# phantomzone-org/fhe-ram

Measured on AMD Instinct MI355X. Metric: encrypted RAM read ops/s + write ops/s at 2^18 entries; achieved HBM GB/s vs peak, higher is better.
Workload: dtype f64

## Files before the change

### fhe-ram_amd/csrc/ctx.hpp

```cpp
#pragma once
#include "../../include/fheram.h"
#include "kernels.hpp"
#include "cmux_chain.hpp"
#include "mapped_chains.hpp"

#include <algorithm>
#include <atomic>
#include <cstdio>
#include <cstdlib>
#include <cstring>
#include <map>
#include <string>
#include <vector>

using namespace fk;

namespace {

thread_local std::string g_create_err;


struct ProfCls {
    uint64_t launches = 0, blocks = 0;
    double ms = 0.0;
    std::vector<std::pair<hipEvent_t, hipEvent_t>> pending;
};

}

inline uint64_t next_addr_id() { static std::atomic<uint64_t> n{0}; return ++n; }

struct RamState {
    bool initialized = false, state = false;
    bool memo_top = false;
    int memo_alone = 0;
    bool res_in_trtop = false;
};

struct DenseBufs {
    int cap = 0;
    int32_t *A = nullptr, *B = nullptr, *C = nullptr, *D = nullptr;
    int32_t *part = nullptr, *tmp = nullptr, *tmp2 = nullptr, *res = nullptr, *tree = nullptr, *w = nullptr, *trtop = nullptr;
    double* prep = nullptr;
    int64_t *h_res = nullptr, *d_h_res = nullptr;
};

inline fheram_config config_builtin() {
    fheram_config d{};
    d.limb_split = 1; d.fine_split = 1; d.memo = 1; d.pre_inv = 1; d.tail = 1; d.tail_test = 0; d.mid = 2; d.mid_test = 0;
    d.chain = 1; d.chain_y = 3; d.pair_z = 1; d.fuse = 1; d.graph = 0; d.safe = 0; d.nco = 0; d.tail_ep = 1; d.monitor = 1; d.reserved = 0;
    return d;
}
inline fheram_config config_in_effect(const fheram_config& in) {
    using C = fheram_config;
    fheram_config e{};
    for (int32_t C::*on_off : {&C::limb_split, &C::fine_split, &C::memo, &C::tail, &C::tail_ep, &C::mid_test, &C::chain, &C::pair_z, &C::fuse, &C::graph, &C::safe})
        e.*on_off = in.*on_off ? 1 : 0;
    for (int32_t C::*upto2 : {&C::tail_test, &C::mid, &C::monitor}) e.*upto2 = in.*upto2 < 0 ? 0 : (in.*upto2 > 2 ? 2 : in.*upto2);
    e.chain_y = in.chain_y ? 3 : 0;
    e.nco = in.nco == 2 ? 2 : (in.nco == 1 ? 1 : 0);
    e.pre_inv = e.memo ? (in.pre_inv == 2 ? 2 : (in.pre_inv ? 1 : 0)) : 0;
    if (e.graph) e.pre_inv = 0;
    if (e.safe) { e.tail = 0; e.tail_test = 0; e.mid = 0; e.mid_test = 0; if (e.pre_inv == 1) e.pre_inv = 2; }
    if (e.safe && e.monitor == 1) e.monitor = 2;
    return e;
}

struct CtxResources {
    std::vector<void*> dev, pinned;
    std::vector<hipEvent_t> events;
    template <typename T> hipError_t device(T** p, size_t bytes) { const hipError_t e = hipMalloc((void**)p, bytes); if (e == hipSuccess) dev.push_back(*p); return e; }
    template <typename T> hipError_t host(T** p, size_t bytes, unsigned flags) { const hipError_t e = hipHostMalloc((void**)p, bytes, flags); if (e == hipSuccess) pinned.push_back(*p); return e; }
    hipError_t event(hipEvent_t* ev, bool timing = false) {
        const hipError_t e = timing ? hipEventCreate(ev) : hipEventCreateWithFlags(ev, hipEventDisableTiming);
        if (e == hipSuccess) events.push_back(*ev);
        return e;
    }
    void release() {
        for (hipEvent_t e : events) hipEventDestroy(e);
        for (void* p : dev) hipFree(p);
        for (void* p : pinned) hipHostFree(p);
        events.clear(); dev.clear(); pinned.clear();
    }
};

struct fheram_ctx {
    fheram_params p;
    int device = 0;
    int ws = 0, n2 = 0, n_digits = 0, max_digits = 0;
    size_t rows = 0;
    size_t rows_glob = 0;
    int shard = 0, n_shards = 1;
    std::vector<std::vector<int>> base2d;
    static constexpr int S_CT = 3, S_ADDR = 4, S_INV = 5, DNUM_CT = 3, DNUM_GGSW = 4;
    int s_evk = 4;
    size_t atk = 0;
    static constexpr size_t GLWE = (size_t)S_CT * 2 * N;
    static constexpr size_t GLWE4 = (size_t)S_ADDR * 2 * N;
    static constexpr size_t GGSW = (size_t)DNUM_CT * 2 * GLWE4;
    static constexpr size_t EVK5 = (size_t)DNUM_GGSW * S_INV * 2 * N;
    static constexpr size_t GGSW5 = (size_t)DNUM_GGSW * 2 * S_INV * 2 * N;
    int cus = 256;
    CtxResources res;
    hipStream_t stream = nullptr;
    hipStream_t stream2 = nullptr;
    hipStream_t cur = nullptr;
    hipEvent_t ev_fork = nullptr, ev_join = nullptr;
    hipEvent_t ev_xout = nullptr, ev_xin = nullptr;
    fheram_config cfg = config_builtin();
    bool wide = false;
    double* d_tw = nullptr;
    double ninv = 0.0;
    double* d_atk = nullptr;
    double* d_atk_inv = nullptr;
    double* d_tsk = nullptr;
    int64_t gal[LOGN];
    bool keys_loaded = false;
    unsigned* h_ro_flag = nullptr;
    int32_t* d_data = nullptr;
    int32_t* d_tree = nullptr;
    int32_t* d_scrA = nullptr;
    int32_t* d_scrB = nullptr;
    int32_t* d_scrC = nullptr;
    int32_t* d_scrD = nullptr;
    int32_t* d_res = nullptr;
    int32_t* d_tmp = nullptr;
    int32_t* d_tmp2 = nullptr;
    int32_t* d_w = nullptr;
    int32_t* d_trtop = nullptr;
    int32_t* d_part = nullptr;
    int32_t* d_gat[3] = {nullptr, nullptr, nullptr};
    RamState ram;
    DenseBufs batch;
    double* d_big = nullptr;
    double* d_big2 = nullptr;
    double* d_prep = nullptr;
    bool prep1_ready = false;
    int32_t* d_ggsw_tmp = nullptr;
    int32_t* d_ggsw_tmp2 = nullptr;
    unsigned tail_seq = 0;
    int tail_xoff = 0;
    uint64_t tail_launches = 0;
    unsigned* h_tail_fb = nullptr;
    unsigned tail_fb_mark = 0;
    uint64_t tail_launch_mark = 0;
    unsigned* d_tail_sync = nullptr;
    unsigned mid_seq = 0;
    uint64_t mid_launches = 0, mid_launch_mark = 0;
    unsigned mid_fb_mark = 0;
    int mid_bad_windows = 0, mid_saved = 0;
    uint64_t mid_window_cts = 0, mid_disabled_count = 0;
    unsigned mid_off_ops = 0;
    unsigned* h_mid_fb = nullptr;
    unsigned* d_mid_sync[2] = {nullptr, nullptr};
    double* d_mid_big[2] = {nullptr, nullptr};
    double* d_mid_y[2] = {nullptr, nullptr};
    uint64_t inv_id[2] = {0, 0};
    double* d_prep_inv = nullptr;
    int32_t* d_ggsw_inv = nullptr;
    hipEvent_t ev_inv[2] = {nullptr, nullptr};
    bool inv_pending[2] = {false, false};
    hipEvent_t ev_wdone = nullptr;
    bool wdone_pending = false;
    hipEvent_t ev_opstart = nullptr;
    bool opstart_valid = false;
    bool wide_unsynced = false;
    bool derive_unsynced = false;
    bool main_idle = false;
    int32_t* h_pin[2] = {nullptr, nullptr};
    hipEvent_t ev_pin[2] = {nullptr, nullptr};
    int64_t* h_res = nullptr;
    int64_t* d_h_res = nullptr;
    int32_t* h_w = nullptr;
    hipEvent_t ev_w = nullptr;
    bool w_busy = false;
    bool side_begun = false;
    bool trhi_in_C = false;
    bool tree_rotate_pending = false;
    bool words_staged = false;
    int profile = 0;
    std::map<std::string, ProfCls> prof;
    std::vector<hipEvent_t> ev_pool;
    hipEvent_t t0 = nullptr, t1 = nullptr;
    std::string err;
};

struct fheram_addr {
    fheram_ctx* ctx;
    int32_t* d_ggsw;
    int n_digits;
    int device;
    uint64_t id = next_addr_id();
    hipGraphExec_t graph[3] = {nullptr, nullptr, nullptr};
    unsigned graph_sig[3] = {0, 0, 0};
    bool empty = false;
};

struct fheram_fheuint {
    fheram_ctx* ctx;
    int device, n_bits;
    int32_t* d_std;
    double* d_prep;
};

struct fheram_secret {
    fheram_ctx* ctx;
    int device;
    std::vector<int32_t> sk;
    double* d_hat;
};

namespace {

int fail(fheram_ctx* c, int code, const std::string& msg) {
    if (c) c->err = msg; else g_create_err = msg;
    return code;
}
int check_precision(fheram_ctx* c) {
    if (c->h_ro_flag && __atomic_load_n(c->h_ro_flag, __ATOMIC_RELAXED))
        return fail(c, FHERAM_ERR_PRECISION, "FP64 round-off of an inverse transform exceeded 3/8 (fheram_roundoff_max): the rounded integers are no longer trustworthy");
    return FHERAM_OK;
}
#define HIPCHK(c, call)                                                                     \
    do {                                                                                    \
        hipError_t e_ = (call);                                                             \
        if (e_ != hipSuccess)                                                               \
            return fail((c), FHERAM_ERR_DEVICE, std::string(#call) + ": " + hipGetErrorString(e_)); \
    } while (0)

GlweRef ref(int32_t* p, long sy, long sx) { return GlweRef{p, sy, sx}; }

void main_waited(fheram_ctx* c) { c->wide_unsynced = c->derive_unsynced = false; c->main_idle = true; }
void main_enqueued(fheram_ctx* c) { c->main_idle = false; }

hipEvent_t get_event(fheram_ctx* c) {
    if (!c->ev_pool.empty()) { hipEvent_t e = c->ev_pool.back(); c->ev_pool.pop_back(); return e; }
    hipEvent_t e = nullptr; c->res.event(&e, true); return e;
}
struct ProfScope {
    fheram_ctx* c; ProfCls* cls = nullptr; hipEvent_t a = nullptr;
    ProfScope(fheram_ctx* c_, const char* name, uint64_t blocks, int steps = 1) : c(c_) {
        if (!c->profile) return;
        if (c->profile == 2 && !strstr(name, "chain_launch")) return;
        cls = &c->prof[name];
        cls->launches += steps; cls->blocks += blocks * steps;
        a = get_event(c);
        hipEventRecord(a, c->cur);
    }
    ~ProfScope() {
        if (!cls) return;
        hipEvent_t b = get_event(c);
        hipEventRecord(b, c->cur);
        cls->pending.emplace_back(a, b);
    }
};
void prof_collect(fheram_ctx* c) {
    for (auto& kv : c->prof) {
        for (auto& pr : kv.second.pending) {
            hipEventSynchronize(pr.second);
            float ms = 0.f;
            hipEventElapsedTime(&ms, pr.first, pr.second);
            kv.second.ms += ms;
            c->ev_pool.push_back(pr.first); c->ev_pool.push_back(pr.second);
        }
        kv.second.pending.clear();
    }
}

std::vector<std::vector<int>> base_2d(uint64_t max_addr, const fheram_params& p) {
    std::vector<std::vector<int>> plan;
    uint32_t x = (uint32_t)(max_addr - 1), bits = 0;
    while (x) { bits++; x >>= 1; }
    while (bits != 0) {
        std::vector<int> v;
        for (uint32_t i = 0; i < p.n_decomp; i++) {
            const uint32_t b = p.decomp_n[i];
            if (b <= bits) { v.push_back((int)b); bits -= b; }
            else { if (bits != 0) { v.push_back((int)bits); bits = 0; } break; }
        }
        plan.push_back(v);
    }
    return plan;
}
int ilog2_ceil(size_t x) { int k = 0; while (((size_t)1 << k) < x) k++; return k; }
int galois_mod(int64_t g) { const int64_t m = 2 * N; return (int)(((g % m) + m) % m); }
int galois_inv_mod(int g) {
    int64_t r = 1, b = g, e = N - 1, m = 2 * N;
    while (e) { if (e & 1) r = r * b % m; b = b * b % m; e >>= 1; }
    return (int)r;
}
int64_t galois_element(int i) {
    if (i == 0) return -1;
    int64_t g = 5, e = (int64_t)1 << (i - 1), r = 1, m = 2 * N;
    while (e) { if (e & 1) r = r * g % m; g = g * g % m; e >>= 1; }
    return r;
}

bool narrow(const int64_t* src, int32_t* dst, size_t n) {
    int64_t bad = 0;
    for (size_t i = 0; i < n; i++) {
        const int64_t v = src[i];
        bad |= (v > 65536) | (v < -65536);
        dst[i] = (int32_t)v;
    }
    return bad == 0;
}
void widen(const int32_t* src, int64_t* dst, size_t n) { for (size_t i = 0; i < n; i++) dst[i] = src[i]; }

constexpr size_t PIN_CHUNK = (size_t)1 << 21;
int pin_init(fheram_ctx* c) {
    if (c->h_pin[0]) return FHERAM_OK;
    for (int b = 0; b < 2; b++) {
        HIPCHK(c, c->res.host(&c->h_pin[b], PIN_CHUNK * sizeof(int32_t), hipHostMallocDefault));
        HIPCHK(c, c->res.event(&c->ev_pin[b]));
    }
    return FHERAM_OK;
}
int upload_i64(fheram_ctx* c, int32_t* dst, const int64_t* src, size_t n) {
    int rc = pin_init(c);
    if (rc != FHERAM_OK) return rc;
    bool ok = true;
    int k = 0;
    for (size_t off = 0; off < n && ok; off += PIN_CHUNK, k++) {
        const int b = k & 1;
        const size_t m = std::min(PIN_CHUNK, n - off);
        if (k >= 2) HIPCHK(c, hipEventSynchronize(c->ev_pin[b]));
        ok = narrow(src + off, c->h_pin[b], m);
        if (!ok) break;
        HIPCHK(c, hipMemcpyAsync(dst + off, c->h_pin[b], m * sizeof(int32_t), hipMemcpyHostToDevice, c->stream));
        HIPCHK(c, hipEventRecord(c->ev_pin[b], c->stream));
    }
    HIPCHK(c, hipStreamSynchronize(c->stream));
    if (!ok) return fail(c, FHERAM_ERR_RANGE, "limb out of the normalised range [-2^16, 2^16]");
    return FHERAM_OK;
}
int download_i64(fheram_ctx* c, int64_t* dst, const int32_t* src, size_t n) {
    int rc = pin_init(c);
    if (rc != FHERAM_OK) return rc;
    const size_t n_chunks = (n + PIN_CHUNK - 1) / PIN_CHUNK;
    for (size_t k = 0; k <= n_chunks; k++) {
        if (k < n_chunks) {
            const size_t off = k * PIN_CHUNK, m = std::min(PIN_CHUNK, n - off);
            HIPCHK(c, hipMemcpyAsync(c->h_pin[k & 1], src + off, m * sizeof(int32_t), hipMemcpyDeviceToHost, c->stream));
            HIPCHK(c, hipEventRecord(c->ev_pin[k & 1], c->stream));
        }
        if (k > 0) {
            const size_t off = (k - 1) * PIN_CHUNK, m = std::min(PIN_CHUNK, n - off);
            HIPCHK(c, hipEventSynchronize(c->ev_pin[(k - 1) & 1]));
            widen(c->h_pin[(k - 1) & 1], dst + off, m);
        }
    }
    return FHERAM_OK;
}
int stage_words(fheram_ctx* c, int32_t* d_w, const int64_t* w, int n_ct) {
    if (c->w_busy) { HIPCHK(c, hipEventSynchronize(c->ev_w)); c->w_busy = false; }
    const size_t n = (size_t)n_ct * fheram_ctx::GLWE;
    if (!narrow(w, c->h_w, n)) return fail(c, FHERAM_ERR_RANGE, "limb out of the normalised range [-2^16, 2^16]");
    main_enqueued(c);
    HIPCHK(c, hipMemcpyAsync(d_w, c->h_w, n * sizeof(int32_t), hipMemcpyHostToDevice, c->stream));
    HIPCHK(c, hipEventRecord(c->ev_w, c->stream));
    c->w_busy = true;
    return FHERAM_OK;
}

}
```

### fhe-ram_amd/csrc/fheram.hip

```cpp
#include <unistd.h>
#include <atomic>
#include "path.hpp"

extern "C" {

int fheram_params_default(fheram_params* p) {
    if (!p) return FHERAM_ERR_INVALID_ARG;
    std::memset(p, 0, sizeof(*p));
    p->log_n = 12; p->base2k = 17; p->rank = 1;
    p->k_glwe_pt = 3; p->k_glwe_ct = 51; p->k_ggsw_addr = 68; p->k_evk_trace = 68; p->k_evk_ggsw_inv = 85;
    p->word_size = 4; p->n_decomp = 4;
    p->decomp_n[0] = p->decomp_n[1] = p->decomp_n[2] = p->decomp_n[3] = 3;
    p->max_addr = (uint64_t)1 << 14;
    return FHERAM_OK;
}

const char* fheram_last_error(const fheram_ctx* c) { return c ? c->err.c_str() : g_create_err.c_str(); }

void fheram_config_default(fheram_config* cfg) {
    if (!cfg) return;
    fheram_config d = config_builtin();
    auto env = [](const char* n) { const char* v = getenv(n); return (v && v[0]) ? v[0] : '\0'; };
    if (env("FHERAM_LIMB_SPLIT") == '0') d.limb_split = 0;
    if (env("FHERAM_FINE_SPLIT") == '0') d.fine_split = 0;
    if (env("FHERAM_MEMO") == '0') d.memo = 0;
    if (env("FHERAM_PRE_INV") == '0') d.pre_inv = 0; else if (env("FHERAM_PRE_INV") == '2') d.pre_inv = 2;
    const char tl = env("FHERAM_TAIL");
    if (tl == '0') d.tail = 0;
    d.tail_test = tl == '2' ? 1 : (tl == '3' ? 2 : 0);
    const char md = env("FHERAM_MID");
    d.mid = md == '0' ? 0 : (md == '1' ? 1 : 2);
    d.mid_test = md == '2' ? 1 : 0;
    if (env("FHERAM_CHAIN") == '0') d.chain = 0;
    if (env("FHERAM_CHAIN_Y") == '0') d.chain_y = 0;
    if (env("FHERAM_PAIR_Z") == '0') d.pair_z = 0;
    if (env("FHERAM_FUSE") == '0') d.fuse = 0;
    if (env("FHERAM_GRAPH") == '1') d.graph = 1;
    if (env("FHERAM_SAFE") == '1') d.safe = 1;
    const char nc = env("FHERAM_NCO");
    d.nco = nc == '2' ? 2 : (nc == '1' ? 1 : 0);
    if (env("FHERAM_TAIL_EP") == '0') d.tail_ep = 0;
    const char mo = env("FHERAM_MONITOR");
    if (mo == '0') d.monitor = 0; else if (mo == '2') d.monitor = 2;
    *cfg = d;
}

int fheram_ctx_create(const fheram_params* p, int device, fheram_ctx** out) {
    return fheram_ctx_create_cfg(p, device, 0, 1, nullptr, out);
}

int fheram_ctx_create_sharded(const fheram_params* p, int device, int shard, int n_shards, fheram_ctx** out) {
    return fheram_ctx_create_cfg(p, device, shard, n_shards, nullptr, out);
}

int fheram_ctx_create_cfg(const fheram_params* p, int device, int shard, int n_shards, const fheram_config* user_cfg, fheram_ctx** out) {
    if (!p || !out) return fail(nullptr, FHERAM_ERR_INVALID_ARG, "null argument");
    *out = nullptr;
    if (n_shards < 1 || shard < 0 || shard >= n_shards || (n_shards & (n_shards - 1)) != 0)
        return fail(nullptr, FHERAM_ERR_INVALID_ARG, "n_shards must be a power of two and 0 <= shard < n_shards");
    auto limbs = [&](uint32_t k) { return (k + p->base2k - 1) / (p->base2k ? p->base2k : 1); };
    if (p->log_n != 12 || p->base2k != 17 || p->rank != 1 || p->k_glwe_ct == 0 || limbs(p->k_glwe_ct) != 3 || limbs(p->k_ggsw_addr) != 4 ||
        (limbs(p->k_evk_trace) != 4 && limbs(p->k_evk_trace) != 5) || limbs(p->k_evk_ggsw_inv) != 5)
        return fail(nullptr, FHERAM_ERR_UNSUPPORTED, "kernels are built for LOG_N=12, BASE2K=17, RANK=1 and limb counts K_CT: 3, K_ADDR: 4, K_EVK_TRACE: 4 or 5, K_EVK_GGSW_INV: 5");
    if (p->k_glwe_pt == 0 || p->k_glwe_pt > p->k_glwe_ct)
        return fail(nullptr, FHERAM_ERR_INVALID_ARG, "k_glwe_pt must be in [1, k_glwe_ct]");
    if (p->word_size == 0 || p->word_size > 64 || p->n_decomp == 0 || p->n_decomp > 16 || p->max_addr < 2)
        return fail(nullptr, FHERAM_ERR_INVALID_ARG, "bad word_size / decomp_n / max_addr");
    unsigned sum = 0;
    for (uint32_t i = 0; i < p->n_decomp; i++) { if (p->decomp_n[i] == 0) return fail(nullptr, FHERAM_ERR_INVALID_ARG, "zero digit width"); sum += p->decomp_n[i]; }
    if (sum != p->log_n) return fail(nullptr, FHERAM_ERR_INVALID_ARG, "DECOMP_N must sum to LOG_N (parameters.rs:168)");
    if (p->max_addr > ((uint64_t)N * N)) return fail(nullptr, FHERAM_ERR_UNSUPPORTED, "max_addr > N^2 is not supported by the reference either (SURVEY.md 3.1)");
    if (user_cfg && user_cfg->reserved != 0)
        return fail(nullptr, FHERAM_ERR_INVALID_ARG, "fheram_config.reserved must be 0 (start from fheram_config_default())");

    int ndev = 0;
    if (hipGetDeviceCount(&ndev) != hipSuccess || ndev <= 0)
        return fail(nullptr, FHERAM_ERR_DEVICE, "no HIP device: the FHE-RAM evaluator has no CPU path");
    if (device < 0 || device >= ndev) return fail(nullptr, FHERAM_ERR_INVALID_ARG, "bad device index");

    fheram_ctx* c = new fheram_ctx();
    c->p = *p; c->device = device; c->ws = (int)p->word_size;
    c->s_evk = (int)limbs(p->k_evk_trace);
    c->atk = (size_t)fheram_ctx::DNUM_CT * c->s_evk * 2 * N;
    c->rows_glob = (size_t)((p->max_addr + N - 1) / N);
    c->shard = shard; c->n_shards = n_shards;
    if (n_shards > 1 && ((c->rows_glob & (c->rows_glob - 1)) != 0 || c->rows_glob < (size_t)n_shards)) {
        delete c;
        return fail(nullptr, FHERAM_ERR_INVALID_ARG, "row sharding needs a power-of-two number of rows >= n_shards (else: replicas only)");
    }
    c->rows = c->rows_glob / (size_t)n_shards;
    c->base2d = base_2d(p->max_addr, *p);
    c->n2 = (int)c->base2d.size();
    for (auto& v : c->base2d) { c->n_digits += (int)v.size(); c->max_digits = std::max(c->max_digits, (int)v.size()); }
    for (int i = 0; i < LOGN; i++) c->gal[i] = galois_element(i);

#define CCHK(call)                                                                  \
    do {                                                                            \
        hipError_t e_ = (call);                                                     \
        if (e_ != hipSuccess) {                                                     \
            g_create_err = std::string(#call) + ": " + hipGetErrorString(e_);       \
            fheram_ctx_destroy(c);                                                  \
            return FHERAM_ERR_DEVICE;                                               \
        }                                                                           \
    } while (0)
    CCHK(hipSetDevice(device));
    CCHK(hipStreamCreateWithFlags(&c->stream, hipStreamNonBlocking));
    {
        int lo = 0, hi = 0;
        CCHK(hipDeviceGetStreamPriorityRange(&lo, &hi));
        CCHK(hipStreamCreateWithPriority(&c->stream2, hipStreamNonBlocking, lo));
    }
    c->cur = c->stream;
    for (hipEvent_t* ev : {&c->ev_fork, &c->ev_join, &c->ev_xout, &c->ev_xin}) CCHK(c->res.event(ev));
    for (hipEvent_t* ev : {&c->t0, &c->t1}) CCHK(c->res.event(ev, true));
    fheram_config asked;
    if (user_cfg) asked = *user_cfg; else fheram_config_default(&asked);
    c->cfg = config_in_effect(asked);
    static std::atomic<int> serial{0};
    c->tail_xoff = ((serial++ + (int)getpid()) & 1) * (TAIL_GROUPS / 2);
    hipDeviceProp_t prop;
    if (hipGetDeviceProperties(&prop, device) == hipSuccess && prop.multiProcessorCount > 0) c->cus = prop.multiProcessorCount;
#define LDSATTR(k) CCHK(hipFuncSetAttribute(reinterpret_cast<const void*>(k), hipFuncAttributeMaxDynamicSharedMemorySize, (int)LDS_BYTES))
    LDSATTR(k_prepare);
    LDSATTR((&k_ext_product<3, 4, 1>));
    LDSATTR((&k_ext_product<3, 4, 2>));
    LDSATTR((&k_ext_product<3, 4, 1, 1>));
    LDSATTR((&k_ext_product_fine<3, 4>));
    LDSATTR((&k_ext_product_fine<4, 5>));
    LDSATTR((&k_ext_product_chain<3, 4>));
    LDSATTR((&k_ext_product_chain_r<4>));
    LDSATTR((&k_pair_z<4>)); LDSATTR((&k_pair_z<5>));
    LDSATTR((&k_read_chain<4, 4>)); LDSATTR((&k_read_chain<5, 4>)); LDSATTR((&k_write_chain<4, 4>)); LDSATTR((&k_write_chain<5, 4>));
    LDSATTR((&k_write_chain_t<4, 4>)); LDSATTR((&k_write_chain_t<5, 4>));
    LDSATTR((&k_read_chain_w<4, 4>)); LDSATTR((&k_read_chain_w<5, 4>));
    LDSATTR((&k_read_chain_t<4, 4>)); LDSATTR((&k_read_chain_t<5, 4>));
    LDSATTR((&k_trace_tail_t<3, 4, 3>)); LDSATTR((&k_trace_tail_t<3, 5, 3>));
    LDSATTR((&k_keyswitch_chain_w<3, 4, 3, 3>)); LDSATTR((&k_keyswitch_chain_w<3, 5, 3, 3>));
    LDSATTR((&k_keyswitch_chain<3, 4, 3>));
    LDSATTR((&k_keyswitch_chain<3, 4, 3, 3>));
    LDSATTR((&k_keyswitch_chain<3, 5, 3, 3>));
    LDSATTR((&k_trace_tail<3, 4, 3>));
    LDSATTR((&k_chain_mid<false, 4, 3, 2>)); LDSATTR((&k_chain_mid<false, 5, 3, 2>)); LDSATTR((&k_chain_mid<true, 4, 3, 2>));
    LDSATTR((&k_chain_mid<false, 4, 1, 1>)); LDSATTR((&k_chain_mid<false, 5, 1, 1>));
    LDSATTR((&k_chain_mid<false, 4, 1, 2>)); LDSATTR((&k_chain_mid<false, 5, 1, 2>));
#define LDSATTR_KS4(M, SX, SK, SO) LDSATTR((&k_keyswitch<M, SX, SK, SO, 1>)); LDSATTR((&k_keyswitch<M, SX, SK, SO, 1, 1>)); LDSATTR((&k_keyswitch_fine<M, SX, SK>))
#define LDSATTR_KS(M, SX, SK, SO) LDSATTR_KS4(M, SX, SK, SO); LDSATTR((&k_keyswitch<M, SX, SK, SO, 2>))
    LDSATTR_KS(KS_AUTO, 3, 4, 3);
    LDSATTR_KS(KS_TRACE, 3, 4, 3);
    LDSATTR_KS4(KS_PAIR, 3, 4, 3);
    LDSATTR_KS(KS_ADD, 3, 4, 3);
    LDSATTR_KS(KS_SUBNEG, 3, 4, 3);
    LDSATTR((&k_keyswitch_chain<3, 5, 3>));
    LDSATTR((&k_trace_tail<3, 5, 3>));
    LDSATTR_KS(KS_AUTO, 3, 5, 3);
    LDSATTR_KS(KS_TRACE, 3, 5, 3);
    LDSATTR_KS4(KS_PAIR, 3, 5, 3);
    LDSATTR_KS(KS_ADD, 3, 5, 3);
    LDSATTR_KS(KS_SUBNEG, 3, 5, 3);
    LDSATTR_KS4(KS_AUTO, 4, 5, 4);
    LDSATTR_KS4(KS_TENSOR, 4, 5, 4);
    LDSATTR((&k_encrypt_sk<1, 1>));
    LDSATTR((&k_encrypt_sk<3, 0>)); LDSATTR((&k_encrypt_sk<3, 1>));
    LDSATTR((&k_encrypt_sk<4, 0>)); LDSATTR((&k_encrypt_sk<4, 1>));
    LDSATTR((&k_encrypt_sk<5, 0>)); LDSATTR((&k_encrypt_sk<5, 1>));
    CCHK(cmux_chain_register());
    CCHK(mapped_chains_register());
#undef LDSATTR_KS
#undef LDSATTR_KS4
#undef LDSATTR

    std::vector<double> tw = make_fft_twiddles();
    c->ninv = 1.0 / (double)NC;
    {
        CCHK(c->res.host(&c->h_ro_flag, 64, hipHostMallocDefault));
        *c->h_ro_flag = 0;
        const uint64_t mode = (uint64_t)c->cfg.monitor, flag_addr = (uint64_t)(size_t)c->h_ro_flag;
        std::memcpy(&tw[0], &mode, 8);
        std::memcpy(&tw[N + 1], &flag_addr, 8);
    }
    CCHK(c->res.device(&c->d_tw, TW_GLOBAL * sizeof(double)));
    CCHK(hipMemcpy(c->d_tw, tw.data(), TW_GLOBAL * sizeof(double), hipMemcpyHostToDevice));
    const size_t G = fheram_ctx::GLWE, nrow = (size_t)c->ws * c->rows;
    CCHK(c->res.device(&c->d_atk, (size_t)LOGN * c->atk * sizeof(double)));
    for (double** key : {&c->d_atk_inv, &c->d_tsk}) CCHK(c->res.device(key, fheram_ctx::EVK5 * sizeof(double)));
    for (int32_t** arena : {&c->d_data, &c->d_scrA, &c->d_scrB, &c->d_scrC, &c->d_scrD}) CCHK(c->res.device(arena, nrow * G * sizeof(int32_t)));
    CCHK(c->res.device(&c->d_ggsw_tmp2, (size_t)c->max_digits * fheram_ctx::GGSW * sizeof(int32_t)));
    for (int32_t** ct : {&c->d_tmp2, &c->d_part}) CCHK(c->res.device(ct, (size_t)c->ws * G * sizeof(int32_t)));
    for (double** big : {&c->d_big, &c->d_big2}) CCHK(c->res.device(big, (size_t)LIMB_SPLIT_MAX * BIG_STRIDE * sizeof(double)));
    if (n_shards > 1) for (int i = 0; i < 3; i++) CCHK(c->res.device(&c->d_gat[i], (size_t)n_shards * c->ws * G * sizeof(int32_t)));
    for (int32_t** ct : {&c->d_tree, &c->d_res, &c->d_tmp, &c->d_w, &c->d_trtop}) CCHK(c->res.device(ct, (size_t)c->ws * G * sizeof(int32_t)));
    CCHK(c->res.device(&c->d_prep, (size_t)std::max(c->n_digits, c->max_digits) * fheram_ctx::GGSW * sizeof(double)));
    CCHK(c->res.device(&c->d_ggsw_tmp, (size_t)c->max_digits * fheram_ctx::GGSW * sizeof(int32_t)));
    CCHK(hipMemset(c->d_tree, 0, (size_t)c->ws * G * sizeof(int32_t)));
    CCHK(c->res.device(&c->d_prep_inv, (size_t)c->n_digits * fheram_ctx::GGSW * sizeof(double)));
    CCHK(c->res.device(&c->d_ggsw_inv, (size_t)c->n_digits * fheram_ctx::GGSW * sizeof(int32_t)));
    for (hipEvent_t* ev : {&c->ev_inv[0], &c->ev_inv[1], &c->ev_wdone, &c->ev_opstart}) CCHK(c->res.event(ev));
    CCHK(c->res.device(&c->d_tail_sync, (size_t)(TAIL_GROUPS + 1) * 32 * sizeof(unsigned)));
    CCHK(hipMemset(c->d_tail_sync, 0, (size_t)(TAIL_GROUPS + 1) * 32 * sizeof(unsigned)));
    for (int i = 0; i < 2; i++) {
        CCHK(c->res.device(&c->d_mid_sync[i], (size_t)(MID_GROUPS_MAX + 1) * 32 * sizeof(unsigned)));
        CCHK(hipMemset(c->d_mid_sync[i], 0, (size_t)(MID_GROUPS_MAX + 1) * 32 * sizeof(unsigned)));
        CCHK(c->res.device(&c->d_mid_y[i], (size_t)2 * MID_GROUPS_MAX * 2 * N * sizeof(double)));
        CCHK(c->res.device(&c->d_mid_big[i], (size_t)2 * MID_GROUPS_MAX * BIG_STRIDE * sizeof(double)));
    }
    CCHK(c->res.host(&c->h_tail_fb, 64, hipHostMallocDefault));
    *c->h_tail_fb = 0;
    CCHK(c->res.host(&c->h_mid_fb, 128, hipHostMallocDefault));
    memset(c->h_mid_fb, 0, 128);
    CCHK(c->res.host(&c->h_res, ((size_t)c->ws * G + 1) * sizeof(int64_t), hipHostMallocMapped));
    CCHK(hipHostGetDevicePointer((void**)&c->d_h_res, c->h_res, 0));
    CCHK(c->res.host(&c->h_w, (size_t)c->ws * G * sizeof(int32_t), hipHostMallocDefault));
    CCHK(c->res.event(&c->ev_w));
#undef CCHK
    *out = c;
    return FHERAM_OK;
}

void fheram_ctx_destroy(fheram_ctx* c) {
    if (!c) return;
    hipSetDevice(c->device);
    for (hipStream_t s : {c->stream, c->stream2}) if (s) hipStreamSynchronize(s);
    prof_collect(c);
    dense_free(c->batch);
    c->res.release();
    for (hipStream_t s : {c->stream2, c->stream}) if (s) hipStreamDestroy(s);
    delete c;
}

int fheram_ctx_config(const fheram_ctx* c, fheram_config* out) {
    if (!c || !out) return FHERAM_ERR_INVALID_ARG;
    *out = c->cfg;
    out->reserved = 0;
    return FHERAM_OK;
}

size_t fheram_glwe_len(const fheram_ctx*) { return fheram_ctx::GLWE; }
size_t fheram_ggsw_len(const fheram_ctx*) { return fheram_ctx::GGSW; }
size_t fheram_atk_len(const fheram_ctx* c) { return c ? c->atk : 0; }
size_t fheram_evk_inv_len(const fheram_ctx*) { return fheram_ctx::EVK5; }
size_t fheram_rows(const fheram_ctx* c) { return c ? c->rows : 0; }
int fheram_n_digits(const fheram_ctx* c) { return c ? c->n_digits : 0; }
int fheram_n_coordinates(const fheram_ctx* c) { return c ? c->n2 : 0; }

int fheram_keys_load(fheram_ctx* c, const int64_t* gal_els, int n_gal, const int64_t* const* atk_glwe,
                     const int64_t* atk_ggsw_inv, int64_t atk_ggsw_inv_p, const int64_t* tsk) {
    if (!c) return FHERAM_ERR_INVALID_ARG;
    if (!gal_els || !atk_glwe || !atk_ggsw_inv || !tsk) return fail(c, FHERAM_ERR_INVALID_ARG, "null key pointer");
    if (n_gal != LOGN) return fail(c, FHERAM_ERR_KEYS, "expected log2(N) trace keys (keys.rs:39)");
    if (atk_ggsw_inv_p != -1) return fail(c, FHERAM_ERR_KEYS, "auto_key.p() != -1 (coordinate_prepared.rs:134)");
    HIPCHK(c, hipSetDevice(c->device));
    HIPCHK(c, hipStreamSynchronize(c->stream));
    HIPCHK(c, hipStreamSynchronize(c->stream2));
    int order[LOGN];
    for (int i = 0; i < LOGN; i++) {
        order[i] = -1;
        for (int j = 0; j < n_gal; j++) if (gal_els[j] == c->gal[i]) order[i] = j;
        if (order[i] < 0) return fail(c, FHERAM_ERR_KEYS, "missing trace key for a Galois element of GLWE::trace_galois_elements");
    }
    int32_t* d_stage = nullptr;
    const size_t stage_n = std::max(c->atk, fheram_ctx::EVK5);
    HIPCHK(c, hipMalloc(&d_stage, stage_n * sizeof(int32_t)));
    int rc = FHERAM_OK;
    for (int i = 0; i < LOGN && rc == FHERAM_OK; i++) {
        rc = upload_i64(c, d_stage, atk_glwe[order[i]], c->atk);
        if (rc == FHERAM_OK) launch_prepare(c, d_stage, c->d_atk + (size_t)i * c->atk, (int)(c->atk / N), c->gal[i]);
        hipStreamSynchronize(c->stream);
    }
    if (rc == FHERAM_OK) rc = upload_i64(c, d_stage, atk_ggsw_inv, fheram_ctx::EVK5);
    if (rc == FHERAM_OK) { launch_prepare(c, d_stage, c->d_atk_inv, (int)(fheram_ctx::EVK5 / N), -1); hipStreamSynchronize(c->stream); }
    if (rc == FHERAM_OK) rc = upload_i64(c, d_stage, tsk, fheram_ctx::EVK5);
    if (rc == FHERAM_OK) { launch_prepare(c, d_stage, c->d_tsk, (int)(fheram_ctx::EVK5 / N)); hipStreamSynchronize(c->stream); }
    hipFree(d_stage);
    if (rc != FHERAM_OK) return rc;
    HIPCHK(c, hipGetLastError());
    c->keys_loaded = true;
    c->inv_id[0] = c->inv_id[1] = 0;
    c->inv_pending[0] = c->inv_pending[1] = false;
    c->ram.memo_top = false; c->ram.memo_alone = 0;
    return FHERAM_OK;
}

int fheram_ram_upload(fheram_ctx* c, const int64_t* rows) {
    if (!c) return FHERAM_ERR_INVALID_ARG;
    if (!rows) return fail(c, FHERAM_ERR_INVALID_ARG, "null rows");
    HIPCHK(c, hipSetDevice(c->device));
    int rc = upload_i64(c, c->d_data, rows, (size_t)c->ws * c->rows * fheram_ctx::GLWE);
    if (rc != FHERAM_OK) return rc;
    c->ram.initialized = true; c->ram.state = false; c->ram.memo_top = false; c->ram.memo_alone = 0;
    return FHERAM_OK;
}
int fheram_ram_download(fheram_ctx* c, int64_t* rows) {
    if (!c || !rows) return FHERAM_ERR_INVALID_ARG;
    if (!c->ram.initialized) return fail(c, FHERAM_ERR_UNINITIALIZED, "unitialized memory: self.data.len()=0");
    HIPCHK(c, hipSetDevice(c->device));
    const int rc = download_i64(c, rows, c->d_data, (size_t)c->ws * c->rows * fheram_ctx::GLWE);
    return rc == FHERAM_OK ? check_precision(c) : rc;
}
int fheram_ram_tree_download(fheram_ctx* c, int level, int64_t* out) {
    if (!c || !out) return FHERAM_ERR_INVALID_ARG;
    if (level != 0 || c->n2 < 2) return fail(c, FHERAM_ERR_INVALID_ARG, "tree level does not exist (ram.rs:315-324)");
    HIPCHK(c, hipSetDevice(c->device));
    return download_i64(c, out, c->d_tree, (size_t)c->ws * fheram_ctx::GLWE);
}
int fheram_ram_state(const fheram_ctx* c) { return c ? (int)c->ram.state : 0; }

int fheram_address_create(fheram_ctx* c, const int64_t* const* ggsw, int n_ggsw, fheram_addr** out) {
    if (!c || !out) return FHERAM_ERR_INVALID_ARG;
    *out = nullptr;
    if (!ggsw) return fail(c, FHERAM_ERR_INVALID_ARG, "null ggsw");
    if (n_ggsw != c->n_digits) return fail(c, FHERAM_ERR_INVALID_ARG, "address digit count does not match the context's Base2D (ram.rs:404)");
    HIPCHK(c, hipSetDevice(c->device));
    fheram_addr* a = new fheram_addr{c, nullptr, n_ggsw, c->device};
    hipError_t e = hipMalloc(&a->d_ggsw, (size_t)n_ggsw * fheram_ctx::GGSW * sizeof(int32_t));
    if (e != hipSuccess) { delete a; return fail(c, FHERAM_ERR_DEVICE, std::string("hipMalloc: ") + hipGetErrorString(e)); }
    for (int i = 0; i < n_ggsw; i++) {
        if (!ggsw[i]) { fheram_address_destroy(a); return fail(c, FHERAM_ERR_INVALID_ARG, "null ggsw digit"); }
        int rc = upload_i64(c, a->d_ggsw + (size_t)i * fheram_ctx::GGSW, ggsw[i], fheram_ctx::GGSW);
        if (rc != FHERAM_OK) { fheram_address_destroy(a); return rc; }
    }
    *out = a;
    return FHERAM_OK;
}
void fheram_address_destroy(fheram_addr* a) {
    if (!a) return;
    hipSetDevice(a->device);
    for (auto& g : a->graph) if (g) { hipGraphExecDestroy(g); g = nullptr; }
    if (a->d_ggsw) hipFree(a->d_ggsw);
    delete a;
}

int fheram_result_map(fheram_ctx* c, const int64_t** out) {
    if (!c || !out) return FHERAM_ERR_INVALID_ARG;
    HIPCHK(c, hipSetDevice(c->device));
    const ResRun run{c->ram.res_in_trtop ? c->d_trtop : c->d_res, (size_t)c->ws * fheram_ctx::GLWE};
    *out = c->h_res;
    return result_export(c, &run, 1, c->h_res, c->d_h_res, nullptr);
}
int fheram_result_download(fheram_ctx* c, int64_t* out) {
    if (!c || !out) return FHERAM_ERR_INVALID_ARG;
    const int64_t* src = nullptr;
    const int rc = fheram_result_map(c, &src);
    if (rc != FHERAM_OK) return rc;
    std::memcpy(out, src, (size_t)c->ws * fheram_ctx::GLWE * sizeof(int64_t));
    return FHERAM_OK;
}
int fheram_sync(fheram_ctx* c) {
    if (!c) return FHERAM_ERR_INVALID_ARG;
    HIPCHK(c, hipSetDevice(c->device));
    HIPCHK(c, hipStreamSynchronize(c->stream));
    HIPCHK(c, hipGetLastError());
    main_waited(c);
    return check_precision(c);
}
int fheram_roundoff_max(fheram_ctx* c, double* max_out) {
    if (!c || !max_out) return FHERAM_ERR_INVALID_ARG;
    HIPCHK(c, hipSetDevice(c->device));
    HIPCHK(c, hipStreamSynchronize(c->stream));
    HIPCHK(c, hipStreamSynchronize(c->stream2));
    double m = 0.0;
    HIPCHK(c, hipMemcpy(&m, c->d_tw + N, sizeof(double), hipMemcpyDeviceToHost));
    *max_out = m;
    if (c->cfg.monitor && m > MON_LIMIT) __atomic_store_n(c->h_ro_flag, 1u, __ATOMIC_RELAXED);
    return check_precision(c);
}
int fheram_roundoff_reset(fheram_ctx* c) {
    if (!c) return FHERAM_ERR_INVALID_ARG;
    HIPCHK(c, hipSetDevice(c->device));
    HIPCHK(c, hipStreamSynchronize(c->stream));
    HIPCHK(c, hipStreamSynchronize(c->stream2));
    HIPCHK(c, hipMemset(c->d_tw + N, 0, sizeof(double)));
    __atomic_store_n(c->h_ro_flag, 0u, __ATOMIC_RELAXED);
    return FHERAM_OK;
}

int fheram_read(fheram_ctx* c, const fheram_addr* addr, int64_t* out) {
    int rc = check_common(c, addr);
    if (rc != FHERAM_OK) return rc;
    if (c->n_shards != 1) return fail(c, FHERAM_ERR_INVALID_ARG, "row-sharded context: use fheram_read_partial / fheram_read_finish");
    if (c->ram.state) return fail(c, FHERAM_ERR_STATE, "invalid call to Memory.read: internal state is true -> requires calling Memory.write");
    HIPCHK(c, hipSetDevice(c->device));
    rc = run_op(c, addr, 0, [&] { return read_impl(one_addr(c, &addr), ctx_view(c), false); });
    if (rc != FHERAM_OK) return rc;
    HIPCHK(c, hipGetLastError());
    return out ? fheram_result_download(c, out) : FHERAM_OK;
}
int fheram_read_batch(fheram_ctx* c, const fheram_addr* const* addrs, int n_addr, int64_t* out) {
    if (!c) return FHERAM_ERR_INVALID_ARG;
    if (!addrs) return fail(c, FHERAM_ERR_INVALID_ARG, "null address list");
    if (n_addr < 1 || n_addr > FHERAM_READ_BATCH_MAX)
        return fail(c, FHERAM_ERR_INVALID_ARG, "n_addr = " + std::to_string(n_addr) + " is outside [1, FHERAM_READ_BATCH_MAX = " + std::to_string(FHERAM_READ_BATCH_MAX) + "]");
    for (int k = 0; k < n_addr; k++) {
        const int rc = check_common(c, addrs[k]);
        if (rc != FHERAM_OK) return rc;
    }
    if (c->n_shards != 1) return fail(c, FHERAM_ERR_INVALID_ARG, "row-sharded context: use fheram_read_partial / fheram_read_finish");
    if (c->ram.state) return fail(c, FHERAM_ERR_STATE, "invalid call to Memory.read: internal state is true -> requires calling Memory.write");
    HIPCHK(c, hipSetDevice(c->device));
    int rc;
    if (n_addr == 1) {
        rc = run_op(c, addrs[0], 0, [&] { return read_impl(one_addr(c, addrs), ctx_view(c), false); });
        if (rc != FHERAM_OK) return rc;
        HIPCHK(c, hipGetLastError());
        return out ? fheram_result_download(c, out) : FHERAM_OK;
    }
    return read_many(c, c->batch, &c->ram, addrs, n_addr, c->ws, 0, false, out, [&](const Opnds& o) {
        launch_copy(c, o.slice(ref(c->batch.res, (long)fheram_ctx::GLWE, 0), n_addr - 1), ref(c->d_res, (long)fheram_ctx::GLWE, 0), 1, c->ws);
    });
}
int fheram_read_prepare_write(fheram_ctx* c, const fheram_addr* addr, int64_t* out) {
    int rc = check_common(c, addr);
    if (rc != FHERAM_OK) return rc;
    if (c->n_shards != 1) return fail(c, FHERAM_ERR_INVALID_ARG, "row-sharded context: use fheram_read_partial / fheram_read_finish");
    if (c->ram.state) return fail(c, FHERAM_ERR_STATE, "invalid call to Memory.read: internal state is true -> requires calling Memory.write");
    HIPCHK(c, hipSetDevice(c->device));
    rc = run_op(c, addr, 1, [&] { return read_impl(one_addr(c, &addr), ctx_view(c), true); });
    if (rc != FHERAM_OK) return rc;
    c->ram.state = true;
    HIPCHK(c, hipGetLastError());
    return out ? fheram_result_download(c, out) : FHERAM_OK;
}
int fheram_word_stage(fheram_ctx* c, const int64_t* w, int n_w) {
    if (!c || !w) return FHERAM_ERR_INVALID_ARG;
    if (n_w != c->ws) return fail(c, FHERAM_ERR_INVALID_ARG, "w.len() != subrams.len() (ram.rs:243)");
    HIPCHK(c, hipSetDevice(c->device));
    const int rc = stage_words(c, c->d_w, w, c->ws);
    if (rc == FHERAM_OK) c->words_staged = true;
    return rc;
}
int fheram_write(fheram_ctx* c, const int64_t* w, int n_w, const fheram_addr* addr) {
    int rc = check_common(c, addr);
    if (rc != FHERAM_OK) return rc;
    if (n_w != c->ws) return fail(c, FHERAM_ERR_INVALID_ARG, "w.len() != subrams.len() (ram.rs:243)");
    if (!c->ram.state) return fail(c, FHERAM_ERR_STATE, "invalid call to Memory.write: internal state is false -> requires calling Memory.read_prepare_write");
    HIPCHK(c, hipSetDevice(c->device));
    if (c->n_shards != 1) return fail(c, FHERAM_ERR_INVALID_ARG, "row-sharded context: use fheram_write_root / fheram_write_shard");
    if (!w && !c->words_staged) return fail(c, FHERAM_ERR_INVALID_ARG, "w == NULL and no staged words");
    const Opnds o = one_addr(c, &addr);
    if (w && !c->side_begun && !capturing(c)) write_side_begin(o, ctx_view(c));
    if (w) { rc = fheram_word_stage(c, w, n_w); if (rc != FHERAM_OK) { write_side_abort(c); return rc; } }
    rc = run_op(c, addr, 2, [&] {
        if (!c->side_begun) write_side_begin(o, ctx_view(c));
        int r2 = write_top(o, ctx_view(c));
        return r2 == FHERAM_OK ? write_rows(o, ctx_view(c)) : r2;
    });
    if (rc != FHERAM_OK) return rc;
    c->ram.state = false;
    HIPCHK(c, hipGetLastError());
    return FHERAM_OK;
}

namespace {
int export_glwes(fheram_ctx* c, const int32_t* src, void* dst, int on_device, size_t n_glwe) {
    const size_t n = n_glwe * fheram_ctx::GLWE;
    if (on_device) { main_enqueued(c); HIPCHK(c, hipMemcpyAsync(dst, src, n * 4, hipMemcpyDeviceToDevice, c->stream)); return FHERAM_OK; }
    return download_i64(c, (int64_t*)dst, src, n);
}
int import_glwes(fheram_ctx* c, int32_t* dst, const void* src, int on_device, size_t n_glwe) {
    const size_t n = n_glwe * fheram_ctx::GLWE;
    if (on_device) { main_enqueued(c); HIPCHK(c, hipMemcpyAsync(dst, src, n * 4, hipMemcpyDeviceToDevice, c->stream)); return FHERAM_OK; }
    return upload_i64(c, dst, (const int64_t*)src, n);
}
}

int fheram_shard_info(const fheram_ctx* c, int* shard, int* n_shards, size_t* local_rows) {
    if (!c) return FHERAM_ERR_INVALID_ARG;
    if (shard) *shard = c->shard;
    if (n_shards) *n_shards = c->n_shards;
    if (local_rows) *local_rows = c->rows;
    return FHERAM_OK;
}
int fheram_read_partial(fheram_ctx* c, const fheram_addr* addr, int prepare_write, void* out, int out_on_device) {
    int rc = check_common(c, addr);
    if (rc != FHERAM_OK) return rc;
    if (!out) return fail(c, FHERAM_ERR_INVALID_ARG, "null output");
    if (c->ram.state) return fail(c, FHERAM_ERR_STATE, "invalid call to Memory.read: internal state is true -> requires calling Memory.write");
    HIPCHK(c, hipSetDevice(c->device));
    GlweRef packed;
    rc = read_local(one_addr(c, &addr), ctx_view(c), prepare_write != 0, &packed, true);
    if (rc != FHERAM_OK) return rc;
    HIPCHK(c, hipGetLastError());
    if (prepare_write) c->ram.state = true;
    return export_glwes(c, c->d_part, out, out_on_device, (size_t)c->ws);
}
int fheram_stream_signal(fheram_ctx* c, void* hip_stream) {
    if (!c) return FHERAM_ERR_INVALID_ARG;
    HIPCHK(c, hipSetDevice(c->device));
    main_enqueued(c);
    HIPCHK(c, hipEventRecord(c->ev_xout, c->stream));
    HIPCHK(c, hipStreamWaitEvent((hipStream_t)hip_stream, c->ev_xout, 0));
    return FHERAM_OK;
}
int fheram_stream_wait(fheram_ctx* c, void* hip_stream) {
    if (!c) return FHERAM_ERR_INVALID_ARG;
    HIPCHK(c, hipSetDevice(c->device));
    HIPCHK(c, hipEventRecord(c->ev_xin, (hipStream_t)hip_stream));
    main_enqueued(c);
    HIPCHK(c, hipStreamWaitEvent(c->stream, c->ev_xin, 0));
    return FHERAM_OK;
}
int fheram_device_malloc(fheram_ctx* c, size_t bytes, void** out) {
    if (!c || !out || bytes == 0) return fail(c, FHERAM_ERR_INVALID_ARG, "bad argument");
    HIPCHK(c, hipSetDevice(c->device));
    HIPCHK(c, hipMalloc(out, bytes));
    return FHERAM_OK;
}
int fheram_device_free(fheram_ctx* c, void* ptr) {
    if (!c) return FHERAM_ERR_INVALID_ARG;
    HIPCHK(c, hipSetDevice(c->device));
    HIPCHK(c, hipFree(ptr));
    return FHERAM_OK;
}
int fheram_write_begin(fheram_ctx* c, const fheram_addr* addr) {
    int rc = check_common(c, addr);
    if (rc != FHERAM_OK) return rc;
    if (!c->ram.state) return fail(c, FHERAM_ERR_STATE, "invalid call to Memory.write: internal state is false -> requires calling Memory.read_prepare_write");
    HIPCHK(c, hipSetDevice(c->device));
    if (!c->side_begun) write_side_begin(one_addr(c, &addr), ctx_view(c));
    HIPCHK(c, hipGetLastError());
    return FHERAM_OK;
}
int fheram_read_finish(fheram_ctx* c, const fheram_addr* addr, int prepare_write, const void* partials, int partials_on_device, int64_t* out) {
    int rc = check_common(c, addr);
    if (rc != FHERAM_OK) return rc;
    if (!partials) return fail(c, FHERAM_ERR_INVALID_ARG, "null partials");
    HIPCHK(c, hipSetDevice(c->device));
    int32_t* gathered = nullptr;
    if (c->n_shards > 1) {
        rc = import_glwes(c, c->d_gat[0], partials, partials_on_device, (size_t)c->n_shards * c->ws);
        gathered = c->d_gat[0];
    } else {
        rc = import_glwes(c, c->d_part, partials, partials_on_device, (size_t)c->ws);
    }
    if (rc != FHERAM_OK) return rc;
    rc = read_top(one_addr(c, &addr), ctx_view(c), prepare_write != 0, gathered, ref(c->d_part, (long)fheram_ctx::GLWE, 0));
    if (rc != FHERAM_OK) return rc;
    HIPCHK(c, hipGetLastError());
    return out ? fheram_result_download(c, out) : fheram_sync(c);
}
int fheram_write_root(fheram_ctx* c, const int64_t* w, int n_w, const fheram_addr* addr, void* ct_lo_out, int out_on_device) {
    int rc = check_common(c, addr);
    if (rc != FHERAM_OK) return rc;
    if (n_w != c->ws) return fail(c, FHERAM_ERR_INVALID_ARG, "w.len() != subrams.len() (ram.rs:243)");
    if (c->n2 != 2) return fail(c, FHERAM_ERR_INVALID_ARG, "a row-sharded RAM has two coordinates");
    if (!c->ram.state) return fail(c, FHERAM_ERR_STATE, "invalid call to Memory.write: internal state is false -> requires calling Memory.read_prepare_write");
    if (!ct_lo_out) return fail(c, FHERAM_ERR_INVALID_ARG, "null output");
    HIPCHK(c, hipSetDevice(c->device));
    if (w) { rc = fheram_word_stage(c, w, n_w); if (rc != FHERAM_OK) return rc; }
    else if (!c->words_staged) return fail(c, FHERAM_ERR_INVALID_ARG, "w == NULL and no staged words");
    if (!c->side_begun) write_side_begin(one_addr(c, &addr), ctx_view(c));
    rc = write_top(one_addr(c, &addr), ctx_view(c));
    if (rc != FHERAM_OK) return rc;
    HIPCHK(c, hipGetLastError());
    return export_glwes(c, c->d_part, ct_lo_out, out_on_device, (size_t)c->ws);
}
int fheram_write_shard(fheram_ctx* c, const fheram_addr* addr, const void* ct_lo, int on_device) {
    int rc = check_common(c, addr);
    if (rc != FHERAM_OK) return rc;
    if (!ct_lo) return fail(c, FHERAM_ERR_INVALID_ARG, "null ct_lo");
    if (!c->ram.state) return fail(c, FHERAM_ERR_STATE, "invalid call to Memory.write: internal state is false -> requires calling Memory.read_prepare_write");
    HIPCHK(c, hipSetDevice(c->device));
    if (!c->side_begun) write_side_begin(one_addr(c, &addr), ctx_view(c));
    rc = import_glwes(c, c->d_part, ct_lo, on_device, (size_t)c->ws);
    if (rc != FHERAM_OK) { write_side_abort(c); return rc; }
    rc = write_rows(one_addr(c, &addr), ctx_view(c));
    if (rc != FHERAM_OK) return rc;
    HIPCHK(c, hipGetLastError());
    return FHERAM_OK;
}

namespace {
struct DevBuf {
    int32_t* p = nullptr;
    ~DevBuf() { if (p) hipFree(p); }
};
}

int fheram_glwe_external_product(fheram_ctx* c, const int64_t* a, int batch, const int64_t* ggsw, int64_t* res) {
    if (!c || !a || !ggsw || !res || batch <= 0) return fail(c, FHERAM_ERR_INVALID_ARG, "bad argument");
    HIPCHK(c, hipSetDevice(c->device));
    const size_t G = fheram_ctx::GLWE;
    DevBuf da, dg;
    HIPCHK(c, hipMalloc(&da.p, (size_t)batch * G * 4));
    HIPCHK(c, hipMalloc(&dg.p, fheram_ctx::GGSW * 4));
    int rc = upload_i64(c, da.p, a, (size_t)batch * G);
    if (rc == FHERAM_OK) rc = upload_i64(c, dg.p, ggsw, fheram_ctx::GGSW);
    if (rc != FHERAM_OK) return rc;
    DevBuf dout;
    HIPCHK(c, hipMalloc(&dout.p, (size_t)batch * G * 4));
    launch_prepare(c, dg.p, c->d_prep, (int)(fheram_ctx::GGSW / N));
    launch_ep(c, ref(da.p, 0, (long)G), ref(dout.p, 0, (long)G), c->d_prep, batch, 1);
    HIPCHK(c, hipGetLastError());
    return download_i64(c, res, dout.p, (size_t)batch * G);
}
int fheram_glwe_automorphism(fheram_ctx* c, int mode, int64_t gal_el, const int64_t* a, int batch, int64_t* res) {
    if (!c || !a || !res || batch <= 0 || mode < 0 || mode > 2) return fail(c, FHERAM_ERR_INVALID_ARG, "bad argument");
    if (!c->keys_loaded) return fail(c, FHERAM_ERR_KEYS, "evaluation keys not loaded");
    int ki = -1;
    for (int i = 0; i < LOGN; i++) if (c->gal[i] == gal_el) ki = i;
    if (ki < 0) return fail(c, FHERAM_ERR_KEYS, "no key for this Galois element");
    HIPCHK(c, hipSetDevice(c->device));
    const size_t G = fheram_ctx::GLWE;
    DevBuf da, dout;
    HIPCHK(c, hipMalloc(&da.p, (size_t)batch * G * 4));
    HIPCHK(c, hipMalloc(&dout.p, (size_t)batch * G * 4));
    int rc = upload_i64(c, da.p, a, (size_t)batch * G);
    if (rc != FHERAM_OK) return rc;
    KsArgs ka = ks_args(c, ref(da.p, 0, (long)G), ref(da.p, 0, 0), ref(dout.p, 0, (long)G), trace_key(c, ki), gal_el);
    if (mode == 0) launch_ks_tr<KS_AUTO>(c, ka, batch, 1);
    else if (mode == 1) launch_ks_tr<KS_ADD>(c, ka, batch, 1);
    else launch_ks_tr<KS_SUBNEG>(c, ka, batch, 1);
    HIPCHK(c, hipGetLastError());
    return download_i64(c, res, dout.p, (size_t)batch * G);
}
int fheram_glwe_trace(fheram_ctx* c, int start, int end, const int64_t* a, int batch, int64_t* res) {
    if (!c || !a || !res || batch <= 0 || start < 0 || end > LOGN || start > end) return fail(c, FHERAM_ERR_INVALID_ARG, "bad argument");
    if (!c->keys_loaded) return fail(c, FHERAM_ERR_KEYS, "evaluation keys not loaded");
    HIPCHK(c, hipSetDevice(c->device));
    const size_t G = fheram_ctx::GLWE;
    DevBuf da, db, dc;
    HIPCHK(c, hipMalloc(&da.p, (size_t)batch * G * 4));
    HIPCHK(c, hipMalloc(&db.p, (size_t)batch * G * 4));
    HIPCHK(c, hipMalloc(&dc.p, (size_t)batch * G * 4));
    int rc = upload_i64(c, da.p, a, (size_t)batch * G);
    if (rc != FHERAM_OK) return rc;
    trace_steps(c, ref(da.p, 0, (long)G), ref(db.p, 0, (long)G), ref(dc.p, 0, (long)G), start, end, batch, 1);
    HIPCHK(c, hipGetLastError());
    return download_i64(c, res, db.p, (size_t)batch * G);
}
int fheram_glwe_pack(fheram_ctx* c, const int64_t* cts, int count, int64_t* out) {
    if (!c || !cts || !out || count <= 0 || count > N) return fail(c, FHERAM_ERR_INVALID_ARG, "bad argument");
    if (!c->keys_loaded) return fail(c, FHERAM_ERR_KEYS, "evaluation keys not loaded");
    HIPCHK(c, hipSetDevice(c->device));
    const size_t G = fheram_ctx::GLWE;
    DevBuf src, A, B;
    HIPCHK(c, hipMalloc(&src.p, (size_t)count * G * 4));
    HIPCHK(c, hipMalloc(&A.p, (size_t)count * G * 4));
    HIPCHK(c, hipMalloc(&B.p, (size_t)count * G * 4));
    int rc = upload_i64(c, src.p, cts, (size_t)count * G);
    if (rc != FHERAM_OK) return rc;
    const int L0p = LOGN - ilog2_ceil((size_t)count);
    int32_t* packed = pack_levels(c, src.p, A.p, B.p, 0, (long)G, (size_t)count, 1, L0p, L0p);
    HIPCHK(c, hipGetLastError());
    return download_i64(c, out, packed, G);
}
int fheram_ggsw_automorphism_inv(fheram_ctx* c, const int64_t* ggsw_in, int64_t* ggsw_out) {
    if (!c || !ggsw_in || !ggsw_out) return fail(c, FHERAM_ERR_INVALID_ARG, "bad argument");
    if (!c->keys_loaded) return fail(c, FHERAM_ERR_KEYS, "evaluation keys not loaded");
    HIPCHK(c, hipSetDevice(c->device));
    DevBuf din;
    HIPCHK(c, hipMalloc(&din.p, fheram_ctx::GGSW * 4));
    int rc = upload_i64(c, din.p, ggsw_in, fheram_ctx::GGSW);
    if (rc != FHERAM_OK) return rc;
    ggsw_inverse(c, din.p, c->d_ggsw_tmp, 1);
    HIPCHK(c, hipGetLastError());
    return download_i64(c, ggsw_out, c->d_ggsw_tmp, fheram_ctx::GGSW);
}

int fheram_timer_begin(fheram_ctx* c) {
    if (!c) return FHERAM_ERR_INVALID_ARG;
    HIPCHK(c, hipSetDevice(c->device));
    HIPCHK(c, hipEventRecord(c->t0, c->stream));
    return FHERAM_OK;
}
int fheram_timer_end(fheram_ctx* c, float* ms) {
    if (!c || !ms) return FHERAM_ERR_INVALID_ARG;
    HIPCHK(c, hipSetDevice(c->device));
    HIPCHK(c, hipEventRecord(c->t1, c->stream));
    HIPCHK(c, hipEventSynchronize(c->t1));
    HIPCHK(c, hipEventElapsedTime(ms, c->t0, c->t1));
    main_waited(c);
    return check_precision(c);
}
int fheram_profile_enable(fheram_ctx* c, int on) {
    if (!c) return FHERAM_ERR_INVALID_ARG;
    c->profile = on == 2 ? 2 : (on != 0);
    return FHERAM_OK;
}
int fheram_profile_reset(fheram_ctx* c) {
    if (!c) return FHERAM_ERR_INVALID_ARG;
    hipSetDevice(c->device);
    prof_collect(c);
    c->prof.clear();
    return FHERAM_OK;
}
int fheram_profile_get(fheram_ctx* c, const char* cls, uint64_t* launches, uint64_t* blocks, double* total_ms) {
    if (!c || !cls) return FHERAM_ERR_INVALID_ARG;
    hipSetDevice(c->device);
    prof_collect(c);
    auto it = c->prof.find(cls);
    if (launches) *launches = it == c->prof.end() ? 0 : it->second.launches;
    if (blocks) *blocks = it == c->prof.end() ? 0 : it->second.blocks;
    if (total_ms) *total_ms = it == c->prof.end() ? 0.0 : it->second.ms;
    return FHERAM_OK;
}
int fheram_mid_stats(fheram_ctx* c, uint64_t* launches, uint64_t* fallbacks) {
    if (!c) return FHERAM_ERR_INVALID_ARG;
    HIPCHK(c, hipSetDevice(c->device));
    unsigned fb[2] = {0, 0};
    HIPCHK(c, hipStreamSynchronize(c->stream2));
    for (int i = 0; i < 2; i++)
        HIPCHK(c, hipMemcpyAsync(&fb[i], c->d_mid_sync[i] + MID_GROUPS_MAX * 32 + 1, sizeof(unsigned), hipMemcpyDeviceToHost, c->stream));
    HIPCHK(c, hipStreamSynchronize(c->stream));
    if (launches) *launches = c->mid_launches;
    if (fallbacks) *fallbacks = (uint64_t)fb[0] + fb[1];
    return FHERAM_OK;
}
int fheram_mid_state(const fheram_ctx* c, int* enabled, uint64_t* times_disabled) {
    if (!c) return FHERAM_ERR_INVALID_ARG;
    if (enabled) *enabled = c->cfg.mid;
    if (times_disabled) *times_disabled = c->mid_disabled_count;
    return FHERAM_OK;
}
int fheram_tail_stats(fheram_ctx* c, uint64_t* launches, uint64_t* fallbacks) {
    if (!c) return FHERAM_ERR_INVALID_ARG;
    HIPCHK(c, hipSetDevice(c->device));
    unsigned fb = 0;
    HIPCHK(c, hipMemcpyAsync(&fb, c->d_tail_sync + TAIL_GROUPS * 32 + 1, sizeof(unsigned), hipMemcpyDeviceToHost, c->stream));
    HIPCHK(c, hipStreamSynchronize(c->stream));
    if (launches) *launches = c->tail_launches;
    if (fallbacks) *fallbacks = fb;
    return FHERAM_OK;
}
#ifdef FK_STAMP
int fheram_debug_ntt_probe(fheram_ctx* c, int blocks) {
    hipSetDevice(c->device);
    double* sink = nullptr;
    hipMalloc(&sink, (size_t)blocks * T * sizeof(double));
    hipFuncSetAttribute(reinterpret_cast<const void*>(k_ntt_probe), hipFuncAttributeMaxDynamicSharedMemorySize, (int)LDS_BYTES);
    for (int i = 0; i < 3; i++) hipLaunchKernelGGL(k_ntt_probe, dim3(blocks), dim3(T), LDS_BYTES, c->stream, c->d_tw, sink);
    hipStreamSynchronize(c->stream);
    hipFree(sink);
    return 0;
}
int fheram_debug_stamps(fheram_ctx* c, unsigned long long* out, int n) {
    hipSetDevice(c->device);
    hipStreamSynchronize(c->stream);
    return hipMemcpyFromSymbol(out, HIP_SYMBOL(g_stamps), sizeof(unsigned long long) * (n > 192 ? 192 : n)) == hipSuccess ? 0 : 7;
}
#endif
int fheram_bench_external_product(fheram_ctx* c, int batch, int iters, float* total_ms) {
    if (!c || !total_ms || batch <= 0 || iters <= 0) return fail(c, FHERAM_ERR_INVALID_ARG, "bad argument");
    HIPCHK(c, hipSetDevice(c->device));
    const size_t G = fheram_ctx::GLWE;
    DevBuf da, db, dg;
    HIPCHK(c, hipMalloc(&da.p, (size_t)batch * G * 4));
    HIPCHK(c, hipMalloc(&db.p, (size_t)batch * G * 4));
    HIPCHK(c, hipMalloc(&dg.p, fheram_ctx::GGSW * 4));
    {
        std::vector<int32_t> h(std::max((size_t)batch * G, fheram_ctx::GGSW));
        uint64_t x = 0x9E3779B97F4A7C15ull;
        for (auto& v : h) { x ^= x << 13; x ^= x >> 7; x ^= x << 17; v = (int32_t)(x & 0x1FFFF) - 65536; }
        HIPCHK(c, hipMemcpy(da.p, h.data(), (size_t)batch * G * 4, hipMemcpyHostToDevice));
        HIPCHK(c, hipMemcpy(dg.p, h.data(), fheram_ctx::GGSW * 4, hipMemcpyHostToDevice));
    }
    c->cur = c->stream;
    launch_prepare(c, dg.p, c->d_prep, (int)(fheram_ctx::GGSW / N));
    GlweRef ra = ref(da.p, 0, (long)G), rb = ref(db.p, 0, (long)G);
    for (int i = 0; i < 3; i++) { launch_ep(c, ra, rb, c->d_prep, batch, 1); launch_ep(c, rb, ra, c->d_prep, batch, 1); }
    HIPCHK(c, hipEventRecord(c->t0, c->stream));
    for (int i = 0; i < iters; i++) launch_ep(c, (i & 1) ? rb : ra, (i & 1) ? ra : rb, c->d_prep, batch, 1);
    HIPCHK(c, hipEventRecord(c->t1, c->stream));
    HIPCHK(c, hipEventSynchronize(c->t1));
    HIPCHK(c, hipEventElapsedTime(total_ms, c->t0, c->t1));
    HIPCHK(c, hipGetLastError());
    return FHERAM_OK;
}
int fheram_bench_chain(fheram_ctx* c, int kind, int batch, int n, int iters, float* total_ms) {
    if (!c || !total_ms || batch <= 0 || iters <= 0 || n < 1 || n > CHAIN_MAX || kind < 0 || kind > 1) return fail(c, FHERAM_ERR_INVALID_ARG, "bad argument");
    if (kind == 1 && n > c->n_digits) return fail(c, FHERAM_ERR_INVALID_ARG, "a product chain is at most as long as the address has digits (d_prep holds n_digits prepared GGSWs)");
    HIPCHK(c, hipSetDevice(c->device));
    const size_t G = fheram_ctx::GLWE;
    DevBuf da, db, dc, dg;
    HIPCHK(c, hipMalloc(&da.p, (size_t)batch * G * 4));
    HIPCHK(c, hipMalloc(&db.p, (size_t)batch * G * 4));
    HIPCHK(c, hipMalloc(&dc.p, (size_t)batch * G * 4));
    HIPCHK(c, hipMalloc(&dg.p, (size_t)n * fheram_ctx::GGSW * 4));
    {
        std::vector<int32_t> h(std::max((size_t)batch * G, (size_t)n * fheram_ctx::GGSW));
        uint64_t x = 0x9E3779B97F4A7C15ull;
        for (auto& v : h) { x ^= x << 13; x ^= x >> 7; x ^= x << 17; v = (int32_t)(x & 0x1FFFF) - 65536; }
        HIPCHK(c, hipMemcpy(da.p, h.data(), (size_t)batch * G * 4, hipMemcpyHostToDevice));
        HIPCHK(c, hipMemcpy(dg.p, h.data(), (size_t)n * fheram_ctx::GGSW * 4, hipMemcpyHostToDevice));
        if (kind == 0 && !c->keys_loaded)
            for (int i = 0; i < LOGN; i++) { c->cur = c->stream; launch_prepare(c, dg.p, c->d_atk + (size_t)i * c->atk, (int)(c->atk / N), c->gal[i]); }
    }
    c->cur = c->stream;
    if (kind == 1) launch_prepare(c, dg.p, c->d_prep, n * (int)(fheram_ctx::GGSW / N));
    GlweRef ra = ref(da.p, 0, (long)G), rb = ref(db.p, 0, (long)G), rc = ref(dc.p, 0, (long)G);
    auto once = [&](int i) {
        GlweRef src = (i & 1) ? rb : ra, dst = (i & 1) ? ra : rb;
        if (kind == 0) trace_steps(c, src, dst, rc, 0, n, batch, 1);
        else ep_chain(c, src, dst, rc, c->d_prep, n, batch, 1);
    };
    for (int i = 0; i < 4; i++) once(i);
    HIPCHK(c, hipEventRecord(c->t0, c->stream));
    for (int i = 0; i < iters; i++) once(i);
    HIPCHK(c, hipEventRecord(c->t1, c->stream));
    HIPCHK(c, hipEventSynchronize(c->t1));
    HIPCHK(c, hipEventElapsedTime(total_ms, c->t0, c->t1));
    HIPCHK(c, hipGetLastError());
    return FHERAM_OK;
}
int fheram_device_info(const fheram_ctx* c, char* name, size_t name_len, int* cus) {
    if (!c) return FHERAM_ERR_INVALID_ARG;
    hipDeviceProp_t prop;
    if (hipGetDeviceProperties(&prop, c->device) != hipSuccess) return FHERAM_ERR_DEVICE;
    if (name && name_len) { std::snprintf(name, name_len, "%s (%s)", prop.name, prop.gcnArchName); }
    if (cus) *cus = prop.multiProcessorCount;
    return FHERAM_OK;
}

}

#include "setup.hpp"
#include "selftest.hpp"
#include "group.hpp"
#include "bank.hpp"
#include "select.hpp"
```

### fhe-ram_amd/csrc/kernels.hpp

```cpp
#pragma once
#include "../../include/fheram.h"
#include "fft_dev.hpp"
#include <type_traits>

namespace fk {

#ifdef FK_STAMP
__device__ unsigned long long g_stamps[192];
#define STAMP(i)                                                                                   \
    do {                                                                                           \
        __builtin_amdgcn_sched_barrier(0);                                                         \
        if (threadIdx.x == 0 && blockIdx.x == 0 && blockIdx.y == 0 && blockIdx.z == 0) {           \
            unsigned long long t_;                                                                 \
            asm volatile("s_memtime %0\n\ts_waitcnt lgkmcnt(0)" : "=s"(t_)::"memory");            \
            g_stamps[i] = t_;                                                                      \
        }                                                                                          \
        __builtin_amdgcn_sched_barrier(0);                                                         \
    } while (0)
#define STAMPZ(i)                                                                                  \
    do {                                                                                           \
        __builtin_amdgcn_sched_barrier(0);                                                         \
        if (threadIdx.x == 0 && blockIdx.x == 0 && blockIdx.y == 0 && (blockIdx.z == 0 || blockIdx.z == 3)) { \
            unsigned long long t_;                                                                 \
            asm volatile("s_memtime %0\n\ts_waitcnt lgkmcnt(0)" : "=s"(t_)::"memory");            \
// ... 1209 lines not shown
        using std::true_type;
        using std::false_type;
        if (cc == 0) {
#pragma unroll 1
            for (int j = SG - 1; j >= 0; j--) unit(true_type{}, true_type{}, j);
        } else {
#pragma unroll 1
            for (int j = SG - 1; j >= 2; j--) unit(true_type{}, true_type{}, j);
            unit(true_type{}, false_type{}, 1);
            unit(false_type{}, false_type{}, 0);
        }
#pragma unroll
        for (int k = 0; k < E; k++) {
            double a_ = window51(od[k]);
            if constexpr (OUT == 1) {
                if (co == 0) park[64 * k] = a_; else ac[k] = a_;
            } else if constexpr (OUT == 3) {
                const double yn = __builtin_floor(__builtin_fma(a_, 0.5, 0.5));
                if (co == 1) data[2 * LDS_DATA + tid + T * k] = yn; else ac[k] = yn;
                if (store_i32) {
                    const double d2 = take_digit(a_);
                    const double d1 = take_digit(a_);
                    gstore_i32(rp + glwe_off(2, co), (unsigned)(tid + T * k) * 4u, (int)d2);
                    gstore_i32(rp + glwe_off(1, co), (unsigned)(tid + T * k) * 4u, (int)d1);
                    gstore_i32(rp + glwe_off(0, co), (unsigned)(tid + T * k) * 4u, (int)a_);
                }
            } else {
                const double d2 = take_digit(a_);
                const double d1 = take_digit(a_);
                gstore_i32(rp + glwe_off(2, co), (unsigned)(tid + T * k) * 4u, (int)d2);
                gstore_i32(rp + glwe_off(1, co), (unsigned)(tid + T * k) * 4u, (int)d1);
                gstore_i32(rp + glwe_off(0, co), (unsigned)(tid + T * k) * 4u, (int)a_);
            }
        }
    }
    YSTAMP(5);
}
template <int SG>
__global__ __launch_bounds__(T, T / 256) __attribute__((amdgpu_num_vgpr(FK_CHAIN_VGPRS))) void k_ext_product_chain_r(EpChainArgs ca) {
    extern __shared__ __attribute__((aligned(16))) double lds[];
    RoMonitor ro_mon(lds, ca.tw);
    GlweRef in = ca.src;
    double ac[E];
#pragma unroll
    for (int k = 0; k < E; k++) ac[k] = 0.0;
#pragma unroll 1
    for (int i = 0; i < ca.n; i++) {
        const GlweRef out = ca.buf[i & 1];
        int tid = vt((int)threadIdx.x);
        asm volatile("" : "+v"(tid));
        __builtin_assume(tid >= 0 && tid < T);
        if (i == 0) ep_step_r<SG, 0, 1>(in, out, ca.ggsw[i], ca.tw, lds, true, tid, ac);
        else if (i + 1 < ca.n) ep_step_r<SG, 1, 1>(in, out, ca.ggsw[i], ca.tw, lds, false, tid, ac, YSTAMP_STEP(i + 1));
        else ep_step_r<SG, 1, 0>(in, out, ca.ggsw[i], ca.tw, lds, false, tid, ac);
        in = out;
    }
}

struct KsChainArgs {
    KsArgs base;
    GlweRef buf[2];
    const double* key[CHAIN_MAX];
    int ginv[CHAIN_MAX];
    int n;
    const unsigned* pred = nullptr;
    unsigned pred_seq = 0;
    unsigned* host_count = nullptr;
    unsigned* done = nullptr;
    unsigned done_seq = 0;
};
template <int SK>
__global__ __launch_bounds__(T, T / 256) __attribute__((amdgpu_num_vgpr(FK_CHAIN_VGPRS))) void k_pair_z(KsArgs ka) {
    extern __shared__ __attribute__((aligned(16))) double lds[];
    RoMonitor ro_mon(lds, ka.tw);
    static_assert((SK & 1) == 0 || SK == 5, "pairs of output limbs (+ one)");
    constexpr int SX = 3;
    const int tid = vt((int)threadIdx.x);
    const int co = (int)blockIdx.z;
    double* tw = lds;
    double* data = lds + LDS_TW;
    TwRegs twr;
    twiddles_issue(twr, ka.tw, tid);
    const int32_t* ap = at(ka.a);
    const int32_t* bp = at(ka.b);
    int32_t* op = at(ka.out);
    double* mstage = data;
    double* bstage = data + LDS_DATA;
    const int sidx0 = (tid * ka.ginv) & (2 * N - 1);
    const int sstep = (T * ka.ginv) & (2 * N - 1);
    auto load_ab = [&](int col, double (&aa)[E], double (&ab)[E]) {
        RawX<KS_PAIR, SX> rw[E];
#pragma unroll
        for (int k = 0; k < E; k++) load_raw<KS_PAIR, SX>(ka, ap, bp, col, tid + T * k, rw[k]);
        __builtin_amdgcn_sched_barrier(0);
#pragma unroll
        for (int k = 0; k < E; k++) {
            const double va = __builtin_fma(__builtin_fma((double)rw[k].a[0], TWO_B, (double)rw[k].a[1]), TWO_B, (double)rw[k].a[2]);
            aa[k] = rw[k].neg ? -va : va;
            ab[k] = __builtin_fma(__builtin_fma((double)rw[k].b[0], TWO_B, (double)rw[k].b[1]), TWO_B, (double)rw[k].b[2]);
        }
    };
    double u[E];
    {
        double aa[E], ab[E];
        load_ab(1, aa, ab);
#pragma unroll
        for (int k = 0; k < E; k++) {
            mstage[tid + T * k] = __builtin_floor(__builtin_fma(aa[k] - ab[k], 0.5, 0.5));
            if (co == 1) u[k] = window51(__builtin_floor(__builtin_fma(aa[k] + ab[k], 0.5, 0.5)));
        }
        if (co == 0) {
            load_ab(0, aa, ab);
#pragma unroll
            for (int k = 0; k < E; k++) {
                bstage[tid + T * k] = window51(__builtin_floor(__builtin_fma(aa[k] - ab[k], 0.5, 0.5)));
                u[k] = window51(__builtin_floor(__builtin_fma(aa[k] + ab[k], 0.5, 0.5)));
            }
        }
    }
    twiddles_commit(twr, tw, tid);
    double xh[SX][E];
    double od[E], ec[E];
    {
        int sidx = sidx0;
#pragma unroll
        for (int k = 0; k < E; k++) {
            const bool ng = sidx >= N;
            double c = mstage[sidx & (N - 1)];
            const double d2 = take_digit(c);
            const double d1 = take_digit(c);
            const double d0 = cmod17(c);
            xh[2][k] = ng ? -d2 : d2;
            xh[1][k] = ng ? -d1 : d1;
            xh[0][k] = ng ? -d0 : d0;
            double w = 0.0;
            if (co == 0) { const double b = bstage[sidx & (N - 1)]; w = ng ? -b : b; }
            od[k] = w;
            ec[k] = 0.0;
            sidx = (sidx + sstep) & (2 * N - 1);
        }
    }
    OpRegs g[SX];
#pragma unroll
    for (int r = 0; r < SX; r++) load_ops(g[r], ka.key + (long)((r * SK + (SK - 1)) * 2 + co) * N, tid);
    fwd_all<SX>(xh, tw, data, tid);
    auto pair = [&](int j) {
        double acc[2][E];
#pragma unroll
        for (int k = 0; k < E; k++) { acc[0][k] = 0.0; acc[1][k] = 0.0; }
#pragma unroll
        for (int r = 0; r < SX; r++) {
            mac_regs(acc[0], xh[r], g[r]);
            __builtin_amdgcn_sched_barrier(0);
            load_ops(g[r], ka.key + (long)((r * SK + (j - 1)) * 2 + co) * N, tid);
            __builtin_amdgcn_sched_barrier(0);
        }
#pragma unroll
        for (int r = 0; r < SX; r++) mac_regs(acc[1], xh[r], g[r]);
        __builtin_amdgcn_sched_barrier(0);
        ntt_inv2_loop(acc, tw, data, data + LDS_DATA, tid);
        fold_limb<SK>(od, ec, acc[0], j);
        fold_limb<SK>(od, ec, acc[1], j - 1);
        if (j >= 2) {
#pragma unroll
            for (int r = 0; r < SX; r++) load_ops(g[r], ka.key + (long)((r * SK + (j - 2)) * 2 + co) * N, tid);
        }
    };
#pragma unroll 1
    for (int j = SK - 1; j >= 1; j -= 2) pair(j);
    if constexpr (SK & 1) {
        double acc[1][E];
#pragma unroll
        for (int k = 0; k < E; k++) acc[0][k] = 0.0;
#pragma unroll
        for (int r = 0; r < SX; r++) mac_regs(acc[0], xh[r], g[r]);
        ntt_inv1_loop(acc, tw, data, tid);
        fold_limb<SK>(od, ec, acc[0], 0);
    }
#pragma unroll
    for (int k = 0; k < E; k++) {
        double r_ = window51(u[k] - window51(od[k]));
        const double d2 = take_digit(r_);
        const double d1 = take_digit(r_);
        int dst = tid + T * k + ka.t;
        const bool ng = dst >= N;
        if (ng) dst -= N;
        gstore_i32(op + glwe_off(2, co), (unsigned)dst * 4u, cneg((int)d2, ng));
        gstore_i32(op + glwe_off(1, co), (unsigned)dst * 4u, cneg((int)d1, ng));
        gstore_i32(op + glwe_off(0, co), (unsigned)dst * 4u, cneg((int)r_, ng));
    }
}

struct RowChainArgs {
    EpChainArgs ep;
    KsChainArgs ks;
    GlweRef hi, trhi;
    int store_ep = 0;
    GlweRef tree = {nullptr, 0, 0};
    int tree_rho = 0;
};
#define FK_READ_CHAIN_ARGS RowChainArgs
#define FK_READ_CHAIN_TABLE 0
#define FK_KS_CHAIN_NAME k_keyswitch_chain
#define FK_READ_CHAIN_NAME k_read_chain
#define FK_VG FK_CHAIN_VGPRS
#include "chain_kernels.inc"
#undef FK_KS_CHAIN_NAME
#undef FK_READ_CHAIN_NAME
#undef FK_VG
#define FK_KS_CHAIN_NAME k_keyswitch_chain_w
#define FK_READ_CHAIN_NAME k_read_chain_w
#define FK_VG FK_WIDE_VGPRS
#include "chain_kernels.inc"
#undef FK_KS_CHAIN_NAME
#undef FK_READ_CHAIN_NAME
#undef FK_VG
#undef FK_READ_CHAIN_ARGS
#undef FK_READ_CHAIN_TABLE
struct RowChainTableArgs : RowChainArgs {
    long opnd_stride = 0;
    int ws = 1;
    unsigned member_map = 0;
};
static_assert(FHERAM_READ_BATCH_MAX <= 8 && FHERAM_BANK_MAX <= 8 && FHERAM_READ_LIST_MAX <= 8, "the source map holds eight entries of four bits");
static_assert(FHERAM_BANK_MAX <= 16, "a member index fits four bits");
__device__ __forceinline__ long table_opnd_offset(const RowChainTableArgs& ra) {
    int y = (int)blockIdx.y;
    asm volatile("" : "+v"(y));
    return (long)(__builtin_amdgcn_readfirstlane(y) / ra.ws) * ra.opnd_stride;
}
__device__ __forceinline__ GlweRef table_member_row(GlweRef a, const RowChainTableArgs& ra) {
    int y = (int)blockIdx.y;
    asm volatile("" : "+v"(y));
    const int k = __builtin_amdgcn_readfirstlane(y) / ra.ws;
    const int m = (int)((ra.member_map >> (4 * k)) & 15u);
    a.p += (long)((m - k) * ra.ws) * a.sy;
    return a;
}
#define FK_READ_CHAIN_ARGS RowChainTableArgs
#define FK_READ_CHAIN_TABLE 1
#define FK_READ_CHAIN_NAME k_read_chain_t
#define FK_VG FK_WIDE_VGPRS
#include "chain_kernels.inc"
#undef FK_READ_CHAIN_NAME
#ifdef FK_MAPPED_CHAINS
#undef FK_READ_CHAIN_TABLE
#define FK_READ_CHAIN_TABLE 2
#define FK_READ_CHAIN_NAME k_read_chain_m
#include "chain_kernels.inc"
#undef FK_READ_CHAIN_NAME
#endif
#undef FK_VG
#undef FK_READ_CHAIN_ARGS
#undef FK_READ_CHAIN_TABLE

#define FK_WRITE_CHAIN_ARGS RowChainArgs
#define FK_WRITE_CHAIN_TABLE 0
#define FK_WRITE_CHAIN_NAME k_write_chain
#include "write_chain.inc"
#undef FK_WRITE_CHAIN_ARGS
#undef FK_WRITE_CHAIN_TABLE
#undef FK_WRITE_CHAIN_NAME
#define FK_WRITE_CHAIN_ARGS RowChainTableArgs
#define FK_WRITE_CHAIN_TABLE 1
#define FK_WRITE_CHAIN_NAME k_write_chain_t
#include "write_chain.inc"
#ifdef FK_MAPPED_CHAINS
#undef FK_WRITE_CHAIN_TABLE
#undef FK_WRITE_CHAIN_NAME
#define FK_WRITE_CHAIN_TABLE 2
#define FK_WRITE_CHAIN_NAME k_write_chain_m
#include "write_chain.inc"
#endif
#undef FK_WRITE_CHAIN_ARGS
#undef FK_WRITE_CHAIN_TABLE
#undef FK_WRITE_CHAIN_NAME

constexpr int TAIL_GROUPS = 8;
constexpr int GATE_SPIN_MAX = 1 << 13;
#ifndef FK_NO_PLAIN_KERNELS
__global__ __launch_bounds__(64) void k_tail_gate(const unsigned* gate, unsigned seq) {
    if (threadIdx.x != 0) return;
    for (int spin = 0; spin < GATE_SPIN_MAX; spin++) {
        if ((int)(__hip_atomic_load(gate, __ATOMIC_RELAXED, __HIP_MEMORY_SCOPE_AGENT) - seq) >= 0) break;
        __builtin_amdgcn_s_sleep(8);
    }
}
#endif
constexpr int TAIL_SPIN_MAX = 1 << 14;
struct TailArgs {
    GlweRef src, buf[2];
    const double* key[CHAIN_MAX];
    int ginv[CHAIN_MAX];
    const double* tw;
    double* big;
    unsigned* sync;
    unsigned seq;
    int n, n_ct, gx;
    int xoff;
    int give_up_at;
    int n_ep = 0;
    const double* ggsw[4];
    GlweRef ep_out;
};
constexpr int TAIL_EP_MAX = 4;
__device__ __forceinline__ int xcc_id() {
    int v;
    asm volatile("s_getreg_b32 %0, hwreg(HW_REG_XCC_ID)" : "=s"(v));
    return v & 0xf;
}
__device__ __forceinline__ int ld_l2(const int32_t* p) { return __hip_atomic_load(const_cast<int32_t*>(p), __ATOMIC_RELAXED, __HIP_MEMORY_SCOPE_AGENT); }
__device__ __forceinline__ double ld_l2(const double* p) { return __hip_atomic_load(const_cast<double*>(p), __ATOMIC_RELAXED, __HIP_MEMORY_SCOPE_AGENT); }
__device__ __forceinline__ bool tail_barrier(unsigned* ctr, unsigned* abortp, unsigned seq, unsigned want, int* flag, bool check_xcc, int tid) {
    asm volatile("s_waitcnt vmcnt(0)" ::: "memory");
    __syncthreads();
    if (tid == 0) {
        __hip_atomic_fetch_add(ctr, 1u, __ATOMIC_RELAXED, __HIP_MEMORY_SCOPE_AGENT);
        int ok = 0;
        for (int spin = 0; spin < TAIL_SPIN_MAX; spin++) {
            if ((int)(__hip_atomic_load(ctr, __ATOMIC_RELAXED, __HIP_MEMORY_SCOPE_AGENT) - want) >= 0) { ok = 1; break; }
            if ((spin & 15) == 15 && __hip_atomic_load(abortp, __ATOMIC_RELAXED, __HIP_MEMORY_SCOPE_AGENT) == seq) break;
        }
        if (ok && check_xcc) ok = (__builtin_popcount(__hip_atomic_load(ctr + 2, __ATOMIC_RELAXED, __HIP_MEMORY_SCOPE_AGENT)) == 1);
        if (ok && __hip_atomic_load(abortp, __ATOMIC_RELAXED, __HIP_MEMORY_SCOPE_AGENT) == seq) ok = 0;
        if (!ok) __hip_atomic_store(abortp, seq, __ATOMIC_RELAXED, __HIP_MEMORY_SCOPE_AGENT);
        *flag = ok;
    }
    __syncthreads();
    return *flag != 0;
}
__device__ __forceinline__ void tail_arrive(unsigned* ctr, int tid) {
    asm volatile("s_waitcnt vmcnt(0)" ::: "memory");
    __syncthreads();
    if (tid == 0) __hip_atomic_fetch_add(ctr, 1u, __ATOMIC_RELAXED, __HIP_MEMORY_SCOPE_AGENT);
}
__device__ __forceinline__ bool tail_wait(unsigned* ctr, unsigned* abortp, unsigned seq, unsigned want, int* flag, int tid) {
    if (tid == 0) {
        int ok = 0;
        for (int spin = 0; spin < TAIL_SPIN_MAX; spin++) {
            if ((int)(__hip_atomic_load(ctr, __ATOMIC_RELAXED, __HIP_MEMORY_SCOPE_AGENT) - want) >= 0) { ok = 1; break; }
            if ((spin & 15) == 15 && __hip_atomic_load(abortp, __ATOMIC_RELAXED, __HIP_MEMORY_SCOPE_AGENT) == seq) break;
        }
        if (ok && __hip_atomic_load(abortp, __ATOMIC_RELAXED, __HIP_MEMORY_SCOPE_AGENT) == seq) ok = 0;
        if (!ok) __hip_atomic_store(abortp, seq, __ATOMIC_RELAXED, __HIP_MEMORY_SCOPE_AGENT);
        *flag = ok;
    }
    __syncthreads();
    return *flag != 0;
}
__device__ __forceinline__ void ld_l2_pair(const int32_t* p, int& a, int& b) {
    const long long v = __hip_atomic_load(reinterpret_cast<long long*>(const_cast<int32_t*>(p)), __ATOMIC_RELAXED, __HIP_MEMORY_SCOPE_AGENT);
    a = (int)(v & 0xffffffffll);
    b = (int)(v >> 32);
}
#define FK_TAIL_NAME k_trace_tail
#define FK_TAIL_ARGS TailArgs
#define FK_TAIL_TABLE 0
#include "trace_tail.inc"
#undef FK_TAIL_NAME
#undef FK_TAIL_ARGS
#undef FK_TAIL_TABLE
struct TailTableArgs : TailArgs {
    long opnd_stride = 0;
    int ws = 1;
};
#define FK_TAIL_NAME k_trace_tail_t
#define FK_TAIL_ARGS TailTableArgs
#define FK_TAIL_TABLE 1
#include "trace_tail.inc"
#undef FK_TAIL_NAME
#undef FK_TAIL_ARGS
#undef FK_TAIL_TABLE

#ifdef FK_STAMP
__global__ __launch_bounds__(T, T / 256) void k_ntt_probe(const double* __restrict__ tw_g, double* sink) {
    extern __shared__ __attribute__((aligned(16))) double lds[];
    double* tw = lds;
    double* data = lds + LDS_TW;
    const int tid = vt((int)threadIdx.x);
    load_twiddles(tw, tw_g, tid);
    double x[2][E];
#pragma unroll
    for (int k = 0; k < E; k++) { x[0][k] = (double)(tid * 8 + k); x[1][k] = (double)(tid + k); }
    for (int rep = 0; rep < 2; rep++) {
        STAMP(0);
        ntt_inv<2, true>(x, tw, data, tid);
        STAMP(1);
        ntt_fwd<2>(x, tw, data, tid);
        STAMP(2);
#pragma unroll
        for (int k = 0; k < E; k++) { x[0][k] *= 0x1p-11; x[1][k] *= 0x1p-11; }
    }
    double acc = 0;
#pragma unroll
    for (int k = 0; k < E; k++) acc += x[0][k] + x[1][k];
    sink[blockIdx.x * T + tid] = acc;
}
#endif

template <int MODE, int SX, int SK>
__global__ __launch_bounds__(T, T / 256) void k_keyswitch_fine(KsArgs ka) {
    extern __shared__ __attribute__((aligned(16))) double lds[];
    RoMonitor ro_mon(lds, ka.tw);
    double* tw = lds;
    double* data = lds + LDS_TW;
    const int tid = vt((int)threadIdx.x);
    STAMPZ(0);
    TwRegs twr;
    twiddles_issue(twr, ka.tw, tid);
    const int32_t* ap = at(ka.a);
    const int32_t* bp = (MODE == KS_PAIR) ? at(ka.b) : nullptr;
    constexpr int BODY_COL = (MODE == KS_TENSOR) ? 1 : 0;
    constexpr bool PHI = (MODE != KS_TENSOR);
    const int r = (int)blockIdx.z % SX, zz = (int)blockIdx.z / SX;
    const int j = SK - 1 - zz % SK, co = zz / SK;
    OpRegs g;
    load_ops(g, ka.key + (long)((r * SK + j) * 2 + co) * N, tid);
    const int sidx0 = (tid * ka.ginv) & (2 * N - 1);
    const int sstep = (T * ka.ginv) & (2 * N - 1);
    int* mstage = reinterpret_cast<int*>(data);
    const bool adds_body = (r == 0 && co == BODY_COL && j < SX);
    int* bstage = mstage + N;
    int bodyv[E];
    double x[1][E];
    RawX<MODE, SX> rm[E], rb[E];
#pragma unroll
    for (int k = 0; k < E; k++) load_raw<MODE, SX>(ka, ap, bp, 1, tid + T * k, rm[k]);
    if (adds_body) {
#pragma unroll
        for (int k = 0; k < E; k++) load_raw<MODE, SX>(ka, ap, bp, 0, tid + T * k, rb[k]);
    }
    __builtin_amdgcn_sched_barrier(0);
    if constexpr (PHI) {
#pragma unroll
        for (int k = 0; k < E; k++) {
            int xm[SX];
            pre_step<MODE, SX>(rm[k], xm);
            mstage[tid + T * k] = sel_limb(xm, r);
        }
        if (adds_body) {
#pragma unroll
            for (int k = 0; k < E; k++) {
                int xb[SX];
                pre_step<MODE, SX>(rb[k], xb);
                bstage[tid + T * k] = sel_limb(xb, j);
            }
        }
        STAMPZ(1);
        twiddles_commit(twr, tw, tid);
        STAMPZ(2);
        int sidx = sidx0;
#pragma unroll
        for (int k = 0; k < E; k++) {
            x[0][k] = (double)cneg(mstage[sidx & (N - 1)], sidx >= N);
            bodyv[k] = adds_body ? cneg(bstage[sidx & (N - 1)], sidx >= N) : 0;
            sidx = (sidx + sstep) & (2 * N - 1);
        }
    } else {
#pragma unroll
        for (int k = 0; k < E; k++) {
            int xm[SX];
            pre_step<MODE, SX>(rm[k], xm);
            x[0][k] = (double)sel_limb(xm, r);
            bodyv[k] = 0;
            if (adds_body) {
                int xb[SX];
                pre_step<MODE, SX>(rb[k], xb);
                bodyv[k] = sel_limb(xb, j);
            }
        }
        twiddles_commit(twr, tw, tid);
    }
    STAMPZ(3);
    ntt_fwd<1>(x, tw, data, tid);
    STAMPZ(4);
    double acc[1][E];
#pragma unroll
    for (int k = 0; k < E; k++) acc[0][k] = 0.0;
    mac_regs(acc[0], x[0], g);
    STAMPZ(5);
    ntt_inv<1, false>(acc, tw, data, tid);
    STAMPZ(6);
#pragma unroll
    for (int k = 0; k < E; k++) acc[0][k] += (double)bodyv[k];
    double* bgp = ka.big + big_ct() * SX + (long)((co * SK + j) * SX + r) * N;
#pragma unroll
    for (int k = 0; k < E; k++) bgp[tid + T * k] = acc[0][k];
    STAMPZ(7);
}

template <int SA, int SG>
__global__ __launch_bounds__(T, T / 256) void k_ext_product_fine(GlweRef a, const double* __restrict__ ggsw,
                                                                 const double* __restrict__ tw_g, double* __restrict__ big) {
    extern __shared__ __attribute__((aligned(16))) double lds[];
    RoMonitor ro_mon(lds, tw_g);
    double* tw = lds;
    double* data = lds + LDS_TW;
    const int tid = vt((int)threadIdx.x);
    TwRegs twr;
    twiddles_issue(twr, tw_g, tid);
    const int32_t* ap = at(a);
    const int r = (int)blockIdx.z % SA, z1 = (int)blockIdx.z / SA;
    const int cin = z1 % 2, z2 = z1 / 2;
    const int j = SG - 1 - z2 % SG, co = z2 / SG;
    OpRegs g;
    load_ops(g, ggsw + (long)(((2 * r + cin) * SG + j) * 2 + co) * N, tid);
    double x[1][E];
#pragma unroll
    for (int k = 0; k < E; k++) x[0][k] = (double)ap[glwe_off(r, cin) + tid + T * k];
    twiddles_commit(twr, tw, tid);
    ntt_fwd<1>(x, tw, data, tid);
    double acc[1][E];
#pragma unroll
    for (int k = 0; k < E; k++) acc[0][k] = 0.0;
    mac_regs(acc[0], x[0], g);
    ntt_inv<1, false>(acc, tw, data, tid);
    double* bp = big + big_ct() * (2 * SA) + (long)((co * SG + j) * 2 * SA + cin * SA + r) * N;
#pragma unroll
    for (int k = 0; k < E; k++) bp[tid + T * k] = acc[0][k];
}
template <int SA, int SG>
__global__ __launch_bounds__(256) void k_ext_product_fine_norm(GlweRef res, const double* __restrict__ big) {
    constexpr int SLICES = N / 256, NP = 2 * SA;
    const int co = (int)blockIdx.z / SLICES;
    const int i = ((int)blockIdx.z % SLICES) * 256 + (int)threadIdx.x;
    int32_t* rp = at(res);
    const double* bp = big + big_ct() * NP + (long)co * SG * NP * N + i;
    double carry = 0.0;
#pragma unroll
    for (int j = SG - 1; j >= 0; j--) {
        double v = 0.0;
#pragma unroll
        for (int q = 0; q < NP; q++) v += bp[(long)(j * NP + q) * N];
        v += carry;
        const double cy = carry_of(v);
        carry = cy;
        if (j < SA) rp[glwe_off(j, co) + i] = (int)digit_of(v, cy);
    }
}

template <int MODE, int SX, int SK, int SO, int NP = 1>
__global__ __launch_bounds__(256) void k_keyswitch_norm(KsArgs ka) {
    constexpr int SLICES = N / 256;
    const int co = (int)blockIdx.z / SLICES;
    const int i = ((int)blockIdx.z % SLICES) * 256 + (int)threadIdx.x;
    GlweRef ra = ka.a, rb = ka.b, ro = ka.out;
    const int32_t* ap = ra.p + (long)blockIdx.y * ra.sy + (long)blockIdx.x * ra.sx;
    const int32_t* bp = (MODE == KS_PAIR) ? rb.p + (long)blockIdx.y * rb.sy + (long)blockIdx.x * rb.sx : nullptr;
    int32_t* op = ro.p + (long)blockIdx.y * ro.sy + (long)blockIdx.x * ro.sx;
    const double* bgp = ka.big + big_ct() * NP + (long)co * SK * NP * N + i;
    double v_[SK];
#pragma unroll
    for (int j = 0; j < SK; j++) {
        v_[j] = bgp[(long)(j * NP) * N];
#pragma unroll
        for (int q = 1; q < NP; q++) v_[j] += bgp[(long)(j * NP + q) * N];
    }
    int xa[SX];
    if constexpr (MODE == KS_PAIR) load_pair_sum<SX>(ka, ap, bp, co, i, xa);
    else if constexpr (MODE == KS_TRACE || MODE == KS_ADD || MODE == KS_SUBNEG) load_x<MODE, SX>(ka, ap, bp, co, i, xa);
    double carry = 0.0, carry2 = 0.0;
#pragma unroll
    for (int j = SK - 1; j >= 0; j--) {
        double v = v_[j];
        if constexpr (MODE == KS_TRACE || MODE == KS_ADD) { if (j < SX) v += (double)xa[j < SX ? j : 0]; }
        if constexpr (MODE == KS_SUBNEG) v = (j < SX ? (double)xa[j < SX ? j : 0] : 0.0) - v;
        v += carry;
        const double cy = carry_of(v);
        carry = cy;
        if (j < SO) {
            const double d = digit_of(v, cy);
            if constexpr (MODE == KS_PAIR) {
                const double v2 = (double)xa[j < SX ? j : 0] - d + carry2;
                const double cy2 = carry_of(v2);
                carry2 = cy2;
                int dst = i + ka.t;
                const bool ng = dst >= N;
                if (ng) dst -= N;
                op[glwe_off(j, co) + dst] = cneg((int)digit_of(v2, cy2), ng);
            } else {
                op[glwe_off(j, co) + i] = (int)d;
            }
        }
    }
}

template <int S>
__global__ __launch_bounds__(256) void k_sub_add_norm(GlweRef a, GlweRef b, GlweRef c, GlweRef out) {
    const int32_t* ap = at(a);
    const int32_t* bp = at(b);
    const int32_t* cp = at(c);
    int32_t* op = at(out);
    for (int idx = blockIdx.z * blockDim.x + threadIdx.x; idx < 2 * N; idx += blockDim.x * gridDim.z) {
        const int col = idx >> LOGN, i = idx & (N - 1);
        double in_l[S], out_l[S];
#pragma unroll
        for (int j = 0; j < S; j++) {
            const long o = glwe_off(j, col) + i;
            in_l[j] = (double)(ap[o] - bp[o] + cp[o]);
        }
        normalize_coeff<S, S>(in_l, out_l);
#pragma unroll
        for (int j = 0; j < S; j++) op[glwe_off(j, col) + i] = (int)out_l[j];
    }
}
constexpr unsigned MID_POISON = 0x80000000u;
// ... 425 lines not shown
```

### fhe-ram_amd/csrc/launch.hpp

```cpp
#pragma once
#include "ctx.hpp"

namespace {

template <typename F>
void with_evk(const fheram_ctx* c, F&& f) {
    if (c->s_evk == 5) f(std::integral_constant<int, 5>{});
    else f(std::integral_constant<int, 4>{});
}
template <typename F>
void with_evk_wide(fheram_ctx* c, bool wide, F&& f) {
    if (wide) c->wide_unsynced = true;
    with_evk(c, [&](auto sk) { if (wide) f(sk, std::true_type{}); else f(sk, std::false_type{}); });
}
bool capturing(const fheram_ctx* c) { return c->cfg.graph && !c->profile; }

constexpr int LIMB_SPLIT_MAX = 64;
constexpr int EW_SLICES = 8;
int pick_nco(const fheram_ctx* c, int gx, int gy, bool one_wg = false) {
    if (c->cfg.nco != 0) return c->cfg.nco;
    if (one_wg) return 2;
    return ((long)gx * gy * 2 <= c->cus) ? 1 : 2;
}
void launch_prepare(fheram_ctx* c, const int32_t* in, double* out, int npoly, int64_t gal = 0) {
    ProfScope ps(c, "prepare", npoly);
    const int ginv = gal == 0 ? 0 : galois_inv_mod(galois_mod(gal));
    hipLaunchKernelGGL(k_prepare, dim3((npoly + 1) / 2), dim3(T), LDS_PREPARE_BYTES, c->cur, in, out, c->d_tw, c->ninv, ginv, npoly);
}
double* big_of(const fheram_ctx* c) { return c->cur == c->stream2 ? c->d_big2 : c->d_big; }
bool use_limb_split(const fheram_ctx* c, int gx, int gy, int sk) {
    return c->cfg.limb_split && (long)gx * gy <= LIMB_SPLIT_MAX && (long)gx * gy * 2 * sk <= c->cus;
}
bool use_fine_split(const fheram_ctx* c, int gx, int gy, int wgs) {
    return c->cfg.limb_split && c->cfg.fine_split && (long)gx * gy * wgs <= c->cus && (long)gx * gy * wgs * N * 8 <= (long)LIMB_SPLIT_MAX * BIG_STRIDE * 8;
}
void launch_ep(fheram_ctx* c, GlweRef a, GlweRef res, const double* ggsw, int gx, int gy) {
    if (gx <= 0 || gy <= 0) return;
    ProfScope ps(c, "ext_product", (uint64_t)gx * gy);
    if (use_fine_split(c, gx, gy, 2 * 4 * 2 * 3)) {
        hipLaunchKernelGGL((k_ext_product_fine<3, 4>), dim3(gx, gy, 2 * 4 * 2 * 3), dim3(T), LDS_BYTES, c->cur, a, ggsw, c->d_tw, big_of(c));
        hipLaunchKernelGGL((k_ext_product_fine_norm<3, 4>), dim3(gx, gy, 2 * (N / 256)), dim3(256), 0, c->cur, res, big_of(c));
        return;
    }
    if (use_limb_split(c, gx, gy, 4)) {
        hipLaunchKernelGGL((k_ext_product<3, 4, 1, 1>), dim3(gx, gy, 8), dim3(T), LDS_BYTES, c->cur, a, res, ggsw, c->d_tw, big_of(c));
        hipLaunchKernelGGL((k_ext_product<3, 4, 1, 2>), dim3(gx, gy, 2), dim3(T), 0, c->cur, a, res, ggsw, c->d_tw, big_of(c));
        return;
    }
    if (pick_nco(c, gx, gy) == 1) hipLaunchKernelGGL((k_ext_product<3, 4, 1>), dim3(gx, gy, 2), dim3(T), LDS_BYTES, c->cur, a, res, ggsw, c->d_tw, big_of(c));
    else {
        ProfScope pf(c, "ext_product_fused", (uint64_t)gx * gy);
        hipLaunchKernelGGL((k_ext_product<3, 4, 2>), dim3(gx, gy, 1), dim3(T), LDS_BYTES, c->cur, a, res, ggsw, c->d_tw, big_of(c));
    }
}
template <int MODE, int SX, int SK, int SO>
void launch_ks(fheram_ctx* c, const KsArgs& ka, int gx, int gy, bool beside = false) {
    if (gx <= 0 || gy <= 0) return;
    ProfScope ps(c, "keyswitch", (uint64_t)gx * gy);
    if (!beside && use_fine_split(c, gx, gy, 2 * SK * SX)) {
        KsArgs kb = ka;
        kb.big = big_of(c);
        hipLaunchKernelGGL((k_keyswitch_fine<MODE, SX, SK>), dim3(gx, gy, 2 * SK * SX), dim3(T), LDS_BYTES, c->cur, kb);
        hipLaunchKernelGGL((k_keyswitch_norm<MODE, SX, SK, SO, SX>), dim3(gx, gy, 2 * (N / 256)), dim3(256), 0, c->cur, kb);
        return;
    }
    if (!beside && use_limb_split(c, gx, gy, SK)) {
        KsArgs kb = ka;
        kb.big = big_of(c);
        hipLaunchKernelGGL((k_keyswitch<MODE, SX, SK, SO, 1, 1>), dim3(gx, gy, 2 * SK), dim3(T), LDS_BYTES, c->cur, kb);
        hipLaunchKernelGGL((k_keyswitch_norm<MODE, SX, SK, SO>), dim3(gx, gy, 2 * (N / 256)), dim3(256), 0, c->cur, kb);
        return;
    }
    constexpr bool FUSABLE = (SX == 3) && (MODE != KS_PAIR);
    if constexpr (MODE == KS_PAIR && SX == 3 && SO == 3) {
        if (c->cfg.pair_z) {
            hipLaunchKernelGGL((k_pair_z<SK>), dim3(gx, gy, 2), dim3(T), LDS_BYTES, c->cur, ka);
            return;
        }
    }
    if (!FUSABLE || pick_nco(c, gx, gy) == 1) {
        hipLaunchKernelGGL((k_keyswitch<MODE, SX, SK, SO, 1>), dim3(gx, gy, 2), dim3(T), LDS_BYTES, c->cur, ka);
    } else if constexpr (FUSABLE) {
        ProfScope pf(c, "keyswitch_fused", (uint64_t)gx * gy);
        hipLaunchKernelGGL((k_keyswitch<MODE, SX, SK, SO, 2>), dim3(gx, gy, 1), dim3(T), LDS_BYTES, c->cur, ka);
    }
}
void launch_copy(fheram_ctx* c, GlweRef src, GlweRef dst, int gx, int gy) {
    if (gx <= 0 || gy <= 0) return;
    ProfScope ps(c, "elementwise", (uint64_t)gx * gy);
    hipLaunchKernelGGL((k_copy<3>), dim3(gx, gy, EW_SLICES), dim3(256), 0, c->cur, src, dst);
}
KsArgs ks_args(fheram_ctx* c, GlweRef a, GlweRef b, GlweRef out, const double* key, int64_t gal, int t = 0, int rot_mul = 0, int rot_base = 0) {
    KsArgs ka;
    ka.a = a; ka.b = b; ka.out = out; ka.key = key; ka.tw = c->d_tw;
    ka.g = galois_mod(gal); ka.ginv = galois_inv_mod(ka.g); ka.t = t; ka.rot_mul = rot_mul; ka.rot_base = rot_base; ka.big = c->d_big;
    return ka;
}
const double* trace_key(fheram_ctx* c, int i) { return c->d_atk + (size_t)i * c->atk; }
template <int MODE>
void launch_ks_tr(fheram_ctx* c, const KsArgs& ka, int gx, int gy) {
    with_evk(c, [&](auto sk) { launch_ks<MODE, 3, decltype(sk)::value, 3>(c, ka, gx, gy); });
}
bool same(const GlweRef& a, const GlweRef& b) { return a.p == b.p; }

template <typename F>
void run_chain(fheram_ctx* c, int n, GlweRef src, GlweRef dst, GlweRef tmp, int gx, int gy, F&& step) {
    if (n <= 0) { if (!same(src, dst)) launch_copy(c, src, dst, gx, gy); return; }
    if (same(src, dst) && (n % 2 == 1)) {
        run_chain(c, n, src, tmp, dst, gx, gy, step);
        launch_copy(c, tmp, dst, gx, gy);
        return;
    }
    GlweRef cur = src;
    for (int i = 0; i < n; i++) {
        GlweRef out = ((n - 1 - i) % 2 == 0) ? dst : tmp;
        step(i, cur, out);
        cur = out;
    }
}
enum class ChainForm { Tail, Mid, Chain, Steps };
struct ChainPlan {
    ChainForm form;
    int split;
};
struct ChainQuery {
    bool ep;
    int n, gx, gy;
    bool rotated = false;
    bool one_wg = false;
    bool handoff = true;
};
ChainPlan chain_form(const fheram_ctx* c, const ChainQuery& q) {
    const long batch = (long)q.gx * q.gy;
    const int sk = q.ep ? 4 : c->s_evk;
    const bool len = q.n >= 2 && q.n <= CHAIN_MAX;
    const bool handoff = q.handoff && len && c->cfg.limb_split &&
                         c->cus >= TAIL_GROUPS * 32 &&
                         !capturing(c);
    if (handoff && !q.ep && !q.rotated && c->cfg.tail && c->cfg.fine_split && batch <= TAIL_GROUPS &&
        c->cur == c->stream &&
        2 * sk * 3 <= 32)
        return {ChainForm::Tail, 0};
    if (handoff && c->cfg.mid && batch > TAIL_GROUPS) {
        if (batch <= 16) return {ChainForm::Mid, 1};
        if (!q.ep && c->cfg.mid >= 2) {
            if (batch <= 8 * (32 / (2 * sk))) return {ChainForm::Mid, 2};
            if (batch <= 8 * (32 / sk)) return {ChainForm::Mid, 3};
        }
    }
    if (len && c->cfg.chain && pick_nco(c, q.gx, q.gy, q.one_wg) == 2 && !use_limb_split(c, q.gx, q.gy, sk) &&
        !use_fine_split(c, q.gx, q.gy, q.ep ? 2 * 4 * 2 * 3 : 2 * sk * 3))
        return {ChainForm::Chain, 0};
    return {ChainForm::Steps, 0};
}
bool chain_bufs(int n, GlweRef src, GlweRef dst, GlweRef tmp, GlweRef (&b)[2]) {
    if (n % 2 == 1) { if (same(src, dst)) return false; b[0] = dst; b[1] = tmp; }
    else { b[0] = tmp; b[1] = dst; }
    return !same(b[0], src);
}
ChainPlan plan_chain(const fheram_ctx* c, ChainQuery q, GlweRef src, GlweRef dst, GlweRef tmp, GlweRef (&b)[2], bool& fits) {
    fits = chain_bufs(q.n, src, dst, tmp, b);
    ChainPlan p = chain_form(c, q);
    if ((p.form == ChainForm::Tail && !(fits && !same(b[1], src))) || (p.form == ChainForm::Mid && !fits)) {
        q.handoff = false;
        p = chain_form(c, q);
    }
    return p;
}
void mid_rearm(fheram_ctx* c) {
    if (!c->cfg.mid && c->mid_saved && ++c->mid_off_ops >= 256) { c->cfg.mid = c->mid_saved; c->mid_saved = 0; c->mid_bad_windows = 0; c->mid_off_ops = 0; }
}
template <bool EP>
void fill_mid(fheram_ctx* c, MidArgs& ma, GlweRef src, GlweRef dst, int n, int gx, int gy) {
    const int side = c->cur == c->stream2 ? 1 : 0;
    ma.src = src; ma.dst = dst; ma.tw = c->d_tw; ma.big = c->d_mid_big[side]; ma.sync = c->d_mid_sync[side]; ma.y = c->d_mid_y[side];
    if (++c->mid_seq == 0) ++c->mid_seq;
    c->mid_launches++;
    c->mid_window_cts += (uint64_t)(gx * gy);
    if (!c->cfg.mid_test && c->mid_launches - c->mid_launch_mark >= 64) {
        const unsigned fb = __atomic_load_n(c->h_mid_fb, __ATOMIC_RELAXED) + __atomic_load_n(c->h_mid_fb + 16, __ATOMIC_RELAXED);
        const unsigned redone = fb - c->mid_fb_mark;
        const bool bad = (uint64_t)redone * 4u > c->mid_window_cts;
        c->mid_bad_windows = bad ? c->mid_bad_windows + 1 : 0;
        if (c->cfg.mid && c->mid_bad_windows >= 2) { c->mid_saved = c->cfg.mid; c->cfg.mid = 0; c->mid_disabled_count++; }
        c->mid_fb_mark = fb;
        c->mid_launch_mark = c->mid_launches;
        c->mid_window_cts = 0;
    }
    ma.seq = c->mid_seq; ma.n = n; ma.n_ct = gx * gy; ma.gx = gx; ma.rot_mul = 0; ma.rot_base = 0;
    ma.give_up_at = c->cfg.mid_test ? n - 2 : -1;
}
template <int SK, int RS, int LPM>
void launch_k_mid_trace(fheram_ctx* c, const MidArgs& ma) {
    constexpr int members = RS * 2 * SK / LPM;
    hipLaunchKernelGGL((k_chain_mid<false, SK, RS, LPM>), dim3(8 * (32 / members) * members), dim3(T), LDS_BYTES, c->cur, ma);
}
void launch_mid_trace(fheram_ctx* c, GlweRef src, const GlweRef (&b)[2], int start, int n, int gx, int gy, int rot_mul, int rot_base, int split) {
    ProfScope ps(c, "keyswitch", (uint64_t)gx * gy, n);
    ProfScope pm(c, "keyswitch_mid_launch", (uint64_t)gx * gy * n, 1);
    MidArgs ma;
    fill_mid<false>(c, ma, src, b[(n - 1) & 1], n, gx, gy);
    ma.rot_mul = rot_mul; ma.rot_base = rot_base;
    KsChainArgs ca;
    ca.base = ks_args(c, src, src, b[0], trace_key(c, start), c->gal[start], 0, rot_mul, rot_base);
    ca.buf[0] = b[0]; ca.buf[1] = b[1]; ca.n = n;
    ca.done = ma.sync; ca.done_seq = ma.seq; ca.host_count = c->h_mid_fb + (c->cur == c->stream2 ? 16 : 0);
    for (int i = 0; i < n; i++) { ma.opnd[i] = ca.key[i] = trace_key(c, start + i); ma.ginv[i] = ca.ginv[i] = galois_inv_mod(galois_mod(c->gal[start + i])); }
    with_evk(c, [&](auto sk) {
        constexpr int SK = decltype(sk)::value;
        if (split == 1) launch_k_mid_trace<SK, 3, 2>(c, ma); else if (split == 2) launch_k_mid_trace<SK, 1, 1>(c, ma); else launch_k_mid_trace<SK, 1, 2>(c, ma);
        hipLaunchKernelGGL((k_keyswitch_chain<3, SK, 3>), dim3(gx, gy, 1), dim3(T), LDS_BYTES, c->cur, ca);
    });
}
void launch_mid_ep(fheram_ctx* c, GlweRef src, const GlweRef (&b)[2], const double* prep, int d, int gx, int gy) {
    ProfScope ps(c, "ext_product", (uint64_t)gx * gy, d);
    ProfScope pm(c, "ext_product_mid_launch", (uint64_t)gx * gy * d, 1);
    MidArgs ma;
    fill_mid<true>(c, ma, src, b[(d - 1) & 1], d, gx, gy);
    EpChainArgs ca;
    ca.src = src; ca.buf[0] = b[0]; ca.buf[1] = b[1]; ca.tw = c->d_tw; ca.n = d;
    ca.done = ma.sync; ca.done_seq = ma.seq; ca.host_count = c->h_mid_fb + (c->cur == c->stream2 ? 16 : 0);
    for (int i = 0; i < d; i++) { ma.opnd[i] = ca.ggsw[i] = prep + (size_t)i * fheram_ctx::GGSW; ma.ginv[i] = 1; }
    hipLaunchKernelGGL((k_chain_mid<true, 4, 3, 2>), dim3(8 * 2 * 12), dim3(T), LDS_BYTES, c->cur, ma);
    hipLaunchKernelGGL((k_ext_product_chain<3, 4>), dim3(gx, gy, 1), dim3(T), LDS_BYTES, c->cur, ca);
}
void launch_ep_chain(fheram_ctx* c, GlweRef src, const GlweRef (&b)[2], const double* prep, int d, int gx, int gy) {
    ProfScope ps(c, "ext_product", (uint64_t)gx * gy, d);
    ProfScope pf(c, "ext_product_fused", (uint64_t)gx * gy, d);
    EpChainArgs ca;
    ca.src = src; ca.buf[0] = b[0]; ca.buf[1] = b[1]; ca.tw = c->d_tw; ca.n = d;
    for (int i = 0; i < d; i++) ca.ggsw[i] = prep + (size_t)i * fheram_ctx::GGSW;
    if (d >= 2) hipLaunchKernelGGL((k_ext_product_chain_r<4>), dim3(gx, gy, 1), dim3(T), LDS_BYTES, c->cur, ca);
    else hipLaunchKernelGGL((k_ext_product_chain<3, 4>), dim3(gx, gy, 1), dim3(T), LDS_BYTES, c->cur, ca);
}
void ep_chain(fheram_ctx* c, GlweRef src, GlweRef dst, GlweRef tmp, const double* prep, int d, int gx, int gy) {
    if (gx <= 0 || gy <= 0) return;
    GlweRef b[2];
    bool fits;
    switch (plan_chain(c, ChainQuery{true, d, gx, gy}, src, dst, tmp, b, fits).form) {
    case ChainForm::Mid: launch_mid_ep(c, src, b, prep, d, gx, gy); return;
    case ChainForm::Chain:
        if (!fits && !chain_bufs(d, src, tmp, dst, b)) break;
        launch_ep_chain(c, src, b, prep, d, gx, gy);
        if (!fits) launch_copy(c, tmp, dst, gx, gy);
        return;
    default: break;
    }
    run_chain(c, d, src, dst, tmp, gx, gy, [&](int i, GlweRef in, GlweRef out) { launch_ep(c, in, out, prep + (size_t)i * fheram_ctx::GGSW, gx, gy); });
}
void launch_trace_chain(fheram_ctx* c, GlweRef src, const GlweRef (&b)[2], int start, int n, int gx, int gy, int rot_mul, int rot_base) {
    ProfScope ps(c, "keyswitch", (uint64_t)gx * gy, n);
    ProfScope pf(c, "keyswitch_fused", (uint64_t)gx * gy, n);
    ProfScope pl(c, "keyswitch_chain_launch", (uint64_t)gx * gy * n, 1);
    KsChainArgs ca;
    ca.base = ks_args(c, src, src, b[0], trace_key(c, start), c->gal[start], 0, rot_mul, rot_base);
    ca.buf[0] = b[0]; ca.buf[1] = b[1]; ca.n = n;
    for (int i = 0; i < n; i++) { ca.key[i] = trace_key(c, start + i); ca.ginv[i] = galois_inv_mod(galois_mod(c->gal[start + i])); }
    const int yf = n >= 2 ? c->cfg.chain_y : 0;
    with_evk_wide(c, yf && c->wide, [&](auto sk, auto w) {
        constexpr int SK = decltype(sk)::value;
        if (!yf) hipLaunchKernelGGL((k_keyswitch_chain<3, SK, 3>), dim3(gx, gy, 1), dim3(T), LDS_BYTES, c->cur, ca);
        else if constexpr (decltype(w)::value) hipLaunchKernelGGL((k_keyswitch_chain_w<3, SK, 3, 3>), dim3(gx, gy, 1), dim3(T), LDS_BYTES, c->cur, ca);
        else hipLaunchKernelGGL((k_keyswitch_chain<3, SK, 3, 3>), dim3(gx, gy, 1), dim3(T), LDS_BYTES, c->cur, ca);
    });
}
struct OpndTable { int ws = 0; long stride = 0; unsigned member_map = 0; bool store_mapped = false; };
constexpr unsigned MEMBER_MAP_IDENTITY = 0x76543210u;
bool map_is_identity(unsigned map, int n) { for (int k = 0; k < n; k++) if (((map >> (4 * k)) & 15u) != (unsigned)k) return false; return true; }
bool use_row_fuse(const fheram_ctx* c, int d, int n_tr, int gx, int gy, bool one_wg = false) {
    return c->cfg.fuse && c->cfg.chain_y == 3 && !capturing(c) &&
           chain_form(c, ChainQuery{true, d, gx, gy, false, one_wg}).form == ChainForm::Chain &&
           chain_form(c, ChainQuery{false, n_tr, gx, gy, false, one_wg}).form == ChainForm::Chain;
}
RowChainTableArgs with_table(const RowChainArgs& ra, const OpndTable& t) {
    RowChainTableArgs rt;
    static_cast<RowChainArgs&>(rt) = ra;
    rt.opnd_stride = t.stride; rt.ws = t.ws; rt.member_map = t.member_map;
    return rt;
}
void fill_row_chain(fheram_ctx* c, RowChainArgs& ra, const double* prep, int d, int start, int n_tr) {
    ra.ep.tw = c->d_tw; ra.ep.n = d;
    for (int i = 0; i < d; i++) ra.ep.ggsw[i] = prep + (size_t)i * fheram_ctx::GGSW;
    ra.ks.n = n_tr;
    for (int i = 0; i < n_tr; i++) { ra.ks.key[i] = trace_key(c, start + i); ra.ks.ginv[i] = galois_inv_mod(galois_mod(c->gal[start + i])); }
}
void launch_read_chain(fheram_ctx* c, GlweRef src, const GlweRef* ep_store, GlweRef dst, const double* prep, int d, int n_tr, int gx, int gy, const OpndTable& t) {
    ProfScope ps(c, "read_chain_launch", (uint64_t)gx * gy, 1);
    RowChainArgs ra;
    fill_row_chain(c, ra, prep, d, 0, n_tr);
    ra.ep.src = src;
    ra.ep.buf[0] = ra.ep.buf[1] = ep_store ? *ep_store : dst;
    ra.store_ep = ep_store ? 1 : 0;
    ra.ks.base = ks_args(c, dst, dst, dst, trace_key(c, 0), c->gal[0]);
    ra.ks.buf[0] = ra.ks.buf[1] = dst;
    ra.hi = dst; ra.trhi = dst;
    if (t.ws > 0) {
        c->wide_unsynced = true;
        if (ep_store && t.store_mapped) {
            read_chain_m_launch(c->s_evk, dim3(gx, gy, 1), c->cur, with_table(ra, t));
            return;
        }
        with_evk(c, [&](auto sk) {
            constexpr int SK = decltype(sk)::value;
            hipLaunchKernelGGL((k_read_chain_t<SK, 4>), dim3(gx, gy, 1), dim3(T), LDS_BYTES, c->cur, with_table(ra, t));
        });
        return;
    }
    with_evk_wide(c, c->wide, [&](auto sk, auto w) {
        constexpr int SK = decltype(sk)::value;
        if constexpr (decltype(w)::value) hipLaunchKernelGGL((k_read_chain_w<SK, 4>), dim3(gx, gy, 1), dim3(T), LDS_BYTES, c->cur, ra);
        else hipLaunchKernelGGL((k_read_chain<SK, 4>), dim3(gx, gy, 1), dim3(T), LDS_BYTES, c->cur, ra);
    });
}
void launch_write_chain(fheram_ctx* c, GlweRef src, int rot_mul, int rot_base, GlweRef data, GlweRef trhi, const double* prep, int d, int n_tr, int gx, int gy, const OpndTable& t,
                        const GlweRef* tree = nullptr, int tree_rho = 0) {
    ProfScope ps(c, "write_chain_launch", (uint64_t)gx * gy, 1);
    RowChainArgs ra;
    fill_row_chain(c, ra, prep, d, 0, n_tr);
    ra.ks.base = ks_args(c, src, src, data, trace_key(c, 0), c->gal[0], 0, rot_mul, rot_base);
    ra.ks.buf[0] = ra.ks.buf[1] = data;
    ra.hi = data; ra.trhi = trhi;
    ra.ep.src = data; ra.ep.buf[0] = ra.ep.buf[1] = data;
    if (tree) { ra.tree = *tree; ra.tree_rho = tree_rho; }
    c->wide_unsynced = true;
    if (t.ws > 0 && t.store_mapped) {
        write_chain_m_launch(c->s_evk, dim3(gx, gy, 1), c->cur, with_table(ra, t));
        return;
    }
    with_evk(c, [&](auto sk) {
        constexpr int SK = decltype(sk)::value;
        if (t.ws > 0) hipLaunchKernelGGL((k_write_chain_t<SK, 4>), dim3(gx, gy, 1), dim3(T), LDS_BYTES, c->cur, with_table(ra, t));
        else hipLaunchKernelGGL((k_write_chain<SK, 4>), dim3(gx, gy, 1), dim3(T), LDS_BYTES, c->cur, ra);
    });
}
void launch_trace_tail(fheram_ctx* c, GlweRef src, const GlweRef (&b)[2], int start, int n, int gx, int gy,
                       const double* prep = nullptr, int d = 0, GlweRef ep_out = GlweRef{nullptr, 0, 0}, bool store_ep = false, const OpndTable& t = {}) {
    ProfScope ps(c, "keyswitch", (uint64_t)gx * gy, n);
    ProfScope pt(c, "keyswitch_tail_launch", (uint64_t)gx * gy * n, 1);
    TailArgs ta;
    ta.src = src; ta.buf[0] = b[0]; ta.buf[1] = b[1]; ta.tw = c->d_tw; ta.big = big_of(c); ta.sync = c->d_tail_sync;
    ta.n_ep = prep ? d : 0; ta.ep_out = ep_out;
    for (int i = 0; i < TAIL_EP_MAX; i++) ta.ggsw[i] = (prep && i < d) ? prep + (size_t)i * fheram_ctx::GGSW : nullptr;
    if (++c->tail_seq == 0) ++c->tail_seq;
    c->tail_launches++;
    if (c->cfg.tail_test != 1 && c->tail_launches - c->tail_launch_mark >= 64) {
        const unsigned fb = *(volatile unsigned*)c->h_tail_fb;
        if (fb - c->tail_fb_mark > 16) c->cfg.tail = 0;
        c->tail_fb_mark = fb;
        c->tail_launch_mark = c->tail_launches;
    }
    ta.seq = c->tail_seq; ta.n = n; ta.n_ct = gx * gy; ta.gx = gx; ta.xoff = c->tail_xoff; ta.give_up_at = c->cfg.tail_test ? ta.n_ep + n - 2 : -1;
    KsChainArgs ca;
    ca.base = ks_args(c, src, src, b[0], trace_key(c, start), c->gal[start], 0, 0, 0);
    ca.buf[0] = b[0]; ca.buf[1] = b[1]; ca.n = n;
    ca.pred = c->d_tail_sync + TAIL_GROUPS * 32; ca.pred_seq = ta.seq; ca.host_count = c->h_tail_fb;
    for (int i = 0; i < n; i++) { ta.key[i] = ca.key[i] = trace_key(c, start + i); ta.ginv[i] = ca.ginv[i] = galois_inv_mod(galois_mod(c->gal[start + i])); }
    RowChainArgs ra;
    if (ta.n_ep) {
        fill_row_chain(c, ra, prep, d, start, n);
        ra.ep.src = src; ra.ep.buf[0] = ra.ep.buf[1] = ep_out; ra.store_ep = store_ep ? 1 : 0;
        ra.ks.base = ks_args(c, b[(n - 1) & 1], b[(n - 1) & 1], b[(n - 1) & 1], trace_key(c, start), c->gal[start]);
        ra.ks.buf[0] = ra.ks.buf[1] = b[(n - 1) & 1];
        ra.hi = ra.trhi = b[(n - 1) & 1];
        ra.ks.pred = ca.pred; ra.ks.pred_seq = ca.pred_seq; ra.ks.host_count = ca.host_count;
    }
    with_evk(c, [&](auto sk) {
        constexpr int SK = decltype(sk)::value;
        const dim3 groups(TAIL_GROUPS * 2 * SK * 3);
        if (t.ws > 0 && ta.n_ep) {
            TailTableArgs tt;
            static_cast<TailArgs&>(tt) = ta;
            tt.opnd_stride = t.stride; tt.ws = t.ws;
            hipLaunchKernelGGL((k_trace_tail_t<3, SK, 3>), groups, dim3(T), LDS_BYTES, c->cur, tt);
            c->wide_unsynced = true;
            hipLaunchKernelGGL((k_read_chain_t<SK, 4>), dim3(gx, gy, 1), dim3(T), LDS_BYTES, c->cur, with_table(ra, OpndTable{t.ws, t.stride, MEMBER_MAP_IDENTITY}));
            return;
        }
        hipLaunchKernelGGL((k_trace_tail<3, SK, 3>), groups, dim3(T), LDS_BYTES, c->cur, ta);
        if (ta.n_ep) hipLaunchKernelGGL((k_read_chain<SK, 4>), dim3(gx, gy, 1), dim3(T), LDS_BYTES, c->cur, ra);
        else hipLaunchKernelGGL((k_keyswitch_chain<3, SK, 3>), dim3(gx, gy, 1), dim3(T), LDS_BYTES, c->cur, ca);
    });
}
void trace_steps(fheram_ctx* c, GlweRef src, GlweRef dst, GlweRef tmp, int start, int end, int gx, int gy, int rot_mul = 0, int rot_base = 0) {
    if (gx <= 0 || gy <= 0) return;
    const int n = end - start;
    GlweRef b[2];
    bool fits;
    const ChainPlan p = plan_chain(c, ChainQuery{false, n, gx, gy, rot_mul != 0 || rot_base != 0}, src, dst, tmp, b, fits);
    switch (p.form) {
    case ChainForm::Tail: launch_trace_tail(c, src, b, start, n, gx, gy); return;
    case ChainForm::Mid: launch_mid_trace(c, src, b, start, n, gx, gy, rot_mul, rot_base, p.split); return;
    case ChainForm::Chain:
        if (!fits && !chain_bufs(n, src, tmp, dst, b)) break;
        launch_trace_chain(c, src, b, start, n, gx, gy, rot_mul, rot_base);
        if (!fits) launch_copy(c, tmp, dst, gx, gy);
        return;
    case ChainForm::Steps: break;
    }
    run_chain(c, n, src, dst, tmp, gx, gy, [&](int i, GlweRef in, GlweRef out) {
        KsArgs ka = ks_args(c, in, in, out, trace_key(c, start + i), c->gal[start + i], 0, i == 0 ? rot_mul : 0, i == 0 ? rot_base : 0);
        launch_ks_tr<KS_TRACE>(c, ka, gx, gy);
    });
}
int32_t* pack_levels(fheram_ctx* c, int32_t* src, int32_t* A, int32_t* B, long sy, long sx, size_t count, int gy,
                     int n_alone, int first_pair, bool keep_alone = false, int32_t* P0 = nullptr, int32_t* P1 = nullptr) {
    const int k = ilog2_ceil(count);
    int32_t* cur = src;
    auto other = [&](int32_t* x) { return x == A ? B : A; };
    if (n_alone > 0 && count > 0) {
        int32_t* b0 = other(src);
        int32_t* b1 = other(b0);
        if (b1 == src && P0 && P0 != src && chain_form(c, ChainQuery{false, n_alone, (int)count, gy}).form == ChainForm::Tail) b1 = P0;
        cur = keep_alone ? A : ((n_alone - 1) & 1) ? b1 : b0;
        trace_steps(c, ref(src, sy, sx), ref(cur, sy, sx), ref(cur == b0 ? b1 : b0, sy, sx), 0, n_alone, (int)count, gy);
    }
    size_t live = count;
    for (int m = 0; m < k; m++) {
        const int i = first_pair + m;
        const long h = (long)1 << (k - 1 - m);
        int32_t* nxt = (keep_alone && P0) ? (cur == P0 ? P1 : P0) : other(cur);
        const long n_pair = std::max<long>(0, std::min<long>(h, (long)live - h));
        const long n_alone_here = std::min<long>(h, (long)live) - n_pair;
        if (n_pair > 0) {
            KsArgs ka = ks_args(c, ref(cur, sy, sx), ref(cur + h * sx, sy, sx), ref(nxt, sy, sx), trace_key(c, i), c->gal[i], N >> (i + 1));
            launch_ks_tr<KS_PAIR>(c, ka, (int)n_pair, gy);
        }
        if (n_alone_here > 0) {
            KsArgs ka = ks_args(c, ref(cur + n_pair * sx, sy, sx), ref(cur, sy, sx), ref(nxt + n_pair * sx, sy, sx), trace_key(c, i), c->gal[i]);
            launch_ks_tr<KS_TRACE>(c, ka, (int)n_alone_here, gy);
        }
        live = std::min<size_t>(live, (size_t)h);
        cur = nxt;
    }
    return cur;
}
int coord_first_digit(const fheram_ctx* c, int ci) { int s = 0; for (int i = 0; i < ci; i++) s += (int)c->base2d[i].size(); return s; }
double* digits_of(const fheram_ctx* c, double* table, int ci) { return table + (size_t)coord_first_digit(c, ci) * fheram_ctx::GGSW; }
void coordinate_prepare(fheram_ctx* c, const fheram_addr* addr, int ci, double* table) {
    const int d = (int)c->base2d[ci].size();
    launch_prepare(c, addr->d_ggsw + (size_t)coord_first_digit(c, ci) * fheram_ctx::GGSW, digits_of(c, table, ci), d * (int)(fheram_ctx::GGSW / N));
}
void coordinate_prepare_all(fheram_ctx* c, const fheram_addr* addr, double* table) {
    launch_prepare(c, addr->d_ggsw, table, c->n_digits * (int)(fheram_ctx::GGSW / N));
}
void ggsw_inverse(fheram_ctx* c, const int32_t* in, int32_t* tmp, int d, bool beside = false) {
    const long g4 = (long)fheram_ctx::GLWE4;
    int32_t* inp = const_cast<int32_t*>(in);
    KsArgs ka = ks_args(c, ref(inp, (long)fheram_ctx::GGSW, 2 * g4), ref(inp, 0, 0), ref(tmp, (long)fheram_ctx::GGSW, 2 * g4), c->d_atk_inv, -1);
    launch_ks<KS_AUTO, 4, 5, 4>(c, ka, fheram_ctx::DNUM_CT, d, beside);
    KsArgs kt = ks_args(c, ref(tmp, (long)fheram_ctx::GGSW, 2 * g4), ref(tmp, 0, 0), ref(tmp + g4, (long)fheram_ctx::GGSW, 2 * g4), c->d_tsk, 1);
    launch_ks<KS_TENSOR, 4, 5, 4>(c, kt, fheram_ctx::DNUM_CT, d, beside);
}
void coordinate_prepare_inv(fheram_ctx* c, const fheram_addr* addr, int ci, int32_t* tmp, double* prep, bool beside = false) {
    const int d = (int)c->base2d[ci].size();
    ggsw_inverse(c, addr->d_ggsw + (size_t)coord_first_digit(c, ci) * fheram_ctx::GGSW, tmp, d, beside);
    launch_prepare(c, tmp, prep, d * (int)(fheram_ctx::GGSW / N));
}

void precompute_inverse(fheram_ctx* c, const fheram_addr* addr, int ci, bool fork, unsigned gate_seq = 0) {
    if (fork && c->wdone_pending) {
        hipStreamWaitEvent(c->stream2, c->ev_wdone, 0);
        c->wdone_pending = false;
    }
    if (fork && gate_seq) {
        if (c->opstart_valid) { hipStreamWaitEvent(c->stream2, c->ev_opstart, 0); c->opstart_valid = false; }
        hipLaunchKernelGGL(k_tail_gate, dim3(1), dim3(64), 0, c->stream2, c->d_tail_sync + TAIL_GROUPS * 32 + 2, gate_seq);
    } else if (fork) {
        hipEventRecord(c->ev_fork, c->stream);
        hipStreamWaitEvent(c->stream2, c->ev_fork, 0);
    }
    hipStream_t keep = c->cur;
    c->cur = c->stream2;
    coordinate_prepare_inv(c, addr, ci, c->d_ggsw_inv + (size_t)coord_first_digit(c, ci) * fheram_ctx::GGSW, digits_of(c, c->d_prep_inv, ci), true);
    hipEventRecord(c->ev_inv[ci], c->stream2);
    c->cur = keep;
    c->inv_id[ci] = addr->id;
    c->inv_pending[ci] = true;
}
void wait_inverse(fheram_ctx* c, hipStream_t s, int ci) { if (!capturing(c)) hipStreamWaitEvent(s, c->ev_inv[ci], 0); }

}
```

### fhe-ram_amd/csrc/path.hpp

```cpp
#pragma once
#include "launch.hpp"

namespace {

struct Opnds {
    fheram_ctx* c;
    RamState* st;
    const fheram_addr* const* addrs;
    int n, ws;
    double *tab, *tab_inv;
    long stride;
    unsigned member_map;
    bool bank;
    int member(int k) const { return (int)((member_map >> (4 * k)) & 15u); }
    bool rows_dense() const { return map_is_identity(member_map, n); }
    int Y() const { return n * ws; }
    double* prep(int k, int ci) const { return digits_of(c, tab + k * stride, ci); }
    double* inv(int k, int ci) const { return digits_of(c, tab_inv + k * stride, ci); }
    GlweRef slice(GlweRef r, int k) const { r.p += (long)k * ws * r.sy; return r; }
    GlweRef rows(GlweRef r, int k) const { return slice(r, member(k)); }
    OpndTable table() const { return n == 1 ? OpndTable{} : OpndTable{ws, stride, member_map, !rows_dense()}; }
    bool row_fuse(int d, int n_tr, int gx) const { return use_row_fuse(c, d, n_tr, gx, Y(), bank); }
};
Opnds one_addr(fheram_ctx* c, const fheram_addr* const* a, int ws, RamState* st) { return Opnds{c, st, a, 1, ws, c->d_prep, c->d_prep_inv, 0, 0, false}; }
Opnds one_addr(fheram_ctx* c, const fheram_addr* const* a) { return one_addr(c, a, c->ws, &c->ram); }
Opnds table_opnds(fheram_ctx* c, RamState* st, const fheram_addr* const* addrs, int n, int ws, double* tab, double* tab_inv, unsigned member_map, bool bank) {
    return Opnds{c, st, addrs, n, ws, tab, tab_inv, (long)c->n_digits * (long)fheram_ctx::GGSW, member_map, bank};
}

struct RamView {
    int32_t *rows, *A, *B, *C, *D;
    int32_t *part, *tmp, *tmp2, *res, *tree, *w, *trtop;
};
RamView ctx_view(const fheram_ctx* c) {
    return RamView{c->d_data, c->d_scrA, c->d_scrB, c->d_scrC, c->d_scrD, c->d_part, c->d_tmp, c->d_tmp2, c->d_res, c->d_tree, c->d_w, c->d_trtop};
}

void read_local_done(const fheram_ctx* c, RamState* st, bool prepare_write) {
    if (c->n2 == 2) st->memo_alone = (prepare_write && c->cfg.memo) ? LOGN - ilog2_ceil(c->rows_glob) : 0;
}
void read_top_done(fheram_ctx* c, RamState* st, bool prepare_write) {
    st->memo_top = prepare_write && c->cfg.memo;
    st->res_in_trtop = st->memo_top;
    c->prep1_ready = false;
}
void write_done(fheram_ctx* c, RamState* st) { st->memo_top = false; st->memo_alone = 0; c->side_begun = false; c->tree_rotate_pending = false; }

template <typename F>
int run_op(fheram_ctx* c, const fheram_addr* addr, int which, F&& enqueue) {
    if (!capturing(c)) return enqueue();
    main_enqueued(c);
    fheram_addr* a = const_cast<fheram_addr*>(addr);
    const unsigned sig = 1u | (c->ram.memo_top ? 2u : 0u) | ((unsigned)c->ram.memo_alone << 2) | (c->side_begun ? 64u : 0u) |
                         (c->inv_id[0] == addr->id ? 128u : 0u) | (c->inv_id[1] == addr->id ? 256u : 0u);
    if (a->graph[which] && a->graph_sig[which] != sig) { hipGraphExecDestroy(a->graph[which]); a->graph[which] = nullptr; }
    if (!a->graph[which]) {
        hipGraph_t g = nullptr;
        HIPCHK(c, hipStreamBeginCapture(c->stream, hipStreamCaptureModeThreadLocal));
        const int rc = enqueue();
        const hipError_t e = hipStreamEndCapture(c->stream, &g);
        if (rc != FHERAM_OK || e != hipSuccess) {
            if (g) hipGraphDestroy(g);
            return rc != FHERAM_OK ? rc : fail(c, FHERAM_ERR_DEVICE, std::string("hipStreamEndCapture: ") + hipGetErrorString(e));
        }
        const hipError_t e2 = hipGraphInstantiate(&a->graph[which], g, nullptr, nullptr, 0);
        hipGraphDestroy(g);
        if (e2 != hipSuccess) { a->graph[which] = nullptr; return fail(c, FHERAM_ERR_DEVICE, std::string("hipGraphInstantiate: ") + hipGetErrorString(e2)); }
        a->graph_sig[which] = sig;
    }
    HIPCHK(c, hipGraphLaunch(a->graph[which], c->stream));
    if (which == 2) write_done(c, &c->ram);
    else { read_local_done(c, &c->ram, which == 1); read_top_done(c, &c->ram, which == 1); }
    return FHERAM_OK;
}

int check_common(fheram_ctx* c, const fheram_addr* addr) {
    if (!c) return FHERAM_ERR_INVALID_ARG;
    mid_rearm(c);
    if (!addr || addr->ctx != c) return fail(c, FHERAM_ERR_INVALID_ARG, "address does not belong to this context (layout mismatch, ram.rs:404)");
    if (addr->empty) return fail(c, FHERAM_ERR_INVALID_ARG, "empty address: fheram_address_alloc without fheram_address_derive");
    if (!c->ram.initialized) return fail(c, FHERAM_ERR_UNINITIALIZED, "unitialized memory: self.data.len()=0");
    if (!c->keys_loaded) return fail(c, FHERAM_ERR_KEYS, "evaluation keys not loaded");
    return FHERAM_OK;
}

int read_local(const Opnds& o, const RamView& a, bool prepare_write, GlweRef* packed_out, bool to_part) {
    fheram_ctx* c = o.c;
    const int n = o.n, ws = o.ws, Y = o.Y(), R = (int)c->rows;
    main_enqueued(c);
    c->wide = !prepare_write || n > 1;
    if (n == 1 && prepare_write && c->cfg.pre_inv == 1 && !capturing(c) && (c->wide_unsynced || c->derive_unsynced)) {
        hipEventRecord(c->ev_opstart, c->stream);
        c->opstart_valid = true;
    }
    const long G = (long)fheram_ctx::GLWE;
    const long sy = (long)c->rows * G;
    GlweRef data = ref(a.rows, sy, G), A = ref(a.A, sy, G), B = ref(a.B, sy, G);
    GlweRef part = ref(a.part, G, 0);
    const bool all = (c->n_shards == 1 && c->n2 == 2);
    for (int k = 0; k < n; k++)
        if (all) coordinate_prepare_all(c, o.addrs[k], o.tab + k * o.stride); else coordinate_prepare(c, o.addrs[k], 0, o.tab + k * o.stride);
    c->prep1_ready = all;
    read_local_done(c, o.st, prepare_write);
    const int d0 = (int)c->base2d[0].size();
    if (c->n2 == 1) {
        GlweRef row0 = ref(a.rows, sy, 0);
        for (int k = 0; k < n; k++)
            if (prepare_write) ep_chain(c, o.rows(row0, k), o.rows(row0, k), o.slice(ref(a.A, sy, 0), k), o.prep(k, 0), d0, 1, ws);
            else ep_chain(c, o.rows(row0, k), o.slice(part, k), o.slice(ref(a.tmp, G, 0), k), o.prep(k, 0), d0, 1, ws);
        const bool gather = prepare_write && !o.rows_dense();
        if (gather) for (int k = 0; k < n; k++) launch_copy(c, o.rows(row0, k), o.slice(part, k), 1, ws);
        *packed_out = (prepare_write && !gather) ? row0 : part;
        if (prepare_write && to_part && !gather) launch_copy(c, row0, part, 1, Y);
        return FHERAM_OK;
    }
    const int L0 = LOGN - ilog2_ceil(c->rows_glob);
    const bool keep = o.st->memo_alone > 0;
    int32_t* packed;
    if (o.row_fuse(d0, L0, R) && !(prepare_write && (d0 & 1))) {
        launch_read_chain(c, data, prepare_write ? &data : nullptr, A, o.prep(0, 0), d0, L0, R, Y, o.table());
        packed = pack_levels(c, a.A, a.A, a.B, sy, G, (size_t)R, Y, 0, L0, keep, a.C, a.D);
    } else {
        for (int k = 0; k < n; k++)
            if (prepare_write) ep_chain(c, o.rows(data, k), o.rows(data, k), o.slice(A, k), o.prep(k, 0), d0, R, ws);
            else ep_chain(c, o.rows(data, k), o.slice(A, k), o.slice(B, k), o.prep(k, 0), d0, R, ws);
        int32_t* leaves = prepare_write ? a.rows : a.A;
        if (prepare_write && !o.rows_dense()) {
            for (int k = 0; k < n; k++) launch_copy(c, o.rows(data, k), o.slice(ref(a.D, sy, G), k), R, ws);
            leaves = a.D;
        }
        packed = pack_levels(c, leaves, a.A, a.B, sy, G, (size_t)R, Y, L0, L0, keep, a.C, a.D);
    }
    *packed_out = ref(packed, sy, 0);
    if (to_part) launch_copy(c, *packed_out, part, 1, Y);
    return FHERAM_OK;
}
int read_top(const Opnds& o, const RamView& a, bool prepare_write, int32_t* gathered, GlweRef pk) {
    fheram_ctx* c = o.c;
    const int n = o.n, ws = o.ws, Y = o.Y();
    main_enqueued(c);
    c->wide = !prepare_write || n > 1;
    const long G = (long)fheram_ctx::GLWE;
    GlweRef tmp = ref(a.tmp, G, 0);
    GlweRef last = pk;
    const int d1 = c->n2 == 2 ? (int)c->base2d[1].size() : 0;
    auto tail_top = [&] { return chain_form(c, ChainQuery{false, LOGN, 1, Y}).form == ChainForm::Tail; };
    const bool fuse_ep = c->n2 == 2 && c->cfg.tail_ep && d1 >= 2 && d1 <= TAIL_EP_MAX && tail_top();
    GlweRef ep_out = ref(prepare_write ? a.tree : a.tmp2, G, 0);
    auto products1 = [&] { for (int k = 0; k < n; k++) ep_chain(c, o.slice(pk, k), o.slice(ep_out, k), o.slice(tmp, k), o.prep(k, 1), d1, 1, ws); };
    if (c->n2 == 2) {
        if (gathered) {
            const int kG = ilog2_ceil((size_t)c->n_shards);
            int32_t* a0 = c->d_gat[1];
            int32_t* a1 = c->d_gat[2];
            int32_t* packed = pack_levels(c, gathered, a0, a1, G, (long)ws * G, (size_t)c->n_shards, ws, 0, LOGN - kG);
            pk = ref(packed, G, 0);
        }
        if (!c->prep1_ready) coordinate_prepare(c, o.addrs[0], 1, o.tab);
        if (!fuse_ep) products1();
        last = ep_out;
    }
    const bool pre = n == 1 && prepare_write && c->cfg.pre_inv && (long)c->rows * Y <= c->cus;
    const bool gated = pre && c->cfg.pre_inv == 1 && !capturing(c) && tail_top();
    if (pre && !gated)
        for (int ci = c->n2 - 1; ci >= 0; ci--) precompute_inverse(c, o.addrs[0], ci, ci == c->n2 - 1);
    read_top_done(c, o.st, prepare_write);
    const GlweRef res = ref(o.st->memo_top ? a.trtop : a.res, G, 0);
    const uint64_t tl0 = c->tail_launches;
    GlweRef tb[2];
    if (fuse_ep && chain_bufs(LOGN, last, res, tmp, tb))
        launch_trace_tail(c, pk, tb, 0, LOGN, 1, Y, o.prep(0, 1), d1, ep_out, prepare_write, o.table());
    else {
        if (fuse_ep) products1();
        trace_steps(c, last, res, tmp, 0, LOGN, 1, Y);
    }
    if (gated && !c->opstart_valid && (c->wide_unsynced || c->derive_unsynced)) {
        hipEventRecord(c->ev_opstart, c->stream);
        c->opstart_valid = true;
    }
    if (gated) {
        const unsigned seq = c->tail_launches != tl0 ? c->tail_seq : 0;
        for (int ci = c->n2 - 1; ci >= 0; ci--) precompute_inverse(c, o.addrs[0], ci, ci == c->n2 - 1, seq);
    }
    return FHERAM_OK;
}
int read_impl(const Opnds& o, const RamView& a, bool prepare_write) {
    fheram_ctx* c = o.c;
    GlweRef packed;
    int rc = read_local(o, a, prepare_write, &packed, false);
    if (rc != FHERAM_OK) return rc;
    rc = read_top(o, a, prepare_write, nullptr, packed);
    if (o.n == 1 && prepare_write && c->inv_id[0] == o.addrs[0]->id && capturing(c))
        for (int ci = 0; ci < c->n2; ci++) hipStreamWaitEvent(c->stream, c->ev_inv[ci], 0);
    if (rc == FHERAM_OK && prepare_write) o.st->state = true;
    return rc;
}

void dense_free(DenseBufs& L) {
    void* bufs[] = {L.A, L.B, L.C, L.D, L.part, L.tmp, L.tmp2, L.res, L.tree, L.w, L.trtop, L.prep};
    for (void* p : bufs) if (p) hipFree(p);
    if (L.h_res) hipHostFree(L.h_res);
    L = DenseBufs{};
}
bool third_arena_needed(const fheram_ctx* c, int n_ct) {
    return c->n2 == 2 && chain_form(c, ChainQuery{false, LOGN - ilog2_ceil(c->rows_glob), (int)c->rows, n_ct}).form == ChainForm::Tail;
}
int dense_reserve(fheram_ctx* c, DenseBufs& L, int n, int ws, bool all = false, int* fail_alloc = nullptr) {
    const bool work = all || n > 1, third = all || (work && third_arena_needed(c, n * ws));
    if (n <= L.cap && (!work || L.A) && (!third || L.C)) return FHERAM_OK;
    if (n < L.cap) n = L.cap;
    const bool with_work = work || L.A, with_third = third || L.C;
    if (L.cap) {
        HIPCHK(c, hipStreamSynchronize(c->stream));
        if (all) HIPCHK(c, hipStreamSynchronize(c->stream2));
        dense_free(L);
    }
    const size_t ct = (size_t)n * ws * fheram_ctx::GLWE * sizeof(int32_t), row = ct * c->rows;
    hipError_t e = hipSuccess;
    auto dev = [&](auto** p, size_t bytes) {
        if (e != hipSuccess) return;
        if (fail_alloc && *fail_alloc > 0 && --*fail_alloc == 0) e = hipErrorOutOfMemory;
        else e = hipMalloc((void**)p, bytes);
    };
    if (all) {
        for (int32_t** p : {&L.A, &L.B, &L.C, &L.D}) dev(p, row);
        for (int32_t** p : {&L.part, &L.tmp, &L.tmp2, &L.res, &L.tree, &L.w, &L.trtop}) dev(p, ct);
    } else {
        dev(&L.res, ct);
        if (with_work) {
            for (int32_t** p : {&L.A, &L.B}) dev(p, row);
            if (with_third) dev(&L.C, row);
            for (int32_t** p : {&L.tmp, &L.tmp2}) dev(p, ct);
            dev(&L.prep, (size_t)n * c->n_digits * fheram_ctx::GGSW * sizeof(double));
        }
        if (e == hipSuccess) e = hipHostMalloc((void**)&L.h_res, ct * 2 + sizeof(int64_t), hipHostMallocMapped);
        if (e == hipSuccess) e = hipHostGetDevicePointer((void**)&L.d_h_res, L.h_res, 0);
    }
    if (e != hipSuccess) {
        dense_free(L);
        (void)hipGetLastError();
        return fail(c, FHERAM_ERR_DEVICE, (all ? "buffers of a write list of " + std::to_string(n) + " members: " : "read buffers for " + std::to_string(n) + " addresses: ") + hipGetErrorString(e));
    }
    L.cap = n;
    return FHERAM_OK;
}
RamView dense_view(const fheram_ctx* c, const DenseBufs& L) {
    return RamView{c->d_data, L.A, L.B, L.C, L.D, L.part ? L.part : L.tmp2, L.tmp, L.tmp2, L.res, L.tree, L.w, L.trtop};
}

struct SelectBufs {
    int cap = 0, prep_cap = 0, host_cap = 0;
    int32_t *packed = nullptr, *ep = nullptr, *tmp = nullptr, *tmp2 = nullptr, *res = nullptr;
    double* prep = nullptr;
    int64_t *h_res = nullptr, *d_h_res = nullptr;
    int32_t *d_host = nullptr, *h_host = nullptr;
    hipEvent_t ev_host = nullptr;
    bool host_busy = false;
};
void select_free(SelectBufs& S) {
    void* bufs[] = {S.packed, S.ep, S.tmp, S.tmp2, S.res, S.prep, S.d_host};
    for (void* p : bufs) if (p) hipFree(p);
    if (S.h_res) hipHostFree(S.h_res);
    if (S.h_host) hipHostFree(S.h_host);
    if (S.ev_host) hipEventDestroy(S.ev_host);
    S = SelectBufs{};
}

struct ResRun { const int32_t* src; size_t n; };
int result_export(fheram_ctx* c, const ResRun* runs, int n_runs, int64_t* h, int64_t* d_h, int64_t* out) {
    size_t n = 0;
    for (int i = 0; i < n_runs; i++) {
        const int n4 = (int)(runs[i].n / 4);
        hipLaunchKernelGGL(k_export_i64, dim3((n4 + 255) / 256), dim3(256), 0, c->stream, runs[i].src, reinterpret_cast<long long*>(d_h + n), n4,
                           reinterpret_cast<const long long*>(c->d_tw + N));
        n += runs[i].n;
    }
    HIPCHK(c, hipStreamSynchronize(c->stream));
    HIPCHK(c, hipGetLastError());
    main_waited(c);
    double m;
    std::memcpy(&m, h + n, 8);
    if (c->cfg.monitor && m > MON_LIMIT) __atomic_store_n(c->h_ro_flag, 1u, __ATOMIC_RELAXED);
    const int rc = check_precision(c);
    if (rc == FHERAM_OK && out) std::memcpy(out, h, n * sizeof(int64_t));
    return rc;
}

int reads_export(fheram_ctx* c, const DenseBufs& L, size_t first, size_t n_ct, int64_t* out) {
    const ResRun run{L.res + first * fheram_ctx::GLWE, n_ct * fheram_ctx::GLWE};
    return result_export(c, &run, 1, L.h_res, L.d_h_res, out);
}
template <typename F>
int read_many(fheram_ctx* c, DenseBufs& L, RamState* st, const fheram_addr* const* addrs, int n, int ws, unsigned member_map, bool bank, int64_t* out, F&& kept) {
    int rc = dense_reserve(c, L, n, ws);
    if (rc != FHERAM_OK) return rc;
    const Opnds o = table_opnds(c, st, addrs, n, ws, L.prep, nullptr, member_map, bank);
    rc = read_impl(o, dense_view(c, L), false);
    if (rc != FHERAM_OK) return rc;
    kept(o);
    HIPCHK(c, hipGetLastError());
    return out ? reads_export(c, L, 0, (size_t)n * ws, out) : FHERAM_OK;
}

int write_top(const Opnds& o, const RamView& v) {
    fheram_ctx* c = o.c;
    main_enqueued(c);
    c->wide = true;
    const long G = (long)fheram_ctx::GLWE;
    const long sy = (long)c->rows * G;
    const int n = o.n, ws = o.ws, Y = o.Y();
    GlweRef wref = ref(v.w, G, 0), tmp = ref(v.tmp, G, 0), tmp2 = ref(v.tmp2, G, 0), tree = ref(v.tree, G, 0);
    GlweRef top = (c->n2 != 1) ? tree : ref(v.rows, sy, 0);
    GlweRef tr = tmp;
    const bool by_member = c->n2 == 1 && !o.rows_dense();
    if (o.st->memo_top) tr = ref(v.trtop, G, 0);
    else if (by_member) for (int k = 0; k < n; k++) trace_steps(c, o.rows(top, k), o.slice(tmp, k), o.slice(tmp2, k), 0, LOGN, 1, ws);
    else trace_steps(c, top, tmp, tmp2, 0, LOGN, 1, Y);
    if (by_member) {
        ProfScope ps(c, "elementwise", Y);
        for (int k = 0; k < n; k++)
            hipLaunchKernelGGL((k_sub_add_norm<3>), dim3(1, ws, EW_SLICES), dim3(256), 0, c->cur, o.rows(top, k), o.slice(tr, k), o.slice(wref, k), o.rows(top, k));
    } else {
        ProfScope ps(c, "elementwise", Y);
        hipLaunchKernelGGL((k_sub_add_norm<3>), dim3(1, Y, EW_SLICES), dim3(256), 0, c->cur, top, tr, wref, top);
    }
    o.st->memo_top = false;
    if (c->n2 == 2) {
        if (n == 1 && c->inv_id[1] == o.addrs[0]->id) wait_inverse(c, c->stream, 1);
        else {
            if (n == 1 && c->inv_pending[1]) wait_inverse(c, c->stream, 1);
            for (int k = 0; k < n; k++) coordinate_prepare_inv(c, o.addrs[k], 1, c->d_ggsw_tmp, o.inv(k, 1));
        }
        if (n == 1) { c->inv_pending[1] = false; c->inv_id[1] = 0; }
        for (int k = 0; k < n; k++)
            ep_chain(c, o.slice(tree, k), o.slice(ref(v.part, G, 0), k), o.slice(tmp, k), o.inv(k, 1), (int)c->base2d[1].size(), 1, ws);
        c->tree_rotate_pending = true;
    }
    return FHERAM_OK;
}
void write_side_begin(const Opnds& o, const RamView& v) {
    fheram_ctx* c = o.c;
    c->wide = true;
    const long G = (long)fheram_ctx::GLWE;
    const long sy = (long)c->rows * G;
    if (!(c->main_idle && !capturing(c) && c->n_shards == 1)) {
        hipEventRecord(c->ev_fork, c->stream);
        hipStreamWaitEvent(c->stream2, c->ev_fork, 0);
    }
    main_enqueued(c);
    c->cur = c->stream2;
    if (c->n2 == 2) {
        const int kept = o.st->memo_alone;
        c->trhi_in_C = kept > 0 && (LOGN - kept) % 2 == 1;
        if (kept > 0) trace_steps(c, ref(v.A, sy, G), ref(c->trhi_in_C ? v.C : v.A, sy, G), ref(c->trhi_in_C ? v.A : v.C, sy, G), kept, LOGN, (int)c->rows, o.Y());
        else if (!o.rows_dense())
            for (int k = 0; k < o.n; k++) trace_steps(c, o.rows(ref(v.rows, sy, G), k), o.slice(ref(v.A, sy, G), k), o.slice(ref(v.C, sy, G), k), 0, LOGN, (int)c->rows, o.ws);
        else trace_steps(c, ref(v.rows, sy, G), ref(v.A, sy, G), ref(v.C, sy, G), 0, LOGN, (int)c->rows, o.Y());
        o.st->memo_alone = 0;
    }
    if (o.n == 1 && c->inv_id[0] == o.addrs[0]->id) wait_inverse(c, c->stream2, 0);
    else for (int k = 0; k < o.n; k++) coordinate_prepare_inv(c, o.addrs[k], 0, c->d_ggsw_tmp2, o.inv(k, 0));
    if (o.n == 1) { c->inv_id[0] = 0; c->inv_pending[0] = false; }
    hipEventRecord(c->ev_join, c->stream2);
    c->cur = c->stream;
    c->side_begun = true;
}
void write_side_abort(fheram_ctx* c) {
    if (!c->side_begun) return;
    hipStreamWaitEvent(c->stream, c->ev_join, 0);
    c->side_begun = false;
}
int write_rows(const Opnds& o, const RamView& v) {
    fheram_ctx* c = o.c;
    main_enqueued(c);
    c->wide = true;
    const long G = (long)fheram_ctx::GLWE;
    const long sy = (long)c->rows * G;
    const int n = o.n, ws = o.ws, Y = o.Y(), R = (int)c->rows;
    GlweRef data = ref(v.rows, sy, G), A = ref(v.A, sy, G), B = ref(v.B, sy, G), D = ref(v.D, sy, G);
    GlweRef trhi = ref(c->trhi_in_C ? v.C : v.A, sy, G), part = ref(v.part, G, 0);
    const int d0 = (int)c->base2d[0].size();
    const bool fuse = c->n2 == 2 && o.row_fuse(d0, LOGN, R);
    const bool rot_in_chain = fuse && c->tree_rotate_pending && c->n_shards == 1;
    const GlweRef tree = ref(v.tree, G, 0);
    if (fuse) {
        hipStreamWaitEvent(c->stream, c->ev_join, 0);
        launch_write_chain(c, part, c->n_shards, c->shard, data, trhi, o.inv(0, 0), d0, LOGN, R, Y, o.table(), rot_in_chain ? &tree : nullptr, -(int)c->rows_glob);
    } else if (c->n2 == 2)
        trace_steps(c, part, B, D, 0, LOGN, R, Y, c->n_shards, c->shard);
    if (c->tree_rotate_pending && !rot_in_chain) {
        ProfScope ps(c, "elementwise", Y);
        hipLaunchKernelGGL((k_rotate<3>), dim3(1, Y, EW_SLICES), dim3(256), 0, c->cur, part, ref(v.tree, G, 0), -(int)c->rows_glob);
    }
    if (!fuse) {
        hipStreamWaitEvent(c->stream, c->ev_join, 0);
        if (c->n2 == 2) {
            ProfScope ps(c, "elementwise", (uint64_t)R * Y);
            if (o.rows_dense()) hipLaunchKernelGGL((k_sub_add_norm<3>), dim3(R, Y, EW_SLICES), dim3(256), 0, c->cur, data, trhi, B, data);
            else for (int k = 0; k < n; k++)
                hipLaunchKernelGGL((k_sub_add_norm<3>), dim3(R, ws, EW_SLICES), dim3(256), 0, c->cur, o.rows(data, k), o.slice(trhi, k), o.slice(B, k), o.rows(data, k));
        }
        for (int k = 0; k < n; k++) ep_chain(c, o.rows(data, k), o.rows(data, k), o.slice(A, k), o.inv(k, 0), d0, R, ws);
    }
    if (n == 1 && !capturing(c)) { hipEventRecord(c->ev_wdone, c->stream); c->wdone_pending = true; }
    write_done(c, o.st);
    o.st->state = false;
    return FHERAM_OK;
}

template <typename S>
int write_all(const Opnds& o, const RamView& v, S&& stage) {
    write_side_begin(o, v);
    int rc = stage(v.w, o.Y());
    if (rc != FHERAM_OK) { write_side_abort(o.c); return rc; }
    rc = write_top(o, v);
    return rc == FHERAM_OK ? write_rows(o, v) : rc;
}

}
```

### fhe-ram_amd/csrc/trace_tail.inc

```
template <int SX, int SK, int SO>
__global__ __launch_bounds__(T, T / 256) void FK_TAIL_NAME(FK_TAIL_ARGS ta) {
    extern __shared__ __attribute__((aligned(16))) double lds[];
    constexpr int G = 2 * SK * SX;
    constexpr int SG = 4, GE = 2 * SG * SX;
    static_assert(GE <= G && SX == 3 && SO == 3, "the products' members are a subset of the trace steps'");
    const int g = ((int)blockIdx.x + TAIL_GROUPS - ta.xoff) % TAIL_GROUPS, m = (int)blockIdx.x / TAIL_GROUPS;
    if (blockIdx.x == gridDim.x - 1 && threadIdx.x == 0)
        __hip_atomic_store(ta.sync + TAIL_GROUPS * 32 + 2, ta.seq, __ATOMIC_RELAXED, __HIP_MEMORY_SCOPE_AGENT);
    if (g >= ta.n_ct) return;
    RoMonitor ro_mon(lds, ta.tw);
    const int tid = vt((int)threadIdx.x);
    double* tw = lds;
    double* data = lds + LDS_TW;
    int* mstage = reinterpret_cast<int*>(data);
    int* flag = reinterpret_cast<int*>(data + 2 * LDS_DATA);
    unsigned* ctr = ta.sync + g * 32;
    unsigned* abortp = ta.sync + TAIL_GROUPS * 32;
    const int r = m % SX, zz = m / SX;
    const int j = SK - 1 - zz % SK, co = zz / SK;
    const int je = SG - 1 - zz % SG, coe = zz / SG;
    const bool ep_member = m < GE;
    const long ct = (long)(g / ta.gx);
    const long cx = (long)(g % ta.gx);
#if FK_TAIL_TABLE
    const long oset = (ct / ta.ws) * ta.opnd_stride;
#define FK_TAIL_OPND(i) (ta.ggsw[i] + oset)
#else
#define FK_TAIL_OPND(i) ta.ggsw[i]
#endif
    double* const big0 = ta.big + (long)g * BIG_STRIDE * SX;
    const int n_ep = ta.n_ep, n_all = ta.n_ep + ta.n;
    OpRegs kop, kop1;
    if (n_ep > 0) {
        if (ep_member) {
            load_ops(kop, FK_TAIL_OPND(0) + (long)(((2 * r) * SG + je) * 2 + coe) * N, tid);
            load_ops(kop1, FK_TAIL_OPND(0) + (long)(((2 * r + 1) * SG + je) * 2 + coe) * N, tid);
        }
    } else {
        load_ops(kop, ta.key[0] + (long)((r * SK + j) * 2 + co) * N, tid);
    }
    if (tid == 0) {
        __hip_atomic_fetch_or(ctr + 2, 1u << xcc_id(), __ATOMIC_RELAXED, __HIP_MEMORY_SCOPE_AGENT);
        asm volatile("s_waitcnt vmcnt(0)" ::: "memory");
    }
    load_twiddles(tw, ta.tw, tid);
    unsigned epoch = 0;
    auto out_of = [&](int s_) -> GlweRef { return s_ < n_ep ? (s_ == n_ep - 1 ? ta.ep_out : ta.buf[s_ & 1]) : ta.buf[(s_ - n_ep) & 1]; };
#pragma unroll 1
    for (int s = 0; s < n_all; s++) {
        const GlweRef rin = (s == 0) ? ta.src : out_of(s - 1);
        const GlweRef rout = out_of(s);
        const int32_t* ap = rin.p + ct * rin.sy + cx * rin.sx;
        int32_t* op = rout.p + ct * rout.sy + cx * rout.sx;
        const bool is_ep = s < n_ep;
        const int t = s - n_ep;
        const int ginv = is_ep ? 1 : ta.ginv[t];
        const bool stepped = (t > 0);
        const bool fresh = (s == 0);
        const bool last = (s + 1 == n_all);
        double* const bigg = big0 + (long)(s & 1) * TAIL_GROUPS * BIG_STRIDE * SX;
        TSTAMP(0);
        if (is_ep) {
            if (ep_member) {
                double x[2][E];
                if (fresh) {
#pragma unroll
                    for (int c2 = 0; c2 < 2; c2++)
#pragma unroll
                        for (int k = 0; k < E; k++) x[c2][k] = (double)gload_i32(ap + glwe_off(r, c2), (unsigned)(tid + T * k) * 4u);
                } else {
#pragma unroll
                    for (int c2 = 0; c2 < 2; c2++)
#pragma unroll
                        for (int k = 0; k < E; k++) x[c2][k] = (double)ld_l2(ap + glwe_off(r, c2) + tid + T * k);
                }
                ntt_fwd<2>(x, tw, data, tid);
                double acc[1][E];
#pragma unroll
                for (int k = 0; k < E; k++) acc[0][k] = 0.0;
                mac_regs(acc[0], x[0], kop);
                mac_regs(acc[0], x[1], kop1);
                if (s + 1 < n_ep) {
                    load_ops(kop, FK_TAIL_OPND(s + 1) + (long)(((2 * r) * SG + je) * 2 + coe) * N, tid);
                    load_ops(kop1, FK_TAIL_OPND(s + 1) + (long)(((2 * r + 1) * SG + je) * 2 + coe) * N, tid);
                }
                ntt_inv<1, false>(acc, tw, data, tid);
                double* bgp = bigg + (long)((coe * SG + je) * SX + r) * N;
#pragma unroll
                for (int k = 0; k < E; k++) bgp[tid + T * k] = acc[0][k];
            }
            if (s + 1 == n_ep && !last) load_ops(kop, ta.key[0] + (long)((r * SK + j) * 2 + co) * N, tid);
        } else {
        if (stepped) {
            int v[E];
#pragma unroll
            for (int q = 0; q < E / 2; q++) ld_l2_pair(ap + glwe_off(r, 1) + E * tid + 2 * q, v[2 * q], v[2 * q + 1]);
#pragma unroll
            for (int k = 0; k < E; k++) mstage[E * tid + k] = v[k];
        } else {
            int rm[SX][E];
            if (fresh) {
#pragma unroll
                for (int q = 0; q < SX; q++)
#pragma unroll
                    for (int h = 0; h < E / 4; h++) {
                        const int4 v4 = *reinterpret_cast<const int4*>(ap + glwe_off(q, 1) + E * tid + 4 * h);
                        rm[q][4 * h] = v4.x; rm[q][4 * h + 1] = v4.y; rm[q][4 * h + 2] = v4.z; rm[q][4 * h + 3] = v4.w;
                    }
            } else {
#pragma unroll
                for (int q = 0; q < SX; q++)
#pragma unroll
                    for (int h = 0; h < E / 2; h++) ld_l2_pair(ap + glwe_off(q, 1) + E * tid + 2 * h, rm[q][2 * h], rm[q][2 * h + 1]);
            }
#pragma unroll
            for (int k = 0; k < E; k++) {
                int xi[SX], xm[SX];
#pragma unroll
                for (int q = 0; q < SX; q++) xi[q] = rm[q][k];
                rsh1_coeff<SX>(xi, xm);
                mstage[E * tid + k] = sel_limb(xm, r);
            }
        }
        __syncthreads();
        TSTAMP(1);
        double x[1][E];
        {
            int sidx = (tid * ginv) & (2 * N - 1);
            const int sstep = (T * ginv) & (2 * N - 1);
#pragma unroll
            for (int k = 0; k < E; k++) {
                x[0][k] = (double)cneg(mstage[sidx & (N - 1)], sidx >= N);
                sidx = (sidx + sstep) & (2 * N - 1);
            }
        }
        ntt_fwd<1>(x, tw, data, tid);
        TSTAMP(2);
        double acc[1][E];
#pragma unroll
        for (int k = 0; k < E; k++) acc[0][k] = 0.0;
        mac_regs(acc[0], x[0], kop);
        if (!last) load_ops(kop, ta.key[t + 1] + (long)((r * SK + j) * 2 + co) * N, tid);
        ntt_inv<1, false>(acc, tw, data, tid);
        TSTAMP(3);
        {
            double* bgp = bigg + (long)((co * SK + j) * SX + r) * N;
#pragma unroll
            for (int k = 0; k < E; k++) bgp[tid + T * k] = acc[0][k];
        }
        }
        if (ta.give_up_at == s && g == 0 && m == 5) {
            if (tid == 0) __hip_atomic_store(abortp, ta.seq, __ATOMIC_RELAXED, __HIP_MEMORY_SCOPE_AGENT);
            break;
        }
        TSTAMP(4);
        if (!tail_barrier(ctr, abortp, ta.seq, (++epoch) * G, flag, s == 0, tid)) break;
        TSTAMP(5);
        constexpr int CH = (N + G - 1) / G;
        static_assert(CH <= T, "one coefficient per thread and column");
        auto norm_share = [&](const int nco) {
            const int i = m * CH + tid;
            if (tid < CH && i < N) {
                const double* bgp = bigg + (long)nco * SK * SX * N + i;
                double v_[SK];
#pragma unroll
                for (int q = 0; q < SK; q++) {
                    v_[q] = ld_l2(bgp + (long)(q * SX) * N);
#pragma unroll
                    for (int w = 1; w < SX; w++) v_[q] += ld_l2(bgp + (long)(q * SX + w) * N);
                }
                int raw[SX], xa[SX];
#pragma unroll
                for (int q = 0; q < SX; q++) raw[q] = ld_l2(ap + glwe_off(q, nco) + i);
                const int si = (i * ginv) & (2 * N - 1);
                int braw[SX], xb[SX];
#pragma unroll
                for (int q = 0; q < SX; q++) braw[q] = (nco == 0) ? ld_l2(ap + glwe_off(q, 0) + (si & (N - 1))) : 0;
                if (stepped) {
#pragma unroll
                    for (int q = 0; q < SX; q++) { xa[q] = raw[q]; xb[q] = braw[q]; }
                } else {
                    rsh1_coeff<SX>(raw, xa);
                    rsh1_coeff<SX>(braw, xb);
                }
                double carry = 0.0;
                int d[SO], y[SO];
#pragma unroll
                for (int q = SK - 1; q >= 0; q--) {
                    double v = v_[q];
                    if (q < SX) v += (double)xa[q < SX ? q : 0] + (double)cneg(xb[q < SX ? q : 0], si >= N);
                    v += carry;
                    const double cy = carry_of(v);
                    carry = cy;
                    if (q < SO) d[q < SO ? q : 0] = (int)digit_of(v, cy);
                }
                if (last) {
#pragma unroll
                    for (int q = 0; q < SO; q++) y[q] = d[q];
                } else {
                    rsh1_coeff<SO>(d, y);
                }
#pragma unroll
                for (int q = 0; q < SO; q++) op[glwe_off(q, nco) + i] = y[q];
            }
        };
        auto norm_share_ep = [&](const int nco) {
            const int i = m * CH + tid;
            if (tid < CH && i < N) {
                const double* bgp = bigg + (long)nco * SG * SX * N + i;
                double v_[SG];
#pragma unroll
                for (int q = 0; q < SG; q++) {
                    v_[q] = ld_l2(bgp + (long)(q * SX) * N);
#pragma unroll
                    for (int w = 1; w < SX; w++) v_[q] += ld_l2(bgp + (long)(q * SX + w) * N);
                }
                double carry = 0.0;
#pragma unroll
                for (int q = SG - 1; q >= 0; q--) {
                    const double v = v_[q] + carry;
                    const double cy = carry_of(v);
                    carry = cy;
                    if (q < SO) op[glwe_off(q, nco) + i] = (int)digit_of(v, cy);
                }
            }
        };
        if (is_ep) {
            norm_share_ep(1);
            norm_share_ep(0);
            TSTAMP(6);
            if (!last) { if (!tail_barrier(ctr, abortp, ta.seq, (++epoch) * G, flag, false, tid)) break; }
        } else {
        norm_share(1);
        if (last) {
            norm_share(0);
            TSTAMP(6);
        } else {
            tail_arrive(ctr, tid);
            norm_share(0);
            TSTAMP(6);
            ++epoch;
            if (!tail_wait(ctr, abortp, ta.seq, epoch * G, flag, tid)) break;
        }
        }
        TSTAMP(7);
    }
    __syncthreads();
    if (tid == 0) {
        const unsigned old = __hip_atomic_fetch_add(ctr + 1, 1u, __ATOMIC_RELAXED, __HIP_MEMORY_SCOPE_AGENT);
        if (old == (unsigned)(G - 1)) {
            __hip_atomic_store(ctr, 0u, __ATOMIC_RELAXED, __HIP_MEMORY_SCOPE_AGENT);
            __hip_atomic_store(ctr + 2, 0u, __ATOMIC_RELAXED, __HIP_MEMORY_SCOPE_AGENT);
            __hip_atomic_store(ctr + 1, 0u, __ATOMIC_RELAXED, __HIP_MEMORY_SCOPE_AGENT);
        }
    }
}
#undef FK_TAIL_OPND
```

Measured before the change: 1332.

## Defer tail-kernel fallback launch to host and run single write side-work on main stream

The persistent trace-tail kernel now writes a give-up flag to host memory when its grid barrier aborts. The always-enqueued fallback chain kernel is no longer launched after each tail launch. The host records it as pending and only launches it when the flag shows the tail gave up, or when more work is enqueued. Separately, a single-address write with a precomputed inverse keeps its side work on the main stream, which avoids fork/join events with stream2. The write-done event is recorded lazily. Together these changes add host-side bookkeeping and a possible re-run of the export step.

```diff
diff --git a/fhe-ram_amd/csrc/ctx.hpp b/fhe-ram_amd/csrc/ctx.hpp
--- a/fhe-ram_amd/csrc/ctx.hpp
+++ b/fhe-ram_amd/csrc/ctx.hpp
@@ -82,6 +82,14 @@
         for (void* p : pinned) hipHostFree(p);
         events.clear(); dev.clear(); pinned.clear();
     }
+};
+
+struct PendingFallback {
+    int kind = 0;
+    unsigned seq = 0;
+    int gx = 0, gy = 0;
+    RowChainArgs ra;
+    KsChainArgs ca;
 };
 
 struct fheram_ctx {
@@ -145,6 +153,9 @@
     unsigned tail_fb_mark = 0;
     uint64_t tail_launch_mark = 0;
     unsigned* d_tail_sync = nullptr;
+    unsigned* h_tail_gu = nullptr;
+    bool defer_ok = false, defer_fb = false;
+    PendingFallback tail_pend;
     unsigned mid_seq = 0;
     uint64_t mid_launches = 0, mid_launch_mark = 0;
     unsigned mid_fb_mark = 0;
@@ -162,6 +173,7 @@
     bool inv_pending[2] = {false, false};
     hipEvent_t ev_wdone = nullptr;
     bool wdone_pending = false;
+    bool wdone_recorded = false;
     hipEvent_t ev_opstart = nullptr;
     bool opstart_valid = false;
     bool wide_unsynced = false;
@@ -175,6 +187,7 @@
     hipEvent_t ev_w = nullptr;
     bool w_busy = false;
     bool side_begun = false;
+    bool side_on_main = false;
     bool trhi_in_C = false;
     bool tree_rotate_pending = false;
     bool words_staged = false;
@@ -230,8 +243,29 @@
 
 GlweRef ref(int32_t* p, long sy, long sx) { return GlweRef{p, sy, sx}; }
 
-void main_waited(fheram_ctx* c) { c->wide_unsynced = c->derive_unsynced = false; c->main_idle = true; }
-void main_enqueued(fheram_ctx* c) { c->main_idle = false; }
+void fallback_enqueue(fheram_ctx* c) {
+    PendingFallback& f = c->tail_pend;
+    if (!f.kind) return;
+    const dim3 grid(f.gx, f.gy, 1);
+    if (f.kind == 1) {
+        if (c->s_evk == 5) hipLaunchKernelGGL((k_read_chain<5, 4>), grid, dim3(T), LDS_BYTES, c->stream, f.ra);
+        else hipLaunchKernelGGL((k_read_chain<4, 4>), grid, dim3(T), LDS_BYTES, c->stream, f.ra);
+    } else {
+        if (c->s_evk == 5) hipLaunchKernelGGL((k_keyswitch_chain<3, 5, 3>), grid, dim3(T), LDS_BYTES, c->stream, f.ca);
+        else hipLaunchKernelGGL((k_keyswitch_chain<3, 4, 3>), grid, dim3(T), LDS_BYTES, c->stream, f.ca);
+    }
+    f.kind = 0;
+}
+bool main_waited(fheram_ctx* c) {
+    bool ran = false;
+    if (c->tail_pend.kind) {
+        if (__atomic_load_n(c->h_tail_gu, __ATOMIC_ACQUIRE) == c->tail_pend.seq) { fallback_enqueue(c); hipStreamSynchronize(c->stream); ran = true; }
+        else c->tail_pend.kind = 0;
+    }
+    c->wide_unsynced = c->derive_unsynced = false; c->main_idle = true;
+    return ran;
+}
+void main_enqueued(fheram_ctx* c) { fallback_enqueue(c); c->main_idle = false; }
 
 hipEvent_t get_event(fheram_ctx* c) {
     if (!c->ev_pool.empty()) { hipEvent_t e = c->ev_pool.back(); c->ev_pool.pop_back(); return e; }
@@ -319,6 +353,7 @@
 int upload_i64(fheram_ctx* c, int32_t* dst, const int64_t* src, size_t n) {
     int rc = pin_init(c);
     if (rc != FHERAM_OK) return rc;
+    fallback_enqueue(c);
     bool ok = true;
     int k = 0;
     for (size_t off = 0; off < n && ok; off += PIN_CHUNK, k++) {
@@ -337,6 +372,7 @@
 int download_i64(fheram_ctx* c, int64_t* dst, const int32_t* src, size_t n) {
     int rc = pin_init(c);
     if (rc != FHERAM_OK) return rc;
+    fallback_enqueue(c);
     const size_t n_chunks = (n + PIN_CHUNK - 1) / PIN_CHUNK;
     for (size_t k = 0; k <= n_chunks; k++) {
         if (k < n_chunks) {
diff --git a/fhe-ram_amd/csrc/fheram.hip b/fhe-ram_amd/csrc/fheram.hip
--- a/fhe-ram_amd/csrc/fheram.hip
+++ b/fhe-ram_amd/csrc/fheram.hip
@@ -205,6 +205,8 @@
     }
     CCHK(c->res.host(&c->h_tail_fb, 64, hipHostMallocDefault));
     *c->h_tail_fb = 0;
+    CCHK(c->res.host(&c->h_tail_gu, 64, hipHostMallocDefault));
+    *c->h_tail_gu = 0;
     CCHK(c->res.host(&c->h_mid_fb, 128, hipHostMallocDefault));
     memset(c->h_mid_fb, 0, 128);
     CCHK(c->res.host(&c->h_res, ((size_t)c->ws * G + 1) * sizeof(int64_t), hipHostMallocMapped));
@@ -220,6 +222,7 @@
     if (!c) return;
     hipSetDevice(c->device);
     for (hipStream_t s : {c->stream, c->stream2}) if (s) hipStreamSynchronize(s);
+    c->tail_pend.kind = 0;
     prof_collect(c);
     dense_free(c->batch);
     c->res.release();
@@ -250,6 +253,7 @@
     if (atk_ggsw_inv_p != -1) return fail(c, FHERAM_ERR_KEYS, "auto_key.p() != -1 (coordinate_prepared.rs:134)");
     HIPCHK(c, hipSetDevice(c->device));
     HIPCHK(c, hipStreamSynchronize(c->stream));
+    main_waited(c);
     HIPCHK(c, hipStreamSynchronize(c->stream2));
     int order[LOGN];
     for (int i = 0; i < LOGN; i++) {
@@ -348,14 +352,15 @@
     if (!c) return FHERAM_ERR_INVALID_ARG;
     HIPCHK(c, hipSetDevice(c->device));
     HIPCHK(c, hipStreamSynchronize(c->stream));
-    HIPCHK(c, hipGetLastError());
     main_waited(c);
+    HIPCHK(c, hipGetLastError());
     return check_precision(c);
 }
 int fheram_roundoff_max(fheram_ctx* c, double* max_out) {
     if (!c || !max_out) return FHERAM_ERR_INVALID_ARG;
     HIPCHK(c, hipSetDevice(c->device));
     HIPCHK(c, hipStreamSynchronize(c->stream));
+    main_waited(c);
     HIPCHK(c, hipStreamSynchronize(c->stream2));
     double m = 0.0;
     HIPCHK(c, hipMemcpy(&m, c->d_tw + N, sizeof(double), hipMemcpyDeviceToHost));
@@ -367,6 +372,7 @@
     if (!c) return FHERAM_ERR_INVALID_ARG;
     HIPCHK(c, hipSetDevice(c->device));
     HIPCHK(c, hipStreamSynchronize(c->stream));
+    main_waited(c);
     HIPCHK(c, hipStreamSynchronize(c->stream2));
     HIPCHK(c, hipMemset(c->d_tw + N, 0, sizeof(double)));
     __atomic_store_n(c->h_ro_flag, 0u, __ATOMIC_RELAXED);
@@ -379,7 +385,9 @@
     if (c->n_shards != 1) return fail(c, FHERAM_ERR_INVALID_ARG, "row-sharded context: use fheram_read_partial / fheram_read_finish");
     if (c->ram.state) return fail(c, FHERAM_ERR_STATE, "invalid call to Memory.read: internal state is true -> requires calling Memory.write");
     HIPCHK(c, hipSetDevice(c->device));
+    c->defer_ok = true;
     rc = run_op(c, addr, 0, [&] { return read_impl(one_addr(c, &addr), ctx_view(c), false); });
+    c->defer_ok = false;
     if (rc != FHERAM_OK) return rc;
     HIPCHK(c, hipGetLastError());
     return out ? fheram_result_download(c, out) : FHERAM_OK;
@@ -413,7 +421,9 @@
     if (c->n_shards != 1) return fail(c, FHERAM_ERR_INVALID_ARG, "row-sharded context: use fheram_read_partial / fheram_read_finish");
     if (c->ram.state) return fail(c, FHERAM_ERR_STATE, "invalid call to Memory.read: internal state is true -> requires calling Memory.write");
     HIPCHK(c, hipSetDevice(c->device));
+    c->defer_ok = true;
     rc = run_op(c, addr, 1, [&] { return read_impl(one_addr(c, &addr), ctx_view(c), true); });
+    c->defer_ok = false;
     if (rc != FHERAM_OK) return rc;
     c->ram.state = true;
     HIPCHK(c, hipGetLastError());
@@ -667,8 +677,11 @@
     HIPCHK(c, hipSetDevice(c->device));
     HIPCHK(c, hipEventRecord(c->t1, c->stream));
     HIPCHK(c, hipEventSynchronize(c->t1));
+    if (main_waited(c)) {
+        HIPCHK(c, hipEventRecord(c->t1, c->stream));
+        HIPCHK(c, hipEventSynchronize(c->t1));
+    }
     HIPCHK(c, hipEventElapsedTime(ms, c->t0, c->t1));
-    main_waited(c);
     return check_precision(c);
 }
 int fheram_profile_enable(fheram_ctx* c, int on) {
@@ -698,6 +711,8 @@
     HIPCHK(c, hipSetDevice(c->device));
     unsigned fb[2] = {0, 0};
     HIPCHK(c, hipStreamSynchronize(c->stream2));
+    HIPCHK(c, hipStreamSynchronize(c->stream));
+    main_waited(c);
     for (int i = 0; i < 2; i++)
         HIPCHK(c, hipMemcpyAsync(&fb[i], c->d_mid_sync[i] + MID_GROUPS_MAX * 32 + 1, sizeof(unsigned), hipMemcpyDeviceToHost, c->stream));
     HIPCHK(c, hipStreamSynchronize(c->stream));
@@ -715,6 +730,8 @@
     if (!c) return FHERAM_ERR_INVALID_ARG;
     HIPCHK(c, hipSetDevice(c->device));
     unsigned fb = 0;
+    HIPCHK(c, hipStreamSynchronize(c->stream));
+    main_waited(c);
     HIPCHK(c, hipMemcpyAsync(&fb, c->d_tail_sync + TAIL_GROUPS * 32 + 1, sizeof(unsigned), hipMemcpyDeviceToHost, c->stream));
     HIPCHK(c, hipStreamSynchronize(c->stream));
     if (launches) *launches = c->tail_launches;
@@ -754,6 +771,7 @@
         HIPCHK(c, hipMemcpy(dg.p, h.data(), fheram_ctx::GGSW * 4, hipMemcpyHostToDevice));
     }
     c->cur = c->stream;
+    main_enqueued(c);
     launch_prepare(c, dg.p, c->d_prep, (int)(fheram_ctx::GGSW / N));
     GlweRef ra = ref(da.p, 0, (long)G), rb = ref(db.p, 0, (long)G);
     for (int i = 0; i < 3; i++) { launch_ep(c, ra, rb, c->d_prep, batch, 1); launch_ep(c, rb, ra, c->d_prep, batch, 1); }
@@ -785,6 +803,7 @@
             for (int i = 0; i < LOGN; i++) { c->cur = c->stream; launch_prepare(c, dg.p, c->d_atk + (size_t)i * c->atk, (int)(c->atk / N), c->gal[i]); }
     }
     c->cur = c->stream;
+    main_enqueued(c);
     if (kind == 1) launch_prepare(c, dg.p, c->d_prep, n * (int)(fheram_ctx::GGSW / N));
     GlweRef ra = ref(da.p, 0, (long)G), rb = ref(db.p, 0, (long)G), rc = ref(dc.p, 0, (long)G);
     auto once = [&](int i) {
diff --git a/fhe-ram_amd/csrc/kernels.hpp b/fhe-ram_amd/csrc/kernels.hpp
--- a/fhe-ram_amd/csrc/kernels.hpp
+++ b/fhe-ram_amd/csrc/kernels.hpp
@@ -1535,6 +1535,7 @@
     int n_ep = 0;
     const double* ggsw[4];
     GlweRef ep_out;
+    unsigned* give_up_host = nullptr;
 };
 constexpr int TAIL_EP_MAX = 4;
 __device__ __forceinline__ int xcc_id() {
diff --git a/fhe-ram_amd/csrc/launch.hpp b/fhe-ram_amd/csrc/launch.hpp
--- a/fhe-ram_amd/csrc/launch.hpp
+++ b/fhe-ram_amd/csrc/launch.hpp
@@ -153,6 +153,9 @@
         return {ChainForm::Chain, 0};
     return {ChainForm::Steps, 0};
 }
+bool write_one_stream(const fheram_ctx* c, int n, long side_cts, bool inv0_early) {
+    return n == 1 && c->n2 == 2 && c->n_shards == 1 && !capturing(c) && inv0_early && side_cts >= c->cus;
+}
 bool chain_bufs(int n, GlweRef src, GlweRef dst, GlweRef tmp, GlweRef (&b)[2]) {
     if (n % 2 == 1) { if (same(src, dst)) return false; b[0] = dst; b[1] = tmp; }
     else { b[0] = tmp; b[1] = dst; }
@@ -339,7 +342,7 @@
     ProfScope pt(c, "keyswitch_tail_launch", (uint64_t)gx * gy * n, 1);
     TailArgs ta;
     ta.src = src; ta.buf[0] = b[0]; ta.buf[1] = b[1]; ta.tw = c->d_tw; ta.big = big_of(c); ta.sync = c->d_tail_sync;
-    ta.n_ep = prep ? d : 0; ta.ep_out = ep_out;
+    ta.n_ep = prep ? d : 0; ta.ep_out = ep_out; ta.give_up_host = c->h_tail_gu;
     for (int i = 0; i < TAIL_EP_MAX; i++) ta.ggsw[i] = (prep && i < d) ? prep + (size_t)i * fheram_ctx::GGSW : nullptr;
     if (++c->tail_seq == 0) ++c->tail_seq;
     c->tail_launches++;
@@ -377,6 +380,12 @@
             return;
         }
         hipLaunchKernelGGL((k_trace_tail<3, SK, 3>), groups, dim3(T), LDS_BYTES, c->cur, ta);
+        if (c->defer_fb) {
+            PendingFallback& f = c->tail_pend;
+            f.kind = ta.n_ep ? 1 : 2; f.seq = ta.seq; f.gx = gx; f.gy = gy;
+            if (ta.n_ep) f.ra = ra; else f.ca = ca;
+            return;
+        }
         if (ta.n_ep) hipLaunchKernelGGL((k_read_chain<SK, 4>), dim3(gx, gy, 1), dim3(T), LDS_BYTES, c->cur, ra);
         else hipLaunchKernelGGL((k_keyswitch_chain<3, SK, 3>), dim3(gx, gy, 1), dim3(T), LDS_BYTES, c->cur, ca);
     });
@@ -457,10 +466,17 @@
     launch_prepare(c, tmp, prep, d * (int)(fheram_ctx::GGSW / N));
 }
 
+void wdone_mark(fheram_ctx* c) {
+    if (!c->wdone_pending || c->wdone_recorded) return;
+    if (c->main_idle) { c->wdone_pending = false; return; }
+    hipEventRecord(c->ev_wdone, c->stream);
+    c->wdone_recorded = true;
+}
 void precompute_inverse(fheram_ctx* c, const fheram_addr* addr, int ci, bool fork, unsigned gate_seq = 0) {
     if (fork && c->wdone_pending) {
+        if (!c->wdone_recorded) hipEventRecord(c->ev_wdone, c->stream);
         hipStreamWaitEvent(c->stream2, c->ev_wdone, 0);
-        c->wdone_pending = false;
+        c->wdone_pending = c->wdone_recorded = false;
     }
     if (fork && gate_seq) {
         if (c->opstart_valid) { hipStreamWaitEvent(c->stream2, c->ev_opstart, 0); c->opstart_valid = false; }
diff --git a/fhe-ram_amd/csrc/path.hpp b/fhe-ram_amd/csrc/path.hpp
--- a/fhe-ram_amd/csrc/path.hpp
+++ b/fhe-ram_amd/csrc/path.hpp
@@ -44,7 +44,7 @@
     st->res_in_trtop = st->memo_top;
     c->prep1_ready = false;
 }
-void write_done(fheram_ctx* c, RamState* st) { st->memo_top = false; st->memo_alone = 0; c->side_begun = false; c->tree_rotate_pending = false; }
+void write_done(fheram_ctx* c, RamState* st) { st->memo_top = false; st->memo_alone = 0; c->side_begun = c->side_on_main = false; c->tree_rotate_pending = false; }
 
 template <typename F>
 int run_op(fheram_ctx* c, const fheram_addr* addr, int which, F&& enqueue) {
@@ -87,6 +87,7 @@
 int read_local(const Opnds& o, const RamView& a, bool prepare_write, GlweRef* packed_out, bool to_part) {
     fheram_ctx* c = o.c;
     const int n = o.n, ws = o.ws, Y = o.Y(), R = (int)c->rows;
+    if (n == 1 && prepare_write && !capturing(c)) wdone_mark(c);
     main_enqueued(c);
     c->wide = !prepare_write || n > 1;
     if (n == 1 && prepare_write && c->cfg.pre_inv == 1 && !capturing(c) && (c->wide_unsynced || c->derive_unsynced)) {
@@ -168,12 +169,14 @@
     const GlweRef res = ref(o.st->memo_top ? a.trtop : a.res, G, 0);
     const uint64_t tl0 = c->tail_launches;
     GlweRef tb[2];
+    c->defer_fb = c->defer_ok && n == 1 && c->n_shards == 1 && !gathered && !capturing(c) && !c->profile;
     if (fuse_ep && chain_bufs(LOGN, last, res, tmp, tb))
         launch_trace_tail(c, pk, tb, 0, LOGN, 1, Y, o.prep(0, 1), d1, ep_out, prepare_write, o.table());
     else {
         if (fuse_ep) products1();
         trace_steps(c, last, res, tmp, 0, LOGN, 1, Y);
     }
+    c->defer_fb = false;
     if (gated && !c->opstart_valid && (c->wide_unsynced || c->derive_unsynced)) {
         hipEventRecord(c->ev_opstart, c->stream);
         c->opstart_valid = true;
@@ -269,15 +272,18 @@
 struct ResRun { const int32_t* src; size_t n; };
 int result_export(fheram_ctx* c, const ResRun* runs, int n_runs, int64_t* h, int64_t* d_h, int64_t* out) {
     size_t n = 0;
-    for (int i = 0; i < n_runs; i++) {
-        const int n4 = (int)(runs[i].n / 4);
-        hipLaunchKernelGGL(k_export_i64, dim3((n4 + 255) / 256), dim3(256), 0, c->stream, runs[i].src, reinterpret_cast<long long*>(d_h + n), n4,
-                           reinterpret_cast<const long long*>(c->d_tw + N));
-        n += runs[i].n;
-    }
-    HIPCHK(c, hipStreamSynchronize(c->stream));
+    for (bool again = true; again;) {
+        n = 0;
+        for (int i = 0; i < n_runs; i++) {
+            const int n4 = (int)(runs[i].n / 4);
+            hipLaunchKernelGGL(k_export_i64, dim3((n4 + 255) / 256), dim3(256), 0, c->stream, runs[i].src, reinterpret_cast<long long*>(d_h + n), n4,
+                               reinterpret_cast<const long long*>(c->d_tw + N));
+            n += runs[i].n;
+        }
+        HIPCHK(c, hipStreamSynchronize(c->stream));
+        again = main_waited(c);
+    }
     HIPCHK(c, hipGetLastError());
-    main_waited(c);
     double m;
     std::memcpy(&m, h + n, 8);
     if (c->cfg.monitor && m > MON_LIMIT) __atomic_store_n(c->h_ro_flag, 1u, __ATOMIC_RELAXED);
@@ -343,12 +349,14 @@
     c->wide = true;
     const long G = (long)fheram_ctx::GLWE;
     const long sy = (long)c->rows * G;
-    if (!(c->main_idle && !capturing(c) && c->n_shards == 1)) {
+    fallback_enqueue(c);
+    const bool on_main = write_one_stream(c, o.n, (long)c->rows * o.Y(), o.n == 1 && c->inv_id[0] == o.addrs[0]->id);
+    if (!on_main && !(c->main_idle && !capturing(c) && c->n_shards == 1)) {
         hipEventRecord(c->ev_fork, c->stream);
         hipStreamWaitEvent(c->stream2, c->ev_fork, 0);
     }
     main_enqueued(c);
-    c->cur = c->stream2;
+    c->cur = on_main ? c->stream : c->stream2;
     if (c->n2 == 2) {
         const int kept = o.st->memo_alone;
         c->trhi_in_C = kept > 0 && (LOGN - kept) % 2 == 1;
@@ -358,17 +366,18 @@
         else trace_steps(c, ref(v.rows, sy, G), ref(v.A, sy, G), ref(v.C, sy, G), 0, LOGN, (int)c->rows, o.Y());
         o.st->memo_alone = 0;
     }
-    if (o.n == 1 && c->inv_id[0] == o.addrs[0]->id) wait_inverse(c, c->stream2, 0);
+    if (o.n == 1 && c->inv_id[0] == o.addrs[0]->id) wait_inverse(c, c->cur, 0);
     else for (int k = 0; k < o.n; k++) coordinate_prepare_inv(c, o.addrs[k], 0, c->d_ggsw_tmp2, o.inv(k, 0));
     if (o.n == 1) { c->inv_id[0] = 0; c->inv_pending[0] = false; }
-    hipEventRecord(c->ev_join, c->stream2);
+    if (!on_main) hipEventRecord(c->ev_join, c->stream2);
     c->cur = c->stream;
     c->side_begun = true;
+    c->side_on_main = on_main;
 }
 void write_side_abort(fheram_ctx* c) {
     if (!c->side_begun) return;
-    hipStreamWaitEvent(c->stream, c->ev_join, 0);
-    c->side_begun = false;
+    if (!c->side_on_main) hipStreamWaitEvent(c->stream, c->ev_join, 0);
+    c->side_begun = c->side_on_main = false;
 }
 int write_rows(const Opnds& o, const RamView& v) {
     fheram_ctx* c = o.c;
@@ -384,7 +393,7 @@
     const bool rot_in_chain = fuse && c->tree_rotate_pending && c->n_shards == 1;
     const GlweRef tree = ref(v.tree, G, 0);
     if (fuse) {
-        hipStreamWaitEvent(c->stream, c->ev_join, 0);
+        if (!c->side_on_main) hipStreamWaitEvent(c->stream, c->ev_join, 0);
         launch_write_chain(c, part, c->n_shards, c->shard, data, trhi, o.inv(0, 0), d0, LOGN, R, Y, o.table(), rot_in_chain ? &tree : nullptr, -(int)c->rows_glob);
     } else if (c->n2 == 2)
         trace_steps(c, part, B, D, 0, LOGN, R, Y, c->n_shards, c->shard);
@@ -393,7 +402,7 @@
         hipLaunchKernelGGL((k_rotate<3>), dim3(1, Y, EW_SLICES), dim3(256), 0, c->cur, part, ref(v.tree, G, 0), -(int)c->rows_glob);
     }
     if (!fuse) {
-        hipStreamWaitEvent(c->stream, c->ev_join, 0);
+        if (!c->side_on_main) hipStreamWaitEvent(c->stream, c->ev_join, 0);
         if (c->n2 == 2) {
             ProfScope ps(c, "elementwise", (uint64_t)R * Y);
             if (o.rows_dense()) hipLaunchKernelGGL((k_sub_add_norm<3>), dim3(R, Y, EW_SLICES), dim3(256), 0, c->cur, data, trhi, B, data);
@@ -402,7 +411,7 @@
         }
         for (int k = 0; k < n; k++) ep_chain(c, o.rows(data, k), o.rows(data, k), o.slice(A, k), o.inv(k, 0), d0, R, ws);
     }
-    if (n == 1 && !capturing(c)) { hipEventRecord(c->ev_wdone, c->stream); c->wdone_pending = true; }
+    if (n == 1 && !capturing(c)) { c->wdone_pending = true; c->wdone_recorded = false; }
     write_done(c, o.st);
     o.st->state = false;
     return FHERAM_OK;
diff --git a/fhe-ram_amd/csrc/trace_tail.inc b/fhe-ram_amd/csrc/trace_tail.inc
--- a/fhe-ram_amd/csrc/trace_tail.inc
+++ b/fhe-ram_amd/csrc/trace_tail.inc
@@ -46,8 +46,9 @@
     load_twiddles(tw, ta.tw, tid);
     unsigned epoch = 0;
     auto out_of = [&](int s_) -> GlweRef { return s_ < n_ep ? (s_ == n_ep - 1 ? ta.ep_out : ta.buf[s_ & 1]) : ta.buf[(s_ - n_ep) & 1]; };
+    int s = 0;
 #pragma unroll 1
-    for (int s = 0; s < n_all; s++) {
+    for (; s < n_all; s++) {
         const GlweRef rin = (s == 0) ? ta.src : out_of(s - 1);
         const GlweRef rout = out_of(s);
         const int32_t* ap = rin.p + ct * rin.sy + cx * rin.sx;
@@ -245,6 +246,7 @@
         }
         TSTAMP(7);
     }
+    if (s < n_all && tid == 0 && ta.give_up_host) __hip_atomic_store(ta.give_up_host, ta.seq, __ATOMIC_RELAXED, __HIP_MEMORY_SCOPE_SYSTEM);
     __syncthreads();
     if (tid == 0) {
         const unsigned old = __hip_atomic_fetch_add(ctr + 1, 1u, __ATOMIC_RELAXED, __HIP_MEMORY_SCOPE_AGENT);
```

Result: no change. 1340 (median of 6 runs) (+0.6%).
